# harukaki/brl

Measured on AMD Instinct MI355X. Metric: env-steps/sec at num_envs=8192, 32-step rollout, 1/2/4/8 MI355X, higher is better.
Workload: dtype u8

## Files before the change

brl_amd/_capi.py:

```python
from __future__ import annotations

import ctypes as C
import os

_PKG = os.path.dirname(os.path.abspath(__file__))
LIB_PATH = os.path.join(_PKG, "lib", "libbrl_hip.so")

STATE_WORDS = 16
OBS_SIZE = 480
NUM_ACTIONS = 38

_vp = C.c_void_p


class Fields(C.Structure):
    _names = ["current_player", "terminated", "rewards", "step_count", "turn", "dealer", "vul_ns", "vul_ew",
              "shuffled_players", "last_bid", "last_bidder", "call_x", "call_xx", "pass_num",
              "first_denomination_ns", "first_denomination_ew", "hand", "tricks", "lut_idx", "board_ctr", "illegal"]
    _fields_ = [(n, _vp) for n in _names]


class TransitionPtrs(C.Structure):
    _names = ["done", "action", "value", "reward", "log_prob", "obs", "legal_action_mask"]
    _fields_ = [(n, _vp) for n in _names]


class TableInfoPtrs(C.Structure):
    _names = ["terminated", "rewards", "last_bid", "last_bidder", "call_x", "call_xx"]
    _fields_ = [(n, _vp) for n in _names]


class MacroExt(C.Structure):
    _fields_ = [("first", C.c_int32), ("last", C.c_int32), ("value_in", _vp), ("value_stride", C.c_int64), ("value_out", _vp),
                ("done_out", _vp), ("reward_out", _vp), ("actor", _vp), ("reward_scale", C.c_float), ("obs_fmt", C.c_int32),
                ("terminated_count", _vp), ("obs_cast", _vp), ("in_fmt", C.c_int32), ("reserved", C.c_int32),
                ("head_h", _vp), ("head_ldh", C.c_int64), ("head_w", _vp), ("head_b", _vp), ("head_hidden", C.c_int32),
                ("head_fmt", C.c_int32), ("head_part", _vp), ("head_part_stride", C.c_int64), ("head_part_ld", C.c_int32),
                ("head_nparts", C.c_int32)]


class EvalStatsPtrs(C.Structure):
    _names = ["illegal_prob_sum", "step_count", "pass_count", "bid_count"]
    _fields_ = [(n, _vp) for n in _names]


class MlpRef(C.Structure):
    _fields_ = [("nlayers", C.c_int32), ("act", C.c_int32), ("in_features", C.c_int64), ("hidden", C.c_int64),
                ("w", _vp * 8), ("b", _vp * 8), ("actor_w", _vp), ("actor_b", _vp), ("critic_w", _vp), ("critic_b", _vp)]


class ShardGeom(C.Structure):
    _fields_ = [("nbuckets", C.c_int32), ("world", C.c_int32), ("nsub", C.c_int32), ("reserved", C.c_int32),
                ("off", C.c_int64 * 12), ("len", C.c_int64 * 12)]


class FairNet(C.Structure):
    _fields_ = [("w", _vp * 11), ("b", _vp * 11), ("head_w", _vp), ("head_b", _vp)]


class FairWork(C.Structure):
    _names = ("inp", "dzs", "gates", "cat6", "x4", "dz0", "dz6", "dheads", "tiles", "partials", "gram_partials")
    _fields_ = [(n, _vp) for n in _names]


EVAL_COUNTS = 231


class BrlError(RuntimeError):
    pass


_lib = None


def lib() -> C.CDLL:
    global _lib
    if _lib is not None:
        return _lib
    if not os.path.exists(LIB_PATH):
        raise BrlError(
            f"{LIB_PATH} is missing: the HIP extension has not been built. "
            "Run `python -m brl_amd.build` (needs hipcc, gfx950). brl_amd has no CPU fallback."
        )
    L = C.CDLL(LIB_PATH)
    i64, i32, u32, u64, f32 = C.c_int64, C.c_int, C.c_uint32, C.c_uint64, C.c_float
    L.brl_last_error.restype = C.c_char_p
    L.brl_version.restype = i32
    sigs = {
        "brl_create": [i32, _vp, _vp, i64, C.POINTER(_vp)],
        "brl_set_lut": [_vp, _vp, _vp, i64],
        "brl_destroy": [_vp],
        "brl_set_rng": [_vp, u64, u64],
        "brl_init_random": [_vp, _vp, i64, u32, _vp],
        "brl_init_from_deals": [_vp, _vp, i64, _vp, _vp, _vp, _vp, _vp, _vp, _vp],
        "brl_step": [_vp, _vp, _vp, i64, _vp, i32, _vp, _vp, _vp, _vp, _vp, _vp],
        "brl_observe": [_vp, _vp, i64, _vp, _vp, _vp, _vp],
        "brl_get_fields": [_vp, _vp, i64, C.POINTER(Fields), _vp],
        "brl_rollout_random": [_vp, _vp, i64, i32, i32, u32, f32, C.POINTER(TransitionPtrs), _vp, _vp, _vp, _vp],
        "brl_rollout_random_gae": [_vp, _vp, i64, i32, u32, f32, C.POINTER(TransitionPtrs), _vp, _vp, _vp, _vp, f32, f32, _vp, _vp,
                                   _vp],
        "brl_policy_step": [_vp, _vp, _vp, i64, _vp, i32, u32, i32, _vp, _vp, _vp, _vp, _vp, _vp, _vp, _vp],
        "brl_policy_step_at": [_vp, _vp, _vp, i64, _vp, i64, i32, _vp, u32, i32, _vp, _vp, _vp, _vp, _vp, _vp, _vp, _vp],
        "brl_policy_step_ex": [_vp, _vp, _vp, i64, _vp, i64, i32, _vp, u32, i32, _vp, _vp, _vp, _vp, _vp, _vp, _vp,
                               C.POINTER(MacroExt), _vp],
        "brl_obs_cast": [_vp, _vp, i64, _vp, i32, _vp],
        "brl_obs_cast_rows": [_vp, _vp, _vp, i64, _vp, i32, _vp],
        "brl_live_index": [_vp, _vp, i64, _vp, _vp, i64, _vp],
        "brl_linear_act_heads": [_vp, _vp, i64, _vp, i64, _vp, _vp, i64, i64, i32, i32, i32, i32, _vp, i64, i32, _vp, i64, i64, _vp],
        "brl_linear_act": [_vp, _vp, i64, _vp, i64, _vp, _vp, i64, i64, i32, i32, i32, i32, _vp],
        "brl_gae": [_vp, _vp, _vp, _vp, _vp, f32, f32, i32, i64, _vp, _vp, _vp],
        "brl_imp_reward": [_vp, _vp, _vp, _vp, i64, _vp],
        "brl_duplicate_step": [_vp, _vp, _vp, i64, _vp, C.POINTER(TableInfoPtrs), C.POINTER(TableInfoPtrs),
                               _vp, _vp, _vp, _vp, _vp, _vp],
        "brl_eval_step": [_vp, _vp, _vp, i64, _vp, i64, _vp, i64, C.POINTER(TableInfoPtrs), C.POINTER(TableInfoPtrs),
                          C.POINTER(EvalStatsPtrs), i32, _vp, _vp, _vp, _vp, _vp, _vp, _vp, _vp, _vp],
        "brl_eval_step_team": [_vp, _vp, _vp, i64, _vp, i64, i32, C.POINTER(TableInfoPtrs), C.POINTER(TableInfoPtrs),
                               C.POINTER(EvalStatsPtrs), i32, _vp, _vp, _vp, _vp, _vp, _vp, _vp, _vp, _vp, _vp],
        "brl_eval_reduce": [_vp, i64, C.POINTER(TableInfoPtrs), C.POINTER(TableInfoPtrs), _vp, _vp, _vp, _vp],
        "brl_ppo_loss": [i32, _vp, i64, _vp, _vp, _vp, _vp, _vp, _vp, _vp, i64, f32, f32, f32, i32, i32, _vp, _vp, _vp, _vp, _vp],
        "brl_ppo_stats": [i32, _vp, i64, _vp, f32, f32, _vp, _vp],
        "brl_ppo_heads_loss_split": [i32, _vp, i64, _vp, _vp, i64, _vp, _vp, _vp, _vp, _vp, _vp, i64, f32, f32, f32, i32, i32, i32, _vp, _vp, _vp, _vp, _vp, i32, _vp],
        "brl_ppo_heads_bwd": [i32, _vp, _vp, i64, _vp, i64, i64, i32, i32, _vp, _vp, _vp, _vp, _vp, _vp, i64, _vp, _vp, _vp, _vp],
        "brl_ppo_stats_rows": [i32, _vp, _vp, i64, i64, f32, f32, f32, _vp, _vp],
        "brl_mb_gather_bind": [i32, C.POINTER(TransitionPtrs), _vp, _vp, _vp, _vp, i64, _vp, _vp, _vp, _vp, _vp, _vp, _vp, i64, _vp, _vp],
        "brl_adam_clip_fin_gather": [i32, _vp, _vp, _vp, _vp, i64, _vp, f32, _vp, f32, f32, f32, f32, _vp, i64, _vp, _vp, _vp, i64,
                                     i32, _vp, _vp, _vp, _vp, _vp],
        "brl_mb_gather_dev": [i32, _vp, i64, _vp],
        "brl_ppo_stats_gram": [i32, _vp, i64, i64, _vp, i64, f32, f32, f32, _vp, _vp, _vp, _vp],
        "brl_ppo_illegal_grad": [i32, _vp, _vp, _vp, f32, i64, _vp, _vp],
        "brl_act_bwd_colsum": [i32, _vp, _vp, i64, i64, i64, i32, _vp, _vp],
        "brl_act_bwd_colsum_heads_dw": [i32, _vp, _vp, i64, i64, i64, i32, _vp, _vp, _vp, i64, i64, i64, i32, _vp, _vp, _vp, _vp, i64,
                                        _vp, _vp, _vp, _vp],
        "brl_bias_finalize_ex": [i32, i32, _vp, _vp, _vp, _vp, _vp],
        "brl_bias_finalize_rows": [i32, i32, _vp, _vp, _vp, _vp, i32, _vp, _vp],
        "brl_fair_forward": [i32, C.POINTER(FairNet), _vp, i64, i32, _vp, _vp, _vp],
        "brl_mlp_gemm_group": [i32, i32, i32, _vp, _vp, _vp, _vp, _vp, _vp, _vp, _vp, _vp, _vp],
        "brl_fair_chain": [i32, C.POINTER(FairNet), _vp, _vp, _vp, _vp, _vp, _vp, _vp, i64, f32, f32, f32, i32, i32, i32, i32,
                           C.POINTER(FairWork), _vp],
        "brl_mlp_gemm": [i32, i32, i32, _vp, i64, _vp, i64, _vp, i64, i64, i64, i64, i32, _vp, _vp, i64, _vp, _vp, _vp],
        "brl_mlp_gemm_x3_workspace": [i64, i64, i64, _vp],
        "brl_mlp_gemm_x3_group": [i32, i32, i32, _vp, _vp, _vp, _vp, _vp, _vp, _vp, _vp, _vp, _vp],
        "brl_split_planes": [i32, _vp, i64, _vp, i64, _vp],
        "brl_linear_x3p": [i32, _vp, i32, i64, i64, _vp, i64, i64, _vp, i32, _vp, i64, _vp, i64, i64, i64, i64, i64, _vp],
        "brl_mlp_gemm_x3": [i32, i32, i32, _vp, i64, _vp, i64, _vp, i64, i64, i64, i64, i32, _vp, _vp, i64, _vp, _vp, i64, _vp],
        "brl_mlp_forward_rows": [i32, C.POINTER(MlpRef), _vp, _vp, i64, _vp, i64, _vp, i64, _vp],
        "brl_adam_shard_norm": [i32, _vp, C.POINTER(ShardGeom), i32, i32, f32, _vp, _vp, _vp, _vp],
        "brl_adam_shard_apply": [i32, _vp, _vp, _vp, _vp, C.POINTER(ShardGeom), i32, i32, _vp, _vp, f32, _vp, f32, f32, f32, f32, f32, _vp,
                                 _vp, i64, _vp],
        "brl_mlp_gemm_dh_heads_dw": [i32, _vp, i64, _vp, i64, _vp, i64, i64, i64, i64, i32, _vp, i64, _vp, _vp, _vp, i64, i64, i64, i32,
                                     _vp, _vp, _vp, _vp, i64, _vp, _vp, _vp, _vp],
    }
    sigs.update(sl_signatures())
    for name, args in sigs.items():
        fn = getattr(L, name)
        fn.argtypes = args
        fn.restype = i32
    _lib = L
    return L


EXPORTS = ["brl_last_error", "brl_version", "brl_create", "brl_set_lut", "brl_destroy", "brl_set_rng",
           "brl_init_random", "brl_init_from_deals", "brl_step", "brl_observe", "brl_get_fields",
           "brl_rollout_random", "brl_policy_step", "brl_policy_step_at", "brl_obs_cast", "brl_obs_cast_rows", "brl_live_index", "brl_linear_act", "brl_linear_act_heads", "brl_gae", "brl_imp_reward", "brl_duplicate_step",
           "brl_eval_step", "brl_eval_reduce", "brl_ppo_loss", "brl_ppo_stats", "brl_policy_step_ex",
           "brl_eval_step_team", "brl_rollout_random_gae", "brl_ppo_heads_loss_split", "brl_adam_shard_norm", "brl_adam_shard_apply", "brl_ppo_heads_bwd", "brl_ppo_stats_gram",
           "brl_act_bwd_colsum", "brl_act_bwd_colsum_heads_dw", "brl_bias_finalize_ex", "brl_ppo_stats_rows", "brl_mb_gather_bind", "brl_mb_gather_dev", "brl_ppo_illegal_grad", "brl_adam_clip_fin_gather", "brl_mlp_gemm", "brl_mlp_gemm_dh_heads_dw", "brl_mlp_forward_rows",
           "brl_bias_finalize_rows", "brl_fair_chain", "brl_mlp_gemm_group", "brl_fair_forward", "brl_mlp_gemm_x3", "brl_mlp_gemm_x3_workspace", "brl_mlp_gemm_x3_group", "brl_split_planes", "brl_linear_x3p"]


def sl_signatures() -> dict:
    i64, i32, u64, f32 = C.c_int64, C.c_int, C.c_uint64, C.c_float
    return {
        "brl_sl_sample": [i32, _vp, _vp, i64, u64, i64, _vp, _vp, _vp],
        "brl_sl_replay": [i32, _vp, _vp, _vp, i64, _vp, _vp, i64, _vp, _vp, _vp, _vp],
        "brl_sl_loss": [i32, _vp, i64, _vp, _vp, i64, f32, _vp, _vp, _vp, i64, _vp],
    }


def check(rc: int) -> None:
    if rc != 0:
        raise BrlError(f"libbrl_hip error {rc}: {lib().brl_last_error().decode()}")


def ptr(t):
    if t is None:
        return None
    assert t.is_contiguous(), "brl_amd passes raw pointers: tensors must be contiguous"
    return t.data_ptr()
```

brl_amd/csrc/brl_mlp_gemm_x3.hip:

```cpp
#include <hip/hip_runtime.h>
#include <stdint.h>

#include "abi_common.hpp"
#include "mlp_gemm_x3.hpp"
#include "mlp_linear_x3p.hpp"

static int64_t x3_tiles(int64_t m, int64_t n) { return ((m + 127) / 128) * ((n + 127) / 128); }

static int64_t x3_workspace_bytes(int64_t m, int64_t n, int64_t k) {
  const int sk = mgs::pick_splitk(m, n, k);
  if (sk == 1) return 0;
  const int64_t tiles = x3_tiles(m, n);
  return ((tiles * 4 + 255) / 256) * 256 + tiles * sk * (int64_t)mgs::SLAB_FLOATS * 4;
}

extern "C" int brl_mlp_gemm_x3_workspace(int64_t m, int64_t n, int64_t k, int64_t *bytes) {
  NEED(bytes && m > 0 && n > 0 && k > 0, "bytes / m / n / k");
  *bytes = x3_workspace_bytes(m, n, k);
  return BRL_OK;
}

extern "C" int brl_mlp_gemm_x3(int device, int layout, int epilogue, const float *a, int64_t lda, const float *b, int64_t ldb, float *c,
                               int64_t ldc, int64_t m, int64_t n, int64_t k, int act, const float *bias, const float *gate, int64_t ldg,
                               float *colsum, void *workspace, int64_t workspace_bytes, void *stream) {
  NEED(a && b && c && m > 0 && n > 0 && k > 0, "a / b / c / m / n / k");
  NEED(layout >= BRL_GEMM_NT && layout <= BRL_GEMM_TN, "layout (BRL_GEMM_NT / _NN / _TN)");
  NEED(m < (1 << 24) && n < (1 << 24) && k < (1 << 24), "m / n / k below 2^24");
  NEED(n % 4 == 0 && ldc % 4 == 0 && lda % 4 == 0 && ldb % 4 == 0 && ldc >= n, "n and the leading dimensions multiples of 4 (16-byte pieces)");
  const bool akc = layout != BRL_GEMM_TN, bkc = layout == BRL_GEMM_NT;
  NEED(k % 32 == 0, "k a multiple of 32 (whole 32-deep chunks; other k: brl_mlp_gemm)");
  NEED(akc ? lda >= k : lda >= ((m + 3) & ~(int64_t)3), "lda (where m is contiguous in a: at least m rounded up to 4 — whole 16-byte pieces are read)");
  NEED(bkc ? ldb >= k : ldb >= n, "ldb");
  NEED((akc ? m * lda : k * lda) < (1ll << 29) && (bkc ? n * ldb : k * ldb) < (1ll << 29), "operands below 2 GB");
  NEED(act == 0 || act == 1, "act (0 ReLU, 1 tanh)");
  NEED((epilogue == BRL_GEMM_EPI_NONE) || (epilogue == BRL_GEMM_EPI_BIAS_ACT && layout == BRL_GEMM_NT && bias) ||
           (epilogue == BRL_GEMM_EPI_GATE_COLSUM && layout == BRL_GEMM_NN && gate && ldg >= n && ldg % 4 == 0),
       "epilogue (NONE; BIAS_ACT with NT + bias; GATE_COLSUM with NN + gate)");
  NEED((((uintptr_t)a | (uintptr_t)b | (uintptr_t)c | (uintptr_t)bias | (uintptr_t)gate | (uintptr_t)colsum) & 15) == 0, "16-byte alignment");
  HIP_TRY(hipSetDevice(device));
  mgs::Args X{};
  mg::Args &G = X.g;
  G.A = a; G.lda = lda; G.B = b; G.ldb = ldb; G.C = c; G.ldc = ldc;
  G.M = (int)m; G.N = (int)n; G.K = (int)k; G.act = act;
  G.bias = bias; G.gate = gate; G.ldg = ldg; G.colsum = colsum;
  const int64_t tiles = x3_tiles(m, n);
  int sk = mgs::pick_splitk(m, n, k);
  const int64_t tick = ((tiles * 4 + 255) / 256) * 256;
  if (sk > 1 && (workspace == nullptr || workspace_bytes < tick + tiles * sk * (int64_t)mgs::SLAB_FLOATS * 4)) sk = 1;
  NEED(sk == 1 || (((uintptr_t)workspace) & 255) == 0, "workspace: 256-byte alignment");
  NEED(sk == 1 || tiles * sk * (int64_t)mgs::SLAB_FLOATS * 4 < (1ll << 31), "partial tiles below 2 GB");
  X.splitk = sk;
  X.tickets = (unsigned *)workspace;
  X.slabs = sk > 1 ? (float *)((char *)workspace + tick) : nullptr;
  const unsigned blocks = (unsigned)(tiles * sk);
  hipStream_t s = (hipStream_t)stream;
#define X3_LAUNCH(AK, BK_, E) hipLaunchKernelGGL((mgs::k_gemm_x3s<AK, BK_, E>), dim3(blocks), dim3(mgs::THREADS), 0, s, X)
  if (layout == BRL_GEMM_NT) {
    if (epilogue == BRL_GEMM_EPI_BIAS_ACT) X3_LAUNCH(true, true, mg::EPI_BIAS_ACT);
    else X3_LAUNCH(true, true, mg::EPI_NONE);
  } else if (layout == BRL_GEMM_NN) {
    if (epilogue == BRL_GEMM_EPI_GATE_COLSUM) X3_LAUNCH(true, false, mg::EPI_GATE_COLSUM);
    else X3_LAUNCH(true, false, mg::EPI_NONE);
  } else {
    X3_LAUNCH(false, false, mg::EPI_NONE);
  }
#undef X3_LAUNCH
  HIP_TRY(hipGetLastError());
  return BRL_OK;
}

extern "C" int brl_mlp_gemm_x3_group(int device, int layout, int count, const float *const *a, const int64_t *lda, const float *const *b,
                                     const int64_t *ldb, float *const *c, const int64_t *ldc, const int64_t *m, const int64_t *n,
                                     const int64_t *k, void *stream) {
  NEED(count >= 1 && count <= mgs::GROUP_MAX && a && lda && b && ldb && c && ldc && m && n && k, "count (1..8) / NULL array");
  NEED(layout >= BRL_GEMM_NT && layout <= BRL_GEMM_TN, "layout (BRL_GEMM_NT / _NN / _TN)");
  const bool akc = layout != BRL_GEMM_TN, bkc = layout == BRL_GEMM_NT;
  mgs::GroupArgs GA{};
  GA.n = count;
  for (int i = 0; i < count; i++) {
    NEED(a[i] && b[i] && c[i] && m[i] > 0 && n[i] > 0 && k[i] > 0, "a / b / c / m / n / k");
    NEED(m[i] < (1 << 24) && n[i] < (1 << 24) && k[i] < (1 << 24), "m / n / k below 2^24");
    NEED(n[i] % 4 == 0 && ldc[i] % 4 == 0 && lda[i] % 4 == 0 && ldb[i] % 4 == 0 && ldc[i] >= n[i], "n and the leading dimensions multiples of 4");
    NEED(k[i] % 32 == 0, "k a multiple of 32 (whole 32-deep chunks; other k: brl_mlp_gemm_group)");
    NEED(akc ? lda[i] >= k[i] : lda[i] >= ((m[i] + 3) & ~(int64_t)3), "lda (where m is contiguous in a: at least m rounded up to 4)");
    NEED(bkc ? ldb[i] >= k[i] : ldb[i] >= n[i], "ldb");
    NEED((akc ? m[i] * lda[i] : k[i] * lda[i]) < (1ll << 29) && (bkc ? n[i] * ldb[i] : k[i] * ldb[i]) < (1ll << 29), "operands below 2 GB");
    NEED((((uintptr_t)a[i] | (uintptr_t)b[i] | (uintptr_t)c[i]) & 15) == 0, "16-byte alignment");
    mgs::Args &X = GA.x[i];
    mg::Args &G = X.g;
    G.A = a[i]; G.lda = lda[i]; G.B = b[i]; G.ldb = ldb[i]; G.C = c[i]; G.ldc = ldc[i];
    G.M = (int)m[i]; G.N = (int)n[i]; G.K = (int)k[i];
    X.splitk = 1;
    GA.first[i + 1] = GA.first[i] + (int)x3_tiles(m[i], n[i]);
  }
  HIP_TRY(hipSetDevice(device));
  hipStream_t s = (hipStream_t)stream;
  const unsigned blocks = (unsigned)GA.first[count];
  if (layout == BRL_GEMM_NT) hipLaunchKernelGGL((mgs::k_gemm_x3s_group<true, true>), dim3(blocks), dim3(mgs::THREADS), 0, s, GA);
  else if (layout == BRL_GEMM_NN) hipLaunchKernelGGL((mgs::k_gemm_x3s_group<true, false>), dim3(blocks), dim3(mgs::THREADS), 0, s, GA);
  else hipLaunchKernelGGL((mgs::k_gemm_x3s_group<false, false>), dim3(blocks), dim3(mgs::THREADS), 0, s, GA);
  HIP_TRY(hipGetLastError());
  return BRL_OK;
}

extern "C" int brl_split_planes(int device, const float *x, int64_t n, uint16_t *planes, int64_t plane_stride, void *stream) {
  NEED(x && planes && n > 0 && n % 4 == 0 && plane_stride >= n && plane_stride % 4 == 0, "x / planes / n (a multiple of 4) / plane_stride");
  NEED((((uintptr_t)x) & 15) == 0 && (((uintptr_t)planes) & 7) == 0, "alignment (x 16 bytes, planes 8)");
  HIP_TRY(hipSetDevice(device));
  hipLaunchKernelGGL(lx3::k_split_planes, dim3((unsigned)((n / 4 + 255) / 256)), dim3(256), 0, (hipStream_t)stream, x, planes, plane_stride, n / 4);
  HIP_TRY(hipGetLastError());
  return BRL_OK;
}

extern "C" int brl_linear_x3p(int device, const uint16_t *x_planes, int npx, int64_t ldx, int64_t sx, const uint16_t *w_planes, int64_t ldw,
                              int64_t sw, const float *bias, int relu, float *y, int64_t ldy, uint16_t *y_planes, int64_t ldyp, int64_t syp,
                              int64_t m, int64_t n, int64_t k, void *stream) {
  NEED(x_planes && w_planes && bias && (y || y_planes) && m > 0 && n > 0 && k > 0, "x_planes / w_planes / bias / an output / m / n / k");
  NEED(npx == 1 || npx == 3, "npx (3 planes, or 1: x exact in bf16)");
  NEED(n % 128 == 0 && k % 32 == 0, "n a multiple of 128, k a multiple of 32");
  NEED(m < (1 << 24) && n < (1 << 24) && k < (1 << 24), "m / n / k below 2^24");
  NEED(ldx >= k && ldx % 8 == 0 && ldw >= k && ldw % 8 == 0, "ldx / ldw (at least k, multiples of 8: 16-byte pieces)");
  NEED(m * ldx < (1ll << 31) && n * ldw < (1ll << 31), "planes below 4 GB each");
  NEED(!y || (ldy >= n && ldy % 4 == 0), "ldy");
  NEED(!y_planes || (ldyp >= n && ldyp % 8 == 0 && syp % 8 == 0), "ldyp / syp (multiples of 8)");
  NEED(sx % 8 == 0 && sw % 8 == 0, "plane strides multiples of 8");
  NEED((((uintptr_t)x_planes | (uintptr_t)w_planes | (uintptr_t)bias | (uintptr_t)y | (uintptr_t)y_planes) & 15) == 0, "16-byte alignment");
  HIP_TRY(hipSetDevice(device));
  lx3::Args G{};
  G.x = x_planes; G.ldx = ldx; G.sx = sx; G.w = w_planes; G.ldw = ldw; G.sw = sw; G.bias = bias;
  G.y = y; G.ldy = ldy; G.yp = y_planes; G.ldyp = ldyp; G.syp = syp;
  G.M = (int)m; G.N = (int)n; G.K = (int)k; G.relu = relu ? 1 : 0;
  hipStream_t s = (hipStream_t)stream;
  const unsigned blocks = (unsigned)(((m + 127) / 128) * (n / 128));
  if (npx == 3) hipLaunchKernelGGL(lx3::k_linear_x3p<3>, dim3(blocks), dim3(lx3::THREADS), 0, s, G);
  else hipLaunchKernelGGL(lx3::k_linear_x3p<1>, dim3(blocks), dim3(lx3::THREADS), 0, s, G);
  HIP_TRY(hipGetLastError());
  return BRL_OK;
}
```

brl_amd/csrc/brl_ppo.hip:

```cpp
#include <hip/hip_runtime.h>
#include <math.h>
#include <stdint.h>
#include <stdio.h>
#include <stdlib.h>
#include <string.h>

#include "abi_common.hpp"

static inline unsigned thread_grid(int64_t n, int bs) { return (unsigned)((n + bs - 1) / bs); }

struct PpoArgs {
  const float *logits;
  int64_t ls;
  const float *value;
  const uint8_t *mask;
  const int32_t *action;
  const float *old_value, *old_logp, *gae, *tgt;
  int64_t B;
  float clip_eps, vf_coef, ent_coef;
  int masked, value_clipping;
  float *dlogits, *dvalue, *partials, *illp;
  int64_t vs, dls, dvs;
};

template <int CTRL, int ROW_MASK = 0xF>
__device__ __forceinline__ float dpp_move_f(float old, float v) {
  return __uint_as_float((unsigned)__builtin_amdgcn_update_dpp((int)__float_as_uint(old), (int)__float_as_uint(v), CTRL, ROW_MASK, 0xF, false));
}
__device__ __forceinline__ float wave_sum_f(float v) {
  v += dpp_move_f<0xB1>(0.0f, v);
  v += dpp_move_f<0x4E>(0.0f, v);
  v += dpp_move_f<0x124>(0.0f, v);
  v += dpp_move_f<0x128>(0.0f, v);
  v += dpp_move_f<0x142, 0xA>(0.0f, v);
  v += dpp_move_f<0x143, 0xC>(0.0f, v);
  return __uint_as_float(__builtin_amdgcn_readlane(__float_as_uint(v), 63));
}
__device__ __forceinline__ float wave_max_f(float v) {
  const float ninf = -INFINITY;
  v = fmaxf(v, dpp_move_f<0xB1>(ninf, v));
  v = fmaxf(v, dpp_move_f<0x4E>(ninf, v));
  v = fmaxf(v, dpp_move_f<0x124>(ninf, v));
  v = fmaxf(v, dpp_move_f<0x128>(ninf, v));
  v = fmaxf(v, dpp_move_f<0x142, 0xA>(ninf, v));
  v = fmaxf(v, dpp_move_f<0x143, 0xC>(ninf, v));
  return __uint_as_float(__builtin_amdgcn_readlane(__float_as_uint(v), 63));
}

struct PpoSampleIn {
  bool legal;
  int act;
  float old_logp, old_value, tgt, gae;
};
__device__ __forceinline__ PpoSampleIn ppo_sample_load(const PpoArgs &A, int64_t b, bool valid, int lane) {
  const int64_t bb = valid ? b : 0;
  PpoSampleIn S;
  S.legal = (lane < BRL_NUM_ACTIONS) && A.mask[bb * BRL_NUM_ACTIONS + ((lane < BRL_NUM_ACTIONS) ? lane : 0)] != 0;
  S.act = A.action[bb];
  S.old_logp = A.old_logp[bb];
  S.old_value = A.old_value[bb];
  S.tgt = A.tgt[bb];
  S.gae = A.gae[bb];
  return S;
}
__device__ __forceinline__ void ppo_loss_sample(const PpoArgs &A, const PpoSampleIn &S, int64_t b, bool valid, int lane, float lg, float v,
                                                float g, float (&st)[5], float &illp_lane) {
  const bool in = lane < BRL_NUM_ACTIONS;
  const bool legal = S.legal;
  const float invB = 1.0f / (float)A.B;
  const float mx = wave_max_f(legal ? lg : -INFINITY);
  const float lse = logf(wave_sum_f(legal ? expf(lg - mx) : 0.0f));
  const float lsm = legal ? (lg - mx) - lse : 0.0f;
  const float p = legal ? expf(lsm) : 0.0f;
  const float mx2 = wave_max_f(in ? lg : -INFINITY);
  const float lse2 = logf(wave_sum_f(in ? expf(lg - mx2) : 0.0f));
  const float lsm2 = in ? (lg - mx2) - lse2 : 0.0f;
  const float p2 = in ? expf(lsm2) : 0.0f;
  const int act = S.act;
  const float lsel = A.masked ? lsm : lsm2, psel = A.masked ? p : p2;
  const float lp = __shfl(lsel, act & 63, 64);
  const float logratio = lp - S.old_logp;
  const float ratio = expf(logratio);
  const float eps = A.clip_eps;
  const float a1 = ratio * g, a2 = fminf(fmaxf(ratio, 1.0f - eps), 1.0f + eps) * g;
  const float la = -fminf(a1, a2);
  const bool inside = (ratio >= 1.0f - eps) && (ratio <= 1.0f + eps);
  const float dratio = ((a1 < a2) || inside) ? -g : 0.0f;
  const float dlp = dratio * ratio * invB;
  const float ov = S.old_value, t = S.tgt;
  float vl, dv;
  if (A.value_clipping) {
    const float dcl = fminf(fmaxf(v - ov, -eps), eps);
    const float vc = ov + dcl;
    const float l1 = (v - t) * (v - t), l2 = (vc - t) * (vc - t);
    vl = 0.5f * fmaxf(l1, l2);
    const bool unclipped = (v - ov >= -eps) && (v - ov <= eps);
    dv = (l1 >= l2) ? (v - t) : (unclipped ? (vc - t) : 0.0f);
  } else {
    vl = 0.5f * (v - t) * (v - t);
    dv = v - t;
  }
  const float H = -wave_sum_f((legal && p > 0.0f) ? p * lsm : 0.0f);
  const float dH = legal ? -p * (lsm + H) : 0.0f;
  const float onehot = (lane == act) ? 1.0f : 0.0f;
  const bool live = A.masked ? legal : in;
  const float dz = (live ? dlp * (onehot - psel) : 0.0f) - A.ent_coef * invB * dH;
  illp_lane = legal ? 0.0f : p2;
  if (valid && in) {
    A.dlogits[b * A.dls + lane] = dz;
    if (A.illp) A.illp[b * BRL_NUM_ACTIONS + lane] = illp_lane;
  }
  if (lane == 0 && valid) A.dvalue[b * A.dvs] = A.vf_coef * dv * invB;
  st[0] = valid ? vl : 0.0f;
  st[1] = valid ? la : 0.0f;
  st[2] = valid ? H : 0.0f;
  st[3] = valid ? (ratio - 1.0f) - logratio : 0.0f;
  st[4] = (valid && fabsf(ratio - 1.0f) > eps) ? 1.0f : 0.0f;
}

__global__ __launch_bounds__(256) void k_ppo_loss(PpoArgs A) {
  __shared__ float part[4][8];
  const int lane = (int)(threadIdx.x & 63u), wave = (int)(threadIdx.x >> 6);
  const int64_t b = (int64_t)blockIdx.x * 4 + wave;
  const bool valid = b < A.B;
  const int64_t bb = valid ? b : 0;
  const float lg = (lane < BRL_NUM_ACTIONS) ? A.logits[bb * A.ls + lane] : 0.0f;
  const PpoSampleIn S = ppo_sample_load(A, b, valid, lane);
  float st[5], ill;
  ppo_loss_sample(A, S, b, valid, lane, lg, A.value[bb * A.vs], S.gae, st, ill);
  if (lane == 0) {
#pragma unroll
    for (int k = 0; k < 5; k++) part[wave][k] = st[k];
  }
  __syncthreads();
  if (threadIdx.x < 8) {
    const int k = (int)threadIdx.x;
    A.partials[(int64_t)blockIdx.x * 8 + k] = (k < 5) ? ((part[0][k] + part[1][k]) + (part[2][k] + part[3][k])) : 0.0f;
  }
}

__global__ __launch_bounds__(512) void k_ppo_stats(const float *partials, int64_t nblk, int64_t batch, const float *G,
                                                   float vf_coef, float ent_coef, float *out, const int32_t *row_index) {
  if (row_index != nullptr) out += 8 * (int64_t)(*row_index);
  constexpr int D = BRL_NUM_ACTIONS, DD = D * D;
  __shared__ float g[DD], m[DD], t[DD], vec[D], red[2], st[8];
  const int tid = (int)threadIdx.x, lane = tid & 63, wv = tid >> 6;
  if (wv >= 3) {
    const int k = wv - 3;
    float s = 0.0f;
    for (int64_t i = lane; i < nblk; i += 64) s += partials[i * 8 + k];
    s = wave_sum_f(s);
    if (lane == 0) st[k] = s / (float)batch;
  }
  for (int e = tid; e < DD; e += 512) g[e] = G ? G[e] : 0.0f;
  __syncthreads();
  auto trace_of = [&](const float *x) {
    if (wv == 0) {
      const float s = wave_sum_f((lane < D) ? x[lane * D + lane] : 0.0f);
      if (lane == 0) red[0] = fmaxf(s, 1.17549435e-38f);
    }
    __syncthreads();
    return red[0];
  };
  float tr = trace_of(g);
  for (int e = tid; e < DD; e += 512) m[e] = g[e] / tr;
  __syncthreads();
  for (int it = 0; it < 8; it++) {
    for (int e = tid; e < DD; e += 512) {
      const int i = e / D, j = e - i * D;
      float s = 0.0f;
#pragma unroll 2
      for (int k = 0; k < D; k++) s += m[i * D + k] * m[k * D + j];
      t[e] = s;
    }
    __syncthreads();
    tr = trace_of(t);
    for (int e = tid; e < DD; e += 512) m[e] = t[e] / tr;
    __syncthreads();
  }
  if (tid < D) {
    float s = 0.0f;
    for (int k = 0; k < D; k++) s += m[tid * D + k];
    vec[tid] = s;
  }
  __syncthreads();
  if (wv == 0) {
    float gv = 0.0f;
    if (lane < D)
      for (int k = 0; k < D; k++) gv += g[lane * D + k] * vec[k];
    const float vi = (lane < D) ? vec[lane] : 0.0f;
    const float num = wave_sum_f(vi * gv), den = wave_sum_f(vi * vi);
    if (lane == 0) {
      out[6] = 0.5f * sqrtf(fmaxf(num / fmaxf(den, 1.17549435e-38f), 0.0f));
      out[0] = st[1] + vf_coef * st[0] - ent_coef * st[2];
      out[1] = st[0]; out[2] = st[1]; out[3] = st[2]; out[4] = st[3]; out[5] = st[4];
      out[7] = 0.0f;
    }
  }
}

#include "ppo_update.hpp"
#include "ppo_heads.hpp"
#include "fair_chain.hpp"

extern "C" int brl_ppo_loss(int device, const float *logits, int64_t logits_stride, const float *value, const uint8_t *mask,
                            const int32_t *action, const float *old_value, const float *old_log_prob, const float *gae,
                            const float *targets, int64_t batch, float clip_eps, float vf_coef, float ent_coef, int masked,
                            int value_clipping, float *dlogits, float *dvalue, float *partials, float *illegal_probs,
                            void *stream) {
  NEED(batch > 0, "batch");
  NEED(logits && value && mask && action && old_value && old_log_prob && gae && targets, "NULL input array");
  NEED(dlogits && dvalue && partials, "NULL output array");
  NEED(logits_stride >= BRL_NUM_ACTIONS, "logits_stride");
  HIP_TRY(hipSetDevice(device));
  PpoArgs A{logits, logits_stride, value, mask, action, old_value, old_log_prob, gae, targets, batch, clip_eps, vf_coef,
            ent_coef, masked, value_clipping, dlogits, dvalue, partials, illegal_probs, 1, BRL_NUM_ACTIONS, 1};
  hipLaunchKernelGGL(k_ppo_loss, dim3(thread_grid(batch, 4)), dim3(256), 0, (hipStream_t)stream, A);
  HIP_TRY(hipGetLastError());
  return BRL_OK;
}

extern "C" int brl_mb_gather_bind(int device, const brl_transition *flat, const float *adv, const float *targets, const int64_t *perm,
                                  const int32_t *mb_index, int64_t mbs, float *x0, uint8_t *mask, int32_t *action, float *old_value,
                                  float *old_log_prob, float *gae_out, float *targets_out, int64_t nsteps, void *args_dev,
                                  void *stream) {
  NEED(flat && flat->obs && flat->legal_action_mask && flat->action && flat->value && flat->log_prob, "trajectory");
  NEED(adv && targets && perm && mb_index && mbs > 0, "adv / targets / perm / mb_index / mbs");
  NEED(x0 && mask && action && old_value && old_log_prob && gae_out && targets_out && args_dev, "NULL output array / args_dev");
  HIP_TRY(hipSetDevice(device));
  static_assert(sizeof(GatherArgs) <= 256, "args_dev is 256 bytes");
  NEED(nsteps > 0, "nsteps (minibatches in perm)");
  GatherArgs A{flat->obs, flat->legal_action_mask, flat->action, flat->value, flat->log_prob, adv, targets, perm, mb_index, mbs,
               x0, mask, action, old_value, old_log_prob, gae_out, targets_out, nsteps};
  hipLaunchKernelGGL(k_mb_gather_bind, dim3(1), dim3(64), 0, (hipStream_t)stream, A, (GatherArgs *)args_dev);
  HIP_TRY(hipGetLastError());
  return BRL_OK;
}

extern "C" int brl_mb_gather_dev(int device, const void *args_dev, int64_t mbs, void *stream) {
  NEED(args_dev && mbs > 0, "args_dev / mbs");
  HIP_TRY(hipSetDevice(device));
  hipLaunchKernelGGL(k_mb_gather_dev, dim3((unsigned)mbs), dim3(128), 0, (hipStream_t)stream, (const GatherArgs *)args_dev);
  HIP_TRY(hipGetLastError());
  return BRL_OK;
}

extern "C" int brl_act_bwd_colsum(int device, float *dh, const float *h, int64_t rows, int64_t cols, int64_t ld, int act,
                                  float *scratch, void *stream) {
  NEED(dh && h && scratch && rows > 0 && cols > 0 && ld >= cols, "dh / h / scratch / rows / cols / ld");
  NEED(cols % 4 == 0 && ld % 4 == 0, "cols and ld multiples of 4");
  NEED(act == 0 || act == 1, "act (0 ReLU, 1 tanh)");
  HIP_TRY(hipSetDevice(device));
  const int64_t tiles = (rows + 15) / 16;
  hipLaunchKernelGGL(k_relu_bwd_tiles4, dim3((unsigned)((cols + 255) / 256), (unsigned)tiles), dim3(256), 0, (hipStream_t)stream,
                     dh, h, rows, cols, ld, scratch, act);
  HIP_TRY(hipGetLastError());
  return BRL_OK;
}

extern "C" int brl_act_bwd_colsum_heads_dw(int device, float *dz, const float *hh, int64_t rows, int64_t cols, int64_t ld, int act,
                                           float *scratch, const float *dheads, const float *h, int64_t ldh, int64_t batch,
                                           int64_t hidden, int nsplit, float *dw_partials, float *db_partials,
                                           const float *loss_partials, const float *gram_partials, int64_t ngroups,
                                           const int32_t *row_index, float *stat_sums, float *gram_sums, void *stream) {
  NEED(dz && hh && scratch && rows > 0 && cols > 0 && ld >= cols, "dz / h / scratch / rows / cols / ld");
  NEED(cols % 4 == 0 && ld % 4 == 0, "cols and ld multiples of 4");
  NEED(act == 0 || act == 1, "act (0 ReLU, 1 tanh)");
  NEED(batch > 0 && hidden > 0 && hidden % 256 == 0 && ldh >= hidden && ldh % 4 == 0, "batch / hidden (a multiple of 256) / ldh");
  NEED(dheads && h && dw_partials && db_partials, "NULL array");
  NEED(nsplit >= 1 && (batch + nsplit - 1) / nsplit <= 64, "nsplit: at most 64 rows per split");
  HIP_TRY(hipSetDevice(device));
  HeadsBwdArgs A{};
  A.dheads = dheads; A.h = h; A.ldh = ldh; A.B = batch; A.H = (int)hidden; A.act = act; A.nsplit = nsplit;
  A.rows_per_split = (int)((batch + nsplit - 1) / nsplit);
  A.dWh_partials = dw_partials; A.dbh_partials = db_partials;
  A.blocks_a = (int)(hidden / HB_JT) * nsplit;
  const bool sums = gram_sums != nullptr;
  NEED(!sums || (loss_partials && gram_partials && ngroups > 0 && row_index && stat_sums), "statistics sums: partials / ngroups / row_index / stat_sums");
  A.loss_partials = loss_partials; A.gram_partials = gram_partials; A.ngroups = (int)ngroups; A.row_index = row_index;
  A.stat_sums = stat_sums; A.gram_sums = gram_sums;
  const int gx = (int)((cols + 255) / 256), gy = (int)((rows + 15) / 16);
  const unsigned blocks = (unsigned)(gx * gy + A.blocks_a + (sums ? HB_GRAM_BLOCKS : 0));
  hipLaunchKernelGGL(k_relu_bwd_tiles4_heads_dw, dim3(blocks), dim3(256), 0, (hipStream_t)stream, dz, hh, rows, cols, ld, scratch, act, gx, gy, A);
  HIP_TRY(hipGetLastError());
  return BRL_OK;
}

extern "C" int brl_bias_finalize_ex(int device, int nseg, const float *const *partials, const int64_t *cols, const int64_t *tiles,
                                    float *const *out, void *stream) {
  NEED(nseg >= 1 && nseg <= BIAS_MAX_SEGS && partials && cols && tiles && out, "nseg / partials / cols / tiles / out");
  HIP_TRY(hipSetDevice(device));
  BiasSegs S{};
  S.n = nseg;
  int64_t maxc = 0;
  for (int i = 0; i < nseg; i++) {
    NEED(partials[i] && out[i] && cols[i] > 0 && tiles[i] > 0, "segment");
    S.tiles[i] = tiles[i]; S.partials[i] = partials[i]; S.cols[i] = cols[i]; S.db[i] = out[i];
    maxc = cols[i] > maxc ? cols[i] : maxc;
  }
  hipLaunchKernelGGL(k_bias_finalize, dim3((unsigned)((maxc + 63) / 64), (unsigned)nseg), dim3(256), 0, (hipStream_t)stream, S);
  HIP_TRY(hipGetLastError());
  return BRL_OK;
}

extern "C" int brl_bias_finalize_rows(int device, int nseg, const float *const *partials, const int64_t *cols, const int64_t *tiles,
                                      float *const *out, int first_row_seg, const int32_t *row_index, void *stream) {
  NEED(nseg >= 1 && nseg <= BIAS_MAX_SEGS && partials && cols && tiles && out, "nseg / partials / cols / tiles / out");
  NEED(first_row_seg >= 0 && first_row_seg <= nseg && (row_index || first_row_seg == nseg), "first_row_seg / row_index");
  HIP_TRY(hipSetDevice(device));
  BiasSegs S{};
  S.n = nseg;
  int64_t maxc = 0;
  for (int i = 0; i < nseg; i++) {
    NEED(partials[i] && out[i] && cols[i] > 0 && tiles[i] > 0, "segment");
    S.tiles[i] = tiles[i]; S.partials[i] = partials[i]; S.cols[i] = cols[i]; S.db[i] = out[i];
    maxc = cols[i] > maxc ? cols[i] : maxc;
  }
  S.row_index = (first_row_seg < nseg) ? row_index : nullptr;
  S.first_row_seg = first_row_seg;
  hipLaunchKernelGGL(k_bias_finalize, dim3((unsigned)((maxc + 63) / 64), (unsigned)nseg), dim3(256), 0, (hipStream_t)stream, S);
  HIP_TRY(hipGetLastError());
  return BRL_OK;
}

#ifdef FAIR_TIMING
extern "C" int brl_fair_set_dbg(void *p) {
  HIP_TRY(hipMemcpyToSymbol(HIP_SYMBOL(g_fair_dbg), &p, sizeof(p)));
  return BRL_OK;
}
#endif

extern "C" int brl_fair_chain(int device, const brl_fair_net *net, const float *x0, const uint8_t *mask, const int32_t *action,
                              const float *old_value, const float *old_log_prob, const float *gae, const float *targets,
                              int64_t batch, float clip_eps, float vf_coef, float ent_coef, int masked, int value_clipping,
                              int reward_scaling, int act, const brl_fair_work *work, void *stream) {
  NEED(net && work && x0 && mask && action && old_value && old_log_prob && gae && targets, "NULL input");
  NEED(batch > 0 && batch % fair::R == 0, "batch (a multiple of 16)");
  NEED(act == 0 || act == 1, "act");
  fair::Args A{};
  for (int l = 0; l < 11; l++) {
    NEED(net->w[l] && net->b[l], "net: NULL layer");
    NEED((((uintptr_t)net->w[l]) & 15) == 0 && (((uintptr_t)net->b[l]) & 15) == 0, "net: 16-byte alignment");
    A.net.w[l] = net->w[l]; A.net.b[l] = net->b[l];
  }
  NEED(net->head_w && net->head_b && (((uintptr_t)net->head_w) & 15) == 0, "net: heads");
  A.net.wh = net->head_w; A.net.bh = net->head_b;
  NEED(work->inp && work->dzs && work->gates && work->cat6 && work->x4 && work->dz0 && work->dz6 && work->dheads && work->tiles &&
       work->partials, "work: NULL array");
  const void *al[] = {x0, work->inp, work->dzs, work->gates, work->cat6, work->x4, work->dz0, work->dz6, work->tiles};
  for (const void *q : al) NEED((((uintptr_t)q) & 15) == 0, "16-byte alignment");
  A.o = fair::Bufs{work->inp, work->dzs, work->gates, work->cat6, work->x4, work->dz0, work->dz6, work->dheads, work->tiles,
                   work->partials, work->gram_partials};
  A.x0 = x0;
  A.P = PpoArgs{nullptr, 0, nullptr, mask, action, old_value, old_log_prob, gae, targets, batch, clip_eps, vf_coef,
                ent_coef, masked, value_clipping, nullptr, nullptr, nullptr, nullptr, 1, BRL_NUM_ACTIONS, 1};
  A.act = act;
  A.reward_scaling = reward_scaling;
  HIP_TRY(hipSetDevice(device));
  A.nrows = batch;
  hipLaunchKernelGGL(fair::k_fair_chain<true>, dim3((unsigned)(batch / fair::R)), dim3(fair::NW * 64), 0, (hipStream_t)stream, A);
  HIP_TRY(hipGetLastError());
  return BRL_OK;
}

extern "C" int brl_fair_forward(int device, const brl_fair_net *net, const float *x, int64_t rows, int act, float *logits, float *value,
                                void *stream) {
  NEED(net && x && logits && value, "NULL array");
  NEED(rows >= 0 && rows < (1ll << 31), "rows");
  NEED(act == 0 || act == 1, "act");
  if (rows == 0) return BRL_OK;
  fair::Args A{};
  for (int l = 0; l < 11; l++) {
    NEED(net->w[l] && net->b[l], "net: NULL layer");
    NEED((((uintptr_t)net->w[l]) & 15) == 0 && (((uintptr_t)net->b[l]) & 15) == 0, "net: 16-byte alignment");
    A.net.w[l] = net->w[l]; A.net.b[l] = net->b[l];
  }
  NEED(net->head_w && net->head_b && (((uintptr_t)net->head_w) & 15) == 0 && (((uintptr_t)x) & 15) == 0, "net: heads / x: 16-byte alignment");
  A.net.wh = net->head_w; A.net.bh = net->head_b;
  A.x0 = x;
  A.act = act;
  A.nrows = rows;
  A.logits_out = logits;
  A.value_out = value;
  HIP_TRY(hipSetDevice(device));
  hipLaunchKernelGGL(fair::k_fair_chain<false>, dim3((unsigned)((rows + fair::R - 1) / fair::R)), dim3(fair::NW * 64), 0,
                     (hipStream_t)stream, A);
  HIP_TRY(hipGetLastError());
  return BRL_OK;
}

extern "C" int brl_ppo_heads_loss_split(int device, const float *h, int64_t ldh, const float *head_w, const float *head_b,
                                        int64_t hidden, const uint8_t *mask, const int32_t *action, const float *old_value,
                                        const float *old_log_prob, const float *gae, const float *targets, int64_t batch,
                                        float clip_eps, float vf_coef, float ent_coef, int masked, int value_clipping,
                                        int reward_scaling, float *heads_out, float *dheads, float *partials, float *gram_partials,
                                        float *head_parts, int ksplit, void *stream) {
  NEED(batch > 0 && hidden > 0 && hidden % 16 == 0 && ldh >= hidden && ldh % 4 == 0, "batch / hidden (a multiple of 16) / ldh");
  NEED(h && head_w && head_b && mask && action && old_value && old_log_prob && gae && targets, "NULL input array");
  NEED(dheads && partials && head_parts, "NULL output array");
  NEED(ksplit >= 1 && ksplit <= 8, "ksplit (1..8)");
  HIP_TRY(hipSetDevice(device));
  constexpr int64_t HS = BRL_NUM_ACTIONS + 1;
  HeadsProductArgs G{};
  G.h = h; G.ldh = ldh; G.Wh = head_w; G.H = (int)hidden; G.B = batch; G.ksplit = ksplit; G.parts = head_parts; G.part_stride = batch * HS;
  hipLaunchKernelGGL(k_heads_product, dim3((unsigned)((batch + 15) / 16), (unsigned)ksplit), dim3(HD_WAVES * 64), 0, (hipStream_t)stream, G);
  HeadsLossArgs A{};
  A.h = h; A.ldh = ldh; A.Wh = head_w; A.bh = head_b; A.H = (int)hidden;
  A.P = PpoArgs{nullptr, HS, nullptr, mask, action, old_value, old_log_prob, gae, targets, batch, clip_eps, vf_coef,
                ent_coef, masked, value_clipping, dheads, dheads + BRL_NUM_ACTIONS, partials, nullptr, HS, HS, HS};
  A.heads_out = heads_out; A.gram_partials = gram_partials; A.reward_scaling = reward_scaling;
  A.parts = head_parts; A.nparts = ksplit; A.part_stride = batch * HS;
  hipLaunchKernelGGL(k_heads_loss, dim3((unsigned)((batch + HD_ROWS - 1) / HD_ROWS)), dim3(HD_WAVES * 64), 0, (hipStream_t)stream, A);
  HIP_TRY(hipGetLastError());
  return BRL_OK;
}

extern "C" int brl_ppo_heads_bwd(int device, const float *dheads, const float *h, int64_t ldh, const float *head_w, int64_t batch,
                                 int64_t hidden, int act, int nsplit, float *dw_partials, float *db_partials, float *dh,
                                 float *tile_sums, const float *loss_partials, const float *gram_partials, int64_t ngroups,
                                 const int32_t *row_index, float *stat_sums, float *gram_sums, void *stream) {
  NEED(batch > 0 && hidden > 0 && hidden % 256 == 0 && ldh >= hidden && ldh % 4 == 0, "batch / hidden (a multiple of 256) / ldh");
  NEED(dheads && h && head_w && dh && tile_sums && (!dw_partials == !db_partials), "NULL array");
  const bool with_dw = dw_partials != nullptr;
  NEED(act == 0 || act == 1, "act (0 ReLU, 1 tanh)");
  NEED(nsplit >= 1 && (batch + nsplit - 1) / nsplit <= 64, "nsplit: at most 64 rows per split");
  HIP_TRY(hipSetDevice(device));
  HeadsBwdArgs A{};
  A.dheads = dheads; A.h = h; A.ldh = ldh; A.Wh = head_w; A.B = batch; A.H = (int)hidden; A.act = act; A.nsplit = nsplit;
  A.rows_per_split = (int)((batch + nsplit - 1) / nsplit);
  A.dWh_partials = dw_partials; A.dbh_partials = db_partials; A.dh = dh; A.tile_sums = tile_sums;
  A.blocks_a = (int)(hidden / HB_JT) * nsplit;
  const bool sums = with_dw && gram_sums != nullptr;
  NEED(!sums || (loss_partials && gram_partials && ngroups > 0 && row_index && stat_sums), "statistics sums: partials / ngroups / row_index / stat_sums");
  A.loss_partials = loss_partials; A.gram_partials = gram_partials; A.ngroups = (int)ngroups; A.row_index = row_index;
  A.stat_sums = stat_sums; A.gram_sums = gram_sums;
  const int64_t blocks_b = (hidden / 256) * ((batch + HB_ROWS - 1) / HB_ROWS);
  hipLaunchKernelGGL(k_heads_bwd_dh, dim3((unsigned)blocks_b), dim3(256), 0, (hipStream_t)stream, A);
  if (with_dw)
    hipLaunchKernelGGL(k_heads_bwd_dw, dim3((unsigned)(A.blocks_a + (sums ? HB_GRAM_BLOCKS : 0))), dim3(256), 0, (hipStream_t)stream, A);
  HIP_TRY(hipGetLastError());
  return BRL_OK;
}

extern "C" int brl_ppo_stats_gram(int device, const float *partials, int64_t npartials, int64_t batch, const float *gram_partials,
                                  int64_t ngram, float vf_coef, float ent_coef, float illegal_coef, float *out_rows,
                                  const int32_t *row_index, float *vec_out, void *stream) {
  NEED(partials && out_rows && npartials > 0 && batch > 0, "partials / out_rows / npartials / batch");
  NEED(gram_partials && ngram > 0, "gram_partials / ngram");
  HIP_TRY(hipSetDevice(device));
  hipLaunchKernelGGL(k_ppo_stats2, dim3(1), dim3(1024), 0, (hipStream_t)stream, partials, npartials, batch, gram_partials, ngram,
                     vf_coef, ent_coef, illegal_coef, out_rows, row_index, vec_out);
  HIP_TRY(hipGetLastError());
  return BRL_OK;
}

extern "C" int brl_ppo_illegal_grad(int device, const float *heads, const uint8_t *mask, const float *vec, float illegal_coef,
                                    int64_t batch, float *dheads, void *stream) {
  NEED(heads && mask && vec && dheads && batch > 0, "heads / mask / vec / dheads / batch");
  HIP_TRY(hipSetDevice(device));
  hipLaunchKernelGGL(k_illegal_grad, dim3(thread_grid(batch, 4)), dim3(256), 0, (hipStream_t)stream, heads, mask, vec, illegal_coef,
                     batch, dheads);
  HIP_TRY(hipGetLastError());
  return BRL_OK;
}

extern "C" int brl_ppo_stats_rows(int device, const float *stat_sums, const float *gram_sums, int64_t rows, int64_t batch, float vf_coef,
                                  float ent_coef, float illegal_coef, float *out_rows, void *stream) {
  NEED(stat_sums && gram_sums && out_rows && rows > 0 && batch > 0, "stat_sums / gram_sums / out_rows / rows / batch");
  HIP_TRY(hipSetDevice(device));
  hipLaunchKernelGGL(k_ppo_stats2, dim3((unsigned)rows), dim3(256), 0, (hipStream_t)stream, stat_sums, (int64_t)1, batch, gram_sums,
                     (int64_t)1, vf_coef, ent_coef, illegal_coef, out_rows, (const int32_t *)nullptr, (float *)nullptr);
  HIP_TRY(hipGetLastError());
  return BRL_OK;
}

extern "C" int brl_adam_clip_fin_gather(int device, float *p, float *g, float *m, float *v, int64_t n, float *step, float lr,
                                        const float *lr_dev, float beta1, float beta2, float eps, float max_norm, float *scratch,
                                        int64_t scratch_len, int32_t *mb_index, float *norm_out, const void *gather_args, int64_t mbs,
                                        int nseg, const float *const *partials, const int64_t *cols, const int64_t *tiles,
                                        float *const *out, void *stream) {
  NEED(nseg >= 1 && nseg <= BIAS_MAX_SEGS && partials && cols && tiles && out, "nseg / partials / cols / tiles / out");
  NEED(p && g && m && v && step && scratch && n > 0 && n % 4 == 0, "p / g / m / v / step / scratch / n (a multiple of 4)");
  NEED(!gather_args || (mb_index && mbs > 0), "gather_args needs mb_index and the minibatch size");
  BiasSegs S{};
  S.n = nseg;
  int64_t covered = 0;
  const float *lo = g + n;
  for (int i = 0; i < nseg; i++) {
    NEED(partials[i] && out[i] && cols[i] > 0 && tiles[i] > 0, "segment");
    NEED(out[i] >= g && out[i] + cols[i] <= g + n, "segment outputs must lie inside the gradient buffer");
    S.tiles[i] = tiles[i]; S.partials[i] = partials[i]; S.cols[i] = cols[i]; S.db[i] = out[i];
    covered += cols[i];
    lo = (out[i] < lo) ? out[i] : lo;
  }
  const int64_t tail_lo = lo - g;
  NEED(tail_lo % 4 == 0 && covered <= n - tail_lo && n - tail_lo - covered < 4, "the finalised segments must tile the end of the gradient buffer");
  FinBlocks FB{};
  for (int i = 0; i < nseg; i++) FB.off[i + 1] = FB.off[i] + (int)((cols[i] + 63) / 64);
  NEED(scratch_len >= ADAM_BLOCKS + (int64_t)FB.off[nseg], "scratch too small for the finalize blocks' partials");
  HIP_TRY(hipSetDevice(device));
  const int npartials = ADAM_BLOCKS + FB.off[nseg];
  hipLaunchKernelGGL(k_adam_norm_fin, dim3((unsigned)npartials), dim3(ADAM_THREADS), 0, (hipStream_t)stream, g, n, 1.0f, scratch, step,
                     mb_index, S, tail_lo, FB);
  const unsigned extra = gather_args ? (unsigned)((mbs + 1) / 2) : 0u;
  AdamRange R{};
  R.p = p; R.g = g; R.m = m; R.v = v; R.lo4 = 0; R.hi4 = n >> 2; R.partials = scratch; R.npartials = npartials; R.step = step;
  R.lr_dev = lr_dev; R.lr = lr; R.b1 = beta1; R.b2 = beta2; R.eps = eps; R.max_norm = max_norm; R.gscale = 1.0f; R.norm_out = norm_out;
  hipLaunchKernelGGL(k_adam_apply, dim3((unsigned)ADAM_BLOCKS + extra), dim3(ADAM_THREADS), 0, (hipStream_t)stream, R, ADAM_BLOCKS,
                     (const GatherArgs *)gather_args);
  HIP_TRY(hipGetLastError());
  return BRL_OK;
}

static int shard_geom(const brl_shard_geom *geom, int rank_lo, int rank_hi, ShardGeom *out) {
  NEED(geom && geom->nbuckets >= 1 && geom->nbuckets <= SHARD_MAX_BUCKETS && geom->world >= 1 && geom->nsub >= 1, "geometry");
  NEED(rank_lo >= 0 && rank_lo < rank_hi && rank_hi <= geom->world, "rank range");
  ShardGeom G{};
  G.nb = geom->nbuckets; G.world = geom->world; G.J = geom->nsub;
  for (int b = 0; b < G.nb; b++) {
    NEED(geom->off[b] >= 0 && geom->off[b] % 4 == 0 && geom->len[b] > 0 && geom->len[b] % 4 == 0, "bucket offsets / slice lengths multiples of 4 floats");
    G.off4[b] = geom->off[b] >> 2; G.len4[b] = geom->len[b] >> 2;
    G.blk[b + 1] = G.blk[b] + (int)((G.len4[b] + SHARD_PER4 - 1) / SHARD_PER4);
  }
  *out = G;
  return BRL_OK;
}

extern "C" int brl_adam_shard_norm(int device, const float *g, const brl_shard_geom *geom, int rank_lo, int rank_hi, float grad_scale,
                                   float *partials, float *step, int32_t *mb_index, void *stream) {
  NEED(g && partials && step, "g / partials / step");
  ShardGeom G;
  if (int rc = shard_geom(geom, rank_lo, rank_hi, &G)) return rc;
  HIP_TRY(hipSetDevice(device));
  hipLaunchKernelGGL(k_shard_norm, dim3((unsigned)((rank_hi - rank_lo) * G.nb * G.J)), dim3(ADAM_THREADS), 0, (hipStream_t)stream, g, G,
                     rank_lo, grad_scale, partials, step, mb_index);
  HIP_TRY(hipGetLastError());
  return BRL_OK;
}

extern "C" int brl_adam_shard_apply(int device, float *p, const float *g, float *m, float *v, const brl_shard_geom *geom, int rank_lo,
                                    int rank_hi, const float *partials, const float *step, float lr, const float *lr_dev, float beta1,
                                    float beta2, float eps, float max_norm, float grad_scale, float *norm_out, const void *gather_args,
                                    int64_t mbs, void *stream) {
  NEED(p && g && m && v && partials && step, "p / g / m / v / partials / step");
  NEED(!gather_args || mbs > 0, "gather_args needs the minibatch size");
  ShardGeom G;
  if (int rc = shard_geom(geom, rank_lo, rank_hi, &G)) return rc;
  HIP_TRY(hipSetDevice(device));
  AdamRange R{};
  R.p = p; R.g = g; R.m = m; R.v = v; R.partials = partials; R.npartials = G.world * G.nb * G.J; R.step = step;
  R.lr_dev = lr_dev; R.lr = lr; R.b1 = beta1; R.b2 = beta2; R.eps = eps; R.max_norm = max_norm; R.gscale = grad_scale; R.norm_out = norm_out;
  const int sweep = (rank_hi - rank_lo) * G.blk[G.nb];
  const unsigned extra = gather_args ? (unsigned)((mbs + 1) / 2) : 0u;
  hipLaunchKernelGGL(k_shard_apply, dim3((unsigned)sweep + extra), dim3(ADAM_THREADS), 0, (hipStream_t)stream, R, G, rank_lo, sweep,
                     (const GatherArgs *)gather_args);
  HIP_TRY(hipGetLastError());
  return BRL_OK;
}

extern "C" int brl_ppo_stats(int device, const float *partials, int64_t batch, const float *gram, float vf_coef,
                             float ent_coef, float *out, void *stream) {
  NEED(partials && out && batch > 0, "partials / out / batch");
  HIP_TRY(hipSetDevice(device));
  hipLaunchKernelGGL(k_ppo_stats, dim3(1), dim3(512), 0, (hipStream_t)stream, partials, (int64_t)thread_grid(batch, 4), batch,
                     gram, vf_coef, ent_coef, out, (const int32_t *)nullptr);
  HIP_TRY(hipGetLastError());
  return BRL_OK;
}
```

brl_amd/csrc/mlp_gemm_x3.hpp:

```cpp
#pragma once

#include "mlp_gemm.hpp"

namespace mgs {

using mg::BoolTag;
using mg::f32x4;
using mg::IntTag;
using mg::row16_sum;
typedef __bf16 bf16x8 __attribute__((ext_vector_type(8)));
typedef float f32x16 __attribute__((ext_vector_type(16)));
typedef unsigned u32x4 __attribute__((ext_vector_type(4)));
typedef unsigned u32x2 __attribute__((ext_vector_type(2)));
typedef short s16x4 __attribute__((ext_vector_type(4)));

constexpr int BK = 32, THREADS = 512;
constexpr int PLANE = 128 * BK * 2;
constexpr int OFF_B = 3 * PLANE, STAGE = 6 * PLANE;
constexpr int LDS_BYTES = 2 * STAGE;
constexpr int SLAB_FLOATS = 128 * 128;

#ifndef MGS_R1
#define MGS_R1 6
#endif
#ifndef MGS_BAR
#define MGS_BAR 20
#endif
#ifndef MGS_EXP
#define MGS_EXP 0
#endif

struct Args {
  mg::Args g;
  float *slabs;
  unsigned *tickets;
  int splitk;
};

template <bool A_KC, bool B_KC, int EPI>
__device__ __forceinline__ void gemm_tile(const Args &X, unsigned char *lds, int bid, int nblk) {
  const mg::Args &G = X.g;
  constexpr int NP = 4;
  const int tid = (int)threadIdx.x, lane = tid & 63, w = __builtin_amdgcn_readfirstlane(tid >> 6);
  const int tiles_m = (G.M + 127) / 128, tiles_n = (G.N + 127) / 128, SK = X.splitk;
  if (bid >= tiles_m * tiles_n * SK) return;
  const int L = (nblk % 8 == 0) ? (bid % 8) * (nblk / 8) + bid / 8 : bid;
  const int tile = L / SK, ks = L - tile * SK;
  int tm, tn;
  if (tiles_m % 2 == 0 && tiles_n % 4 == 0) {
    const int blk = tile >> 3, i = tile & 7;
    tm = 2 * (blk / (tiles_n / 4)) + (i >> 2);
    tn = 4 * (blk % (tiles_n / 4)) + (i & 3);
  } else {
    tm = tile / tiles_n;
    tn = tile - tm * tiles_n;
  }
  const int m0 = tm * 128, n0 = tn * 128;
  const int nchunks = G.K / BK;
  const int cps = (nchunks + SK - 1) / SK;
  const int c0 = ks * cps, c1 = (c0 + cps < nchunks) ? c0 + cps : nchunks;
  const int ni = c1 > c0 ? c1 - c0 : 0;

  uint32_t go[NP];
  int lw[NP];
#pragma unroll
  for (int j = 0; j < NP; j++) {
    const bool isB = j >= 2;
    const int q = tid + 512 * (j & 1);
    const int x0 = isB ? n0 : m0, Xn = isB ? G.N : G.M;
    const int64_t ld = isB ? G.ldb : G.lda;
    const int base = isB ? OFF_B : 0;
    if (isB ? B_KC : A_KC) {
      const int row = q >> 3, P = (q >> 1) & 3, half = q & 1;
      const int x = (x0 + row < Xn) ? x0 + row : Xn - 1;
      go[j] = (uint32_t)(((int64_t)x * ld + 16 * half + 4 * P) * 4);
      lw[j] = base + row * 64 + ((P ^ ((row >> 2) & 3)) << 4) + 8 * half;
    } else {
      const int kr = q >> 5, p = q & 31;
      const int col = (x0 + 4 * p < Xn) ? x0 + 4 * p : 0;
      go[j] = (uint32_t)(((int64_t)kr * ld + col) * 4);
      lw[j] = base + kr * 256 + ((p ^ ((kr & 3) << 3)) << 3);
    }
  }
  const uint32_t stepa = (uint32_t)((A_KC ? (int64_t)BK : (int64_t)BK * G.lda) * 4), stepb = (uint32_t)((B_KC ? (int64_t)BK : (int64_t)BK * G.ldb) * 4);
  const __amdgpu_buffer_rsrc_t srda = __builtin_amdgcn_make_buffer_rsrc(const_cast<float *>(G.A), (short)0, 0x7FFFFFFF, 0x00020000);
  const __amdgpu_buffer_rsrc_t srdb = __builtin_amdgcn_make_buffer_rsrc(const_cast<float *>(G.B), (short)0, 0x7FFFFFFF, 0x00020000);
  uint32_t soa = (uint32_t)c0 * stepa, sob = (uint32_t)c0 * stepb;
  unsigned msk;
  asm volatile("s_mov_b32 %0, 0xffff0000" : "=s"(msk));
#ifndef MGS_SETS
#define MGS_SETS 1
#endif
  f32x4 rg[MGS_SETS][NP];
  int nreq = 0;
  auto gload = [&](auto set_tag, int j) __attribute__((always_inline)) {
    constexpr int S = decltype(set_tag)::value;
    const bool isB = j >= 2;
    rg[S][j] = __builtin_bit_cast(f32x4, __builtin_amdgcn_raw_buffer_load_b128(isB ? srdb : srda, (int)go[j], (int)(isB ? sob : soa), 0));
  };
  auto gadvance = [&]() __attribute__((always_inline)) {
    nreq++;
    if (nreq < ni) { soa += stepa; sob += stepb; }
  };
  unsigned sh[3][2];
  float sr0, sr1;
  auto stage_part = [&](auto set_tag, int j, int half, int part, unsigned char *st) __attribute__((always_inline)) {
    constexpr int S = decltype(set_tag)::value;
    if (part == 0) {
      const f32x4 v = rg[S][j];
      const float x0 = half ? v.z : v.x, x1 = half ? v.w : v.y;
      const unsigned u0 = __float_as_uint(x0), u1 = __float_as_uint(x1);
      sh[0][half] = __builtin_amdgcn_perm(u1, u0, 0x07060302u);
      if (MGS_EXP & 1) { sr0 = x0; sr1 = x1; }
      else { sr0 = x0 - __uint_as_float(u0 & msk); sr1 = x1 - __uint_as_float(u1 & msk); }
    } else if (part == 1) {
      const unsigned v0 = __float_as_uint(sr0), v1 = __float_as_uint(sr1);
      sh[1][half] = __builtin_amdgcn_perm(v1, v0, 0x07060302u);
      if (!(MGS_EXP & 1)) { sr0 = sr0 - __uint_as_float(v0 & msk); sr1 = sr1 - __uint_as_float(v1 & msk); }
    } else {
      sh[2][half] = __builtin_amdgcn_perm(__float_as_uint(sr1), __float_as_uint(sr0), 0x07060302u);
      if (half) {
        unsigned char *p = st + lw[j];
        *reinterpret_cast<u32x2 *>(p) = u32x2{sh[0][0], sh[0][1]};
        *reinterpret_cast<u32x2 *>(p + PLANE) = u32x2{sh[1][0], sh[1][1]};
        *reinterpret_cast<u32x2 *>(p + 2 * PLANE) = u32x2{sh[2][0], sh[2][1]};
      }
    }
  };

  const int wm = w >> 2, wn = w & 3, r32 = lane & 31, hh = lane >> 5;
  int fa[2], fb;
  {
    const int qq = (lane >> 2) & 3, xg = 16 * ((lane >> 4) & 1) + 4 * (lane & 3);
#pragma unroll
    for (int b = 0; b < 2; b++) {
      const int ra = wm * 64 + 32 * b + r32;
      fa[b] = A_KC ? ra * 64 + ((hh ^ ((ra >> 2) & 3)) << 4) : (4 * hh + qq) * 256 + ((((wm * 64 + 32 * b + xg) >> 2) ^ (qq << 3)) << 3);
    }
    const int rb = wn * 32 + r32;
    fb = OFF_B + (B_KC ? rb * 64 + ((hh ^ ((rb >> 2) & 3)) << 4) : (4 * hh + qq) * 256 + ((((wn * 32 + xg) >> 2) ^ (qq << 3)) << 3));
  }
  auto read_frag = [&](const unsigned char *st, int s, int u) __attribute__((always_inline)) -> bf16x8 {
    const bool isB = u >= 6;
    const bool kc = isB ? B_KC : A_KC;
    const int base = isB ? fb : fa[u / 3], plane = (u % 3) * PLANE;
    if (kc) return __builtin_bit_cast(bf16x8, *reinterpret_cast<const u32x4 *>(st + (base ^ (s << 5)) + plane));
    const unsigned char *p = st + base + plane + 2048 * s;
    const s16x4 lo4 = __builtin_amdgcn_ds_read_tr16_b64_v4i16((__attribute__((address_space(3))) s16x4 *)(p));
    const s16x4 hi4 = __builtin_amdgcn_ds_read_tr16_b64_v4i16((__attribute__((address_space(3))) s16x4 *)(p + 4096));
    typedef short s16x8 __attribute__((ext_vector_type(8)));
    return __builtin_bit_cast(bf16x8, s16x8{lo4[0], lo4[1], lo4[2], lo4[3], hi4[0], hi4[1], hi4[2], hi4[3]});
  };

  f32x16 acc[2][2];
#pragma unroll
  for (int b = 0; b < 2; b++)
#pragma unroll
    for (int c = 0; c < 2; c++)
#pragma unroll
      for (int e = 0; e < 16; e++) acc[b][c][e] = 0.0f;
  auto mf = [&](const bf16x8 (&f)[9], int t) __attribute__((always_inline)) {
    const int b = t / 6, p = t % 6;
    const int pa = (p == 0 || p == 3 || p == 5) ? 0 : (p == 2 || p == 4) ? 1 : 2;
    const int pb = (p == 1 || p == 4 || p == 5) ? 0 : (p == 2 || p == 3) ? 1 : 2;
    const int cls = p < 5 ? 1 : 0;
    if (!(MGS_EXP & 2)) acc[b][cls] = __builtin_amdgcn_mfma_f32_32x32x16_bf16(f[6 + pb], f[3 * b + pa], acc[b][cls], 0, 0, 0);
  };

  MG_STAMP(0);
  if (ni > 0) {
#pragma unroll
    for (int j = 0; j < NP; j++) gload(IntTag<0>{}, j);
    gadvance();
#pragma unroll
    for (int j = 0; j < NP; j++)
#pragma unroll
      for (int h = 0; h < 2; h++)
#pragma unroll
        for (int part = 0; part < 3; part++) stage_part(IntTag<0>{}, j, h, part, lds);
#pragma unroll
    for (int j = 0; j < NP; j++) gload(IntTag<(MGS_SETS == 2 ? 1 : 0)>{}, j);
    gadvance();
    if (MGS_SETS == 2) {
#pragma unroll
      for (int j = 0; j < NP; j++) gload(IntTag<0>{}, j);
      gadvance();
    }
  }
  __syncthreads();
  bf16x8 f0[9], f1[9];
  if (ni > 0) {
#pragma unroll
    for (int u = 0; u < 9; u++) f0[u] = read_frag(lds, 0, u);
  }
  MG_STAMP(1);
  auto phase = [&](auto par_tag) __attribute__((always_inline)) {
    constexpr int PAR = decltype(par_tag)::value, NS = PAR ^ 1;
    unsigned char *st = lds + PAR * STAGE, *sn = lds + NS * STAGE;
    constexpr bool real = true, nxt = true, nxt2 = true;
    constexpr int BAR = MGS_BAR;
    auto slot = [&](int s) __attribute__((always_inline)) {
      if (s >= MGS_R1 && s < MGS_R1 + 3 && real) f1[6 + (s - MGS_R1)] = read_frag(st, 1, 6 + (s - MGS_R1));
      if (s >= MGS_R1 + 3 && s < MGS_R1 + 6 && real) f1[s - MGS_R1 - 3] = read_frag(st, 1, s - MGS_R1 - 3);
      if (s >= 12 && s < 15 && real) f1[3 + (s - 12)] = read_frag(st, 1, 3 + (s - 12));
      if (s < BAR && nxt) {
#pragma unroll
        for (int h = 0; h < 8; h++) {
          const int b = (h * (BAR - 2)) / 8;
#pragma unroll
          for (int part = 0; part < 3; part++)
            if (s == b + part) stage_part(IntTag<(MGS_SETS == 2 ? NS : 0)>{}, h >> 1, h & 1, part, sn);
        }
      }
#pragma unroll
      for (int j = 0; j < NP; j++) {
        if (s == ((2 * j + 1) * (BAR - 2)) / 8 + 2 && nxt2) {
          gload(IntTag<(MGS_SETS == 2 ? NS : 0)>{}, j);
          if (j == NP - 1) gadvance();
        }
      }
      if (s == BAR) {
        asm volatile("s_waitcnt lgkmcnt(0)" ::: "memory");
        __builtin_amdgcn_s_barrier();
        asm volatile("" ::: "memory");
      }
      if (s > BAR && nxt) {
        constexpr int order[9] = {6, 7, 8, 0, 1, 2, 3, 4, 5};
        const int n = 23 - BAR, k = s - BAR - 1;
#pragma unroll
        for (int q = (9 * k) / n; q < (9 * (k + 1)) / n; q++) f0[order[q]] = read_frag(sn, 0, order[q]);
      }
    };
#define MGS_STEP(s)                                                                 \
    {                                                                               \
      __builtin_amdgcn_sched_barrier(0);                                            \
      if (real) { if ((s) < 12) mf(f0, (s)); else mf(f1, (s) - 12); }                \
      __builtin_amdgcn_sched_barrier(0);                                            \
      slot(s);                                                                      \
    }
    MGS_STEP(0) MGS_STEP(1) MGS_STEP(2) MGS_STEP(3) MGS_STEP(4) MGS_STEP(5) MGS_STEP(6) MGS_STEP(7)
    MGS_STEP(8) MGS_STEP(9) MGS_STEP(10) MGS_STEP(11) MGS_STEP(12) MGS_STEP(13) MGS_STEP(14) MGS_STEP(15)
    MGS_STEP(16) MGS_STEP(17) MGS_STEP(18) MGS_STEP(19) MGS_STEP(20) MGS_STEP(21) MGS_STEP(22) MGS_STEP(23)
    __builtin_amdgcn_sched_barrier(0);
#undef MGS_STEP
  };
  {
    int i = 0;
    for (; i + 1 < ni; i += 2) {
      phase(IntTag<0>{});
      phase(IntTag<1>{});
    }
    if (i < ni) phase(IntTag<0>{});
  }
  MG_STAMP(2);

  f32x16 v[2];
#pragma unroll
  for (int b = 0; b < 2; b++)
#pragma unroll
    for (int e = 0; e < 16; e++) v[b][e] = acc[b][1][e] + acc[b][0][e];
  if (SK > 1) {
    const __amdgpu_buffer_rsrc_t srs = __builtin_amdgcn_make_buffer_rsrc(X.slabs, (short)0, 0x7FFFFFFF, 0x00020000);
    const uint32_t sbase = (uint32_t)(((int64_t)tile * SK + ks) * SLAB_FLOATS * 4);
#pragma unroll
    for (int b = 0; b < 2; b++)
#pragma unroll
      for (int g = 0; g < 4; g++)
        __builtin_amdgcn_raw_buffer_store_b128(__builtin_bit_cast(u32x4, f32x4{v[b][4 * g], v[b][4 * g + 1], v[b][4 * g + 2], v[b][4 * g + 3]}), srs,
                                               (int)(sbase + (uint32_t)((((w * 2 + b) * 4 + g) * 64 + lane) * 16)), 0, 16);
    asm volatile("s_waitcnt vmcnt(0)" ::: "memory");
    __syncthreads();
    unsigned *flag = reinterpret_cast<unsigned *>(lds);
    if (tid == 0) {
      const unsigned old = __hip_atomic_fetch_add(&X.tickets[tile], 1u, __ATOMIC_RELAXED, __HIP_MEMORY_SCOPE_AGENT);
      *flag = (old == (unsigned)(SK - 1)) ? 1u : 0u;
      if (old == (unsigned)(SK - 1)) __hip_atomic_store(&X.tickets[tile], 0u, __ATOMIC_RELAXED, __HIP_MEMORY_SCOPE_AGENT);
    }
    __syncthreads();
    if (*flag == 0u) return;
    const uint32_t tbase = (uint32_t)((int64_t)tile * SK * SLAB_FLOATS * 4);
#pragma unroll
    for (int b = 0; b < 2; b++)
#pragma unroll
      for (int g = 0; g < 4; g++) {
        const uint32_t idx = (uint32_t)((((w * 2 + b) * 4 + g) * 64 + lane) * 16);
        f32x4 o = __builtin_bit_cast(f32x4, __builtin_amdgcn_raw_buffer_load_b128(srs, (int)(tbase + idx), 0, 16));
        for (int q = 1; q < SK; q++) {
          const f32x4 p = __builtin_bit_cast(f32x4, __builtin_amdgcn_raw_buffer_load_b128(srs, (int)(tbase + idx), q * SLAB_FLOATS * 4, 16));
          o.x += p.x; o.y += p.y; o.z += p.z; o.w += p.w;
        }
        v[b][4 * g] = o.x; v[b][4 * g + 1] = o.y; v[b][4 * g + 2] = o.z; v[b][4 * g + 3] = o.w;
      }
  }
  const bool relu = G.act == 0;
#pragma unroll
  for (int g = 0; g < 4; g++) {
    const int n = n0 + 32 * wn + 8 * g + 4 * hh, nc = n < G.N ? n : 0;
    f32x4 bias4 = f32x4{0.f, 0.f, 0.f, 0.f};
    if (EPI == mg::EPI_BIAS_ACT) bias4 = *reinterpret_cast<const f32x4 *>(G.bias + nc);
    f32x4 cs = f32x4{0.f, 0.f, 0.f, 0.f};
#pragma unroll
    for (int b = 0; b < 2; b++) {
      const int em = m0 + 64 * wm + 32 * b + r32;
      const bool ok = em < G.M && n < G.N;
      f32x4 o = f32x4{v[b][4 * g], v[b][4 * g + 1], v[b][4 * g + 2], v[b][4 * g + 3]};
      if (EPI == mg::EPI_BIAS_ACT) {
        if (relu) {
#pragma unroll
          for (int i = 0; i < 4; i++) o[i] = fmaxf(o[i] + bias4[i], 0.0f);
        } else {
#pragma unroll
          for (int i = 0; i < 4; i++) o[i] = tanhf(o[i] + bias4[i]);
        }
      }
      if (EPI == mg::EPI_GATE_COLSUM) {
        const f32x4 gt = *reinterpret_cast<const f32x4 *>(G.gate + (int64_t)(em < G.M ? em : G.M - 1) * G.ldg + nc);
        if (relu) {
#pragma unroll
          for (int i = 0; i < 4; i++) o[i] = gt[i] > 0.0f ? o[i] : 0.0f;
        } else {
#pragma unroll
          for (int i = 0; i < 4; i++) o[i] = o[i] * (1.0f - gt[i] * gt[i]);
        }
#pragma unroll
        for (int i = 0; i < 4; i++) cs[i] += ok ? o[i] : 0.0f;
      }
      if (ok) *reinterpret_cast<f32x4 *>(G.C + (int64_t)em * G.ldc + n) = o;
    }
    if (EPI == mg::EPI_GATE_COLSUM && G.colsum != nullptr) {
#pragma unroll
      for (int i = 0; i < 4; i++) {
        float c = row16_sum(cs[i]);
        c += __shfl_xor(c, 16, 64);
        cs[i] = c;
      }
      if (r32 == 0 && n < G.N && 2 * tm + wm < (G.M + 63) / 64) *reinterpret_cast<f32x4 *>(G.colsum + (int64_t)(2 * tm + wm) * G.N + n) = cs;
    }
  }
  MG_STAMP(3);
}

template <bool A_KC, bool B_KC, int EPI>
__global__ __launch_bounds__(THREADS) void k_gemm_x3s(Args X) {
  __shared__ __attribute__((aligned(16))) unsigned char lds[LDS_BYTES];
  gemm_tile<A_KC, B_KC, EPI>(X, lds, (int)blockIdx.x, (int)gridDim.x);
}

constexpr int GROUP_MAX = 8;
struct GroupArgs {
  int n;
  int first[GROUP_MAX + 1];
  Args x[GROUP_MAX];
};
template <bool A_KC, bool B_KC>
__global__ __launch_bounds__(THREADS) void k_gemm_x3s_group(GroupArgs GA) {
  __shared__ __attribute__((aligned(16))) unsigned char lds[LDS_BYTES];
  const int b = (int)blockIdx.x;
  int p = 0;
  while (p + 1 < GA.n && b >= GA.first[p + 1]) p++;
  gemm_tile<A_KC, B_KC, mg::EPI_NONE>(GA.x[p], lds, b - GA.first[p], GA.first[p + 1] - GA.first[p]);
}

static inline int pick_splitk(int64_t m, int64_t n, int64_t k) {
  const int64_t tiles = ((m + 127) / 128) * ((n + 127) / 128);
  int sk = 1;
  while (sk < 8 && tiles * sk < 256 && k / 32 / (2 * sk) >= 2) sk *= 2;
  return sk;
}

}
```

brl_amd/csrc/ppo_heads.hpp:

```cpp
#pragma once

constexpr int HD_ROWS = 4;
constexpr int HD_WAVES = 8;
constexpr int HD_MAX_PARTS = 8;
#include "heads_dw_role.hpp"


struct HeadsLossArgs {
  const float *h;
  int64_t ldh;
  const float *Wh;
  const float *bh;
  int H;
  PpoArgs P;
  float *heads_out;
  float *gram_partials;
  int reward_scaling;
  const float *parts;
  int nparts;
  int64_t part_stride;
};

__global__ __launch_bounds__(HD_WAVES * 64) void k_heads_loss(HeadsLossArgs A) {
  __shared__ float illp_s[HD_ROWS][BRL_NUM_ACTIONS + 2];
  __shared__ float part_s[HD_ROWS][8];
  __shared__ float rs_red[HD_WAVES], rs_stat[2];
  const int tid = (int)threadIdx.x, lane = tid & 63, w = tid >> 6;
  const int64_t B = A.P.B, row0 = (int64_t)blockIdx.x * HD_ROWS;

  float adv_mean = 0.0f, adv_inv = 1.0f;
  if (A.reward_scaling) {
    float s = 0.0f;
    for (int64_t i = tid; i < B; i += HD_WAVES * 64) s += A.P.gae[i];
    s = wave_sum_f(s);
    if (lane == 0) rs_red[w] = s;
    __syncthreads();
    if (tid == 0) {
      float t = 0.0f;
      for (int k = 0; k < HD_WAVES; k++) t += rs_red[k];
      rs_stat[0] = t / (float)B;
    }
    __syncthreads();
    adv_mean = rs_stat[0];
    float q = 0.0f;
    for (int64_t i = tid; i < B; i += HD_WAVES * 64) {
      const float d = A.P.gae[i] - adv_mean;
      q += d * d;
    }
    q = wave_sum_f(q);
    __syncthreads();
    if (lane == 0) rs_red[w] = q;
    __syncthreads();
    if (tid == 0) {
      float t = 0.0f;
      for (int k = 0; k < HD_WAVES; k++) t += rs_red[k];
      rs_stat[1] = 1.0f / (sqrtf(t / (float)B) + 1e-8f);
    }
    __syncthreads();
    adv_inv = rs_stat[1];
  }

  const int64_t my_b = row0 + ((w < HD_ROWS) ? w : 0);
  const bool my_valid = w < HD_ROWS && my_b < B;
  const PpoSampleIn my_in = ppo_sample_load(A.P, my_b, my_valid, lane);
  const float my_bias = (lane < HD_NOUT) ? A.bh[lane] : 0.0f;
  float my_part[HD_MAX_PARTS];
#pragma unroll
  for (int p = 0; p < HD_MAX_PARTS; p++)
    my_part[p] = (my_valid && lane < HD_NOUT && p < A.nparts) ? A.parts[(int64_t)p * A.part_stride + my_b * HD_NOUT + lane] : 0.0f;

  if (w < HD_ROWS) {
    const int sl = w;
    const int64_t b = my_b;
    const bool valid = my_valid;
    float hv = 0.0f;
    if (lane < HD_NOUT) {
      hv = my_bias;
#pragma unroll
      for (int p = 0; p < HD_MAX_PARTS; p++) hv += my_part[p];
      if (valid && A.heads_out) A.heads_out[b * HD_NOUT + lane] = hv;
    }
    const float v = __shfl(hv, BRL_NUM_ACTIONS, 64);
    const float g = A.reward_scaling ? (my_in.gae - adv_mean) * adv_inv : my_in.gae;
    float st[5], ill;
    ppo_loss_sample(A.P, my_in, b, valid, lane, hv, v, g, st, ill);
    if (lane < BRL_NUM_ACTIONS) illp_s[sl][lane] = valid ? ill : 0.0f;
    if (lane == 0) {
#pragma unroll
      for (int k = 0; k < 8; k++) part_s[sl][k] = (k < 5) ? st[k] : 0.0f;
    }
  }
  __syncthreads();
  if (tid < 8) {
    float s = 0.0f;
    for (int k = 0; k < HD_ROWS; k++) s += part_s[k][tid];
    A.P.partials[(int64_t)blockIdx.x * 8 + tid] = s;
  }
  if (A.gram_partials != nullptr) {
    for (int e = tid; e < HD_GRAM; e += HD_WAVES * 64) {
      const int i = e / BRL_NUM_ACTIONS, j = e - i * BRL_NUM_ACTIONS;
      float s = 0.0f;
#pragma unroll
      for (int k = 0; k < HD_ROWS; k++) s += illp_s[k][i] * illp_s[k][j];
      A.gram_partials[(int64_t)blockIdx.x * HD_GRAM + e] = s;
    }
  }
}

constexpr int HB_NG = 10;
constexpr int HB_ROWS = 16;

struct HeadsProductArgs {
  const float *h;
  int64_t ldh;
  const float *Wh;
  int H;
  int64_t B;
  int ksplit;
  float *parts;
  int64_t part_stride;
};

__global__ __launch_bounds__(HD_WAVES * 64) void k_heads_product(HeadsProductArgs A) {
  __shared__ float red[HD_WAVES][3][4][64];
  const int tid = (int)threadIdx.x, lane = tid & 63, w = tid >> 6;
  const int64_t row0 = (int64_t)blockIdx.x * 16;
  const int ks = (int)blockIdx.y;
  const int ngroups = A.H / 16, gps = (ngroups + A.ksplit - 1) / A.ksplit;
  const int g_lo = ks * gps, g_hi = (g_lo + gps < ngroups) ? g_lo + gps : ngroups;
  const int r = lane & 15, kq = lane >> 4;
  const int64_t arow = (row0 + r < A.B) ? row0 + r : A.B - 1;
  const float *ap = A.h + arow * A.ldh + 4 * kq;
  const float *bp[3];
  bool bok[3];
#pragma unroll
  for (int nb = 0; nb < 3; nb++) {
    const int n = 16 * nb + r;
    bok[nb] = n < HD_NOUT;
    bp[nb] = A.Wh + (int64_t)(bok[nb] ? n : 0) * A.H + 4 * kq;
  }
  hd_f32x4 acc[3];
#pragma unroll
  for (int nb = 0; nb < 3; nb++) acc[nb] = hd_f32x4{0.f, 0.f, 0.f, 0.f};
  constexpr int GP = 4;
  for (int g0 = g_lo + w; g0 < g_hi; g0 += GP * HD_WAVES) {
    hd_f32x4 av[GP], bv[GP][3];
#pragma unroll
    for (int u = 0; u < GP; u++) {
      const int g = g0 + u * HD_WAVES;
      const int gc = (g < g_hi) ? g : g0;
      av[u] = *reinterpret_cast<const hd_f32x4 *>(ap + 16 * gc);
#pragma unroll
      for (int nb = 0; nb < 3; nb++) bv[u][nb] = *reinterpret_cast<const hd_f32x4 *>(bp[nb] + 16 * gc);
    }
#pragma unroll
    for (int u = 0; u < GP; u++) {
      if (g0 + u * HD_WAVES >= g_hi) break;
#pragma unroll
      for (int nb = 0; nb < 3; nb++) {
#pragma unroll
        for (int s_ = 0; s_ < 4; s_++)
          acc[nb] = __builtin_amdgcn_mfma_f32_16x16x4f32(av[u][s_], bok[nb] ? bv[u][nb][s_] : 0.0f, acc[nb], 0, 0, 0);
      }
    }
  }
#pragma unroll
  for (int nb = 0; nb < 3; nb++)
#pragma unroll
    for (int q = 0; q < 4; q++) red[w][nb][q][lane] = acc[nb][q];
  __syncthreads();
  float *out = A.parts + (int64_t)ks * A.part_stride;
  for (int e = tid; e < 16 * HD_NOUT; e += HD_WAVES * 64) {
    const int row = e / HD_NOUT, col = e - row * HD_NOUT;
    const int nb = col >> 4, c = col & 15, q = row & 3, rq = row >> 2;
    float v = 0.0f;
#pragma unroll
    for (int k = 0; k < HD_WAVES; k++) v += red[k][nb][q][16 * rq + c];
    if (row0 + row < A.B) out[(row0 + row) * HD_NOUT + col] = v;
  }
}


__global__ __launch_bounds__(256) void k_heads_bwd_dw(HeadsBwdArgs A) { heads_bwd_dw_block(A, (int)blockIdx.x); }

__global__ __launch_bounds__(256) void k_relu_bwd_tiles4_heads_dw(float *dh, const float *h, int64_t rows, int64_t cols, int64_t ld,
                                                                   float *partials, int act, int gx, int gy, HeadsBwdArgs A) {
  const int b = (int)blockIdx.x;
  if (b < gx * gy) relu_bwd_tiles4_block(dh, h, rows, cols, ld, partials, act, b % gx, b / gx);
  else heads_bwd_dw_block(A, b - gx * gy);
}

__global__ __launch_bounds__(256) void k_heads_bwd_dh(HeadsBwdArgs A) {
  __shared__ __attribute__((aligned(16))) float dh_s[HB_ROWS][HD_NOUT + 1];
  __shared__ float4 cs_s[4][64];
  const int tid = (int)threadIdx.x;
  const int bb = (int)blockIdx.x;
  const int ct = bb % (A.H / 256), rt = bb / (A.H / 256);
  const int64_t r0 = (int64_t)rt * HB_ROWS;
  for (int e = tid; e < HB_ROWS * HD_NOUT; e += 256) {
    const int rr = e / HD_NOUT, c = e - rr * HD_NOUT;
    dh_s[rr][c] = (r0 + rr < A.B) ? A.dheads[(r0 + rr) * HD_NOUT + c] : 0.0f;
  }
  __syncthreads();
  const int c4 = tid & 63, rg = tid >> 6;
  const int col = ct * 256 + 4 * c4;
  float4 acc[4];
#pragma unroll
  for (int u = 0; u < 4; u++) acc[u] = make_float4(0.f, 0.f, 0.f, 0.f);
  float4 hv[4];
#pragma unroll
  for (int u = 0; u < 4; u++) {
    const int64_t rw = r0 + rg + 4 * u;
    hv[u] = *reinterpret_cast<const float4 *>(A.h + ((rw < A.B) ? rw : A.B - 1) * A.ldh + col);
  }
  const float *wp = A.Wh + col;
  static_assert(HD_NOUT == 39, "three batches of 13 head rows");
#pragma unroll 1
  for (int n0 = 0; n0 < HD_NOUT; n0 += 13) {
    float4 wv[13];
#pragma unroll
    for (int k = 0; k < 13; k++) wv[k] = *reinterpret_cast<const float4 *>(wp + (int64_t)(n0 + k) * A.H);
#pragma unroll
    for (int k = 0; k < 13; k++) {
#pragma unroll
      for (int u = 0; u < 4; u++) {
        const float d = dh_s[rg + 4 * u][n0 + k];
        acc[u].x += d * wv[k].x; acc[u].y += d * wv[k].y; acc[u].z += d * wv[k].z; acc[u].w += d * wv[k].w;
      }
    }
  }
  float4 cs = make_float4(0.f, 0.f, 0.f, 0.f);
#pragma unroll
  for (int u = 0; u < 4; u++) {
    const int64_t rw = r0 + rg + 4 * u;
    float4 z;
    if (A.act == 0) {
      z = make_float4(hv[u].x > 0.f ? acc[u].x : 0.f, hv[u].y > 0.f ? acc[u].y : 0.f, hv[u].z > 0.f ? acc[u].z : 0.f,
                      hv[u].w > 0.f ? acc[u].w : 0.f);
    } else {
      z = make_float4(acc[u].x * (1.0f - hv[u].x * hv[u].x), acc[u].y * (1.0f - hv[u].y * hv[u].y),
                      acc[u].z * (1.0f - hv[u].z * hv[u].z), acc[u].w * (1.0f - hv[u].w * hv[u].w));
    }
    if (rw < A.B) {
      *reinterpret_cast<float4 *>(A.dh + rw * (int64_t)A.H + col) = z;
      cs.x += z.x; cs.y += z.y; cs.z += z.z; cs.w += z.w;
    }
  }
  cs_s[rg][c4] = cs;
  __syncthreads();
  if (rg == 0) {
    const float4 a = cs_s[0][c4], b = cs_s[1][c4], c = cs_s[2][c4], e = cs_s[3][c4];
    *reinterpret_cast<float4 *>(A.tile_sums + (int64_t)rt * A.H + col) =
        make_float4((a.x + b.x) + (c.x + e.x), (a.y + b.y) + (c.y + e.y), (a.z + b.z) + (c.z + e.z), (a.w + b.w) + (c.w + e.w));
  }
}

__global__ __launch_bounds__(1024) void k_ppo_stats2(const float *partials, int64_t nblk, int64_t batch, const float *gram_partials,
                                                    int64_t ngram, float vf_coef, float ent_coef, float ill_coef, float *out,
                                                    const int32_t *row_index, float *vec_out) {
  if (row_index != nullptr) out += 8 * (int64_t)(*row_index);
  out += 8 * (int64_t)blockIdx.x;
  partials += (int64_t)blockIdx.x * nblk * 8;
  gram_partials += (int64_t)blockIdx.x * ngram * (BRL_NUM_ACTIONS * BRL_NUM_ACTIONS);
  constexpr int D = BRL_NUM_ACTIONS, DD = D * D;
  __shared__ float g[DD], m[DD], t[DD], vec[64], st[8], tr_s;
  const int tid = (int)threadIdx.x, lane = tid & 63, wv = tid >> 6;
  const int NT = (int)blockDim.x;
  const int w0 = (NT >= 1024) ? 8 : 3;
  for (int k = (wv >= w0) ? wv - w0 : 5; k < 5; k += (NT >= 1024) ? 5 : 1) {
    float s = 0.0f;
    for (int64_t i = lane; i < nblk; i += 64) s += partials[i * 8 + k];
    s = wave_sum_f(s);
    if (lane == 0) st[k] = s / (float)batch;
  }
  for (int e = tid; e < DD; e += NT) {
    float s = 0.0f;
    for (int64_t i = 0; i < ngram; i += 32) {
      float v[32];
#pragma unroll
      for (int u = 0; u < 32; u++) v[u] = gram_partials[((i + u < ngram) ? i + u : i) * DD + e];
#pragma unroll
      for (int u = 0; u < 32; u++) s += (i + u < ngram) ? v[u] : 0.0f;
    }
    g[e] = s;
  }
  __syncthreads();
  auto trace_of = [&](const float *x) {
    if (wv == 0) {
      const float s = wave_sum_f((lane < D) ? x[lane * D + lane] : 0.0f);
      if (lane == 0) tr_s = 1.0f / fmaxf(s, 1.17549435e-38f);
    }
    __syncthreads();
    return tr_s;
  };
  float inv = trace_of(g);
  for (int e = tid; e < DD; e += NT) m[e] = g[e] * inv;
  __syncthreads();
  for (int it = 0; it < 4; it++) {
    for (int e = tid; e < DD; e += NT) {
      const int i = e / D, j = e - i * D;
      float s = 0.0f;
#pragma unroll 2
      for (int k = 0; k < D; k++) s += m[k * D + i] * m[k * D + j];
      t[e] = s;
    }
    __syncthreads();
    inv = trace_of(t);
    for (int e = tid; e < DD; e += NT) m[e] = t[e] * inv;
    __syncthreads();
  }
  if (wv == 0) {
    float mc[D];
#pragma unroll
    for (int k = 0; k < D; k++) mc[k] = (lane < D) ? m[k * D + lane] : 0.0f;
    float v = (lane < D) ? 1.0f : 0.0f;
    for (int it = 0; it < 16; it++) {
      float s = 0.0f;
#pragma unroll
      for (int k = 0; k < D; k++)
        s += mc[k] * __uint_as_float(__builtin_amdgcn_readlane(__float_as_uint(v), k));
      const float nrm = wave_sum_f(s * s);
      v = (nrm > 0.0f) ? s * (1.0f / sqrtf(nrm)) : v;
    }
    float gv = 0.0f;
#pragma unroll
    for (int k = 0; k < D; k++)
      gv += ((lane < D) ? g[k * D + lane] : 0.0f) * __uint_as_float(__builtin_amdgcn_readlane(__float_as_uint(v), k));
    const float num = wave_sum_f(v * gv), den = wave_sum_f(v * v);
    const float sigma = sqrtf(fmaxf(num / fmaxf(den, 1.17549435e-38f), 0.0f));
    if (vec_out != nullptr && lane < D + 2) vec_out[lane] = (lane < D) ? v * (1.0f / sqrtf(fmaxf(den, 1.17549435e-38f))) : ((lane == D) ? sigma : 0.0f);
    if (lane == 0) {
      out[6] = 0.5f * sigma;
      out[0] = st[1] + vf_coef * st[0] - ent_coef * st[2] + ill_coef * (0.5f * sigma);
      out[1] = st[0]; out[2] = st[1]; out[3] = st[2]; out[4] = st[3]; out[5] = st[4];
      out[7] = 0.0f;
    }
  }
}

__global__ __launch_bounds__(256) void k_illegal_grad(const float *heads, const uint8_t *mask, const float *vec, float coef, int64_t B,
                                                      float *dheads) {
  const int lane = (int)(threadIdx.x & 63u), wave = (int)(threadIdx.x >> 6);
  const int64_t b = (int64_t)blockIdx.x * 4 + wave;
  if (b >= B) return;
  const bool in = lane < BRL_NUM_ACTIONS;
  const float lg = in ? heads[b * HD_NOUT + lane] : 0.0f;
  const bool illegal = in && mask[b * BRL_NUM_ACTIONS + lane] == 0;
  const float v1 = in ? vec[lane] : 0.0f, sigma = vec[BRL_NUM_ACTIONS];
  const float mx = wave_max_f(in ? lg : -INFINITY);
  const float ex = in ? expf(lg - mx) : 0.0f;
  const float p = ex / wave_sum_f(ex);
  const float q = wave_sum_f(illegal ? p * v1 : 0.0f);
  if (in && sigma > 0.0f) dheads[b * HD_NOUT + lane] += (0.5f * coef) * (q / sigma) * p * ((illegal ? v1 : 0.0f) - q);
}
```

brl_amd/csrc/ppo_update.hpp:

```cpp
#pragma once

struct GatherArgs {
  const uint8_t *obs, *mask;
  const int32_t *action;
  const float *value, *log_prob, *adv, *tgt;
  const int64_t *perm;
  const int32_t *mb_index;
  int64_t B;
  float *x0;
  uint8_t *o_mask;
  int32_t *o_action;
  float *o_value, *o_log_prob, *o_adv, *o_tgt;
  int64_t nsteps;
};

__device__ __forceinline__ void mb_gather_row(const GatherArgs &A, int64_t b, int t);

__global__ __launch_bounds__(128) void k_mb_gather_dev(const GatherArgs *Ad) {
  const GatherArgs A = *Ad;
  mb_gather_row(A, blockIdx.x, (int)threadIdx.x);
}
__global__ void k_mb_gather_bind(GatherArgs A, GatherArgs *dst) {
  if (threadIdx.x == 0 && blockIdx.x == 0) *dst = A;
}

__device__ __forceinline__ void mb_gather_row(const GatherArgs &A, int64_t b, int t) {
  const int64_t row = A.perm[(int64_t)(*A.mb_index) * A.B + b];
  if (t < 120) {
    const uint32_t w = reinterpret_cast<const uint32_t *>(A.obs + row * BRL_OBS_SIZE)[t];
    reinterpret_cast<float4 *>(A.x0 + b * BRL_OBS_SIZE)[t] =
        make_float4((float)(w & 0xFFu), (float)((w >> 8) & 0xFFu), (float)((w >> 16) & 0xFFu), (float)(w >> 24));
  }
  if (t < BRL_NUM_ACTIONS) A.o_mask[b * BRL_NUM_ACTIONS + t] = A.mask[row * BRL_NUM_ACTIONS + t];
  if (t >= 64 && t < 69) {
    const int k = t - 64;
    const uint32_t *src = (k == 0) ? reinterpret_cast<const uint32_t *>(A.action)
                        : (k == 1) ? reinterpret_cast<const uint32_t *>(A.value)
                        : (k == 2) ? reinterpret_cast<const uint32_t *>(A.log_prob)
                        : (k == 3) ? reinterpret_cast<const uint32_t *>(A.adv) : reinterpret_cast<const uint32_t *>(A.tgt);
    uint32_t *dst = (k == 0) ? reinterpret_cast<uint32_t *>(A.o_action)
                  : (k == 1) ? reinterpret_cast<uint32_t *>(A.o_value)
                  : (k == 2) ? reinterpret_cast<uint32_t *>(A.o_log_prob)
                  : (k == 3) ? reinterpret_cast<uint32_t *>(A.o_adv) : reinterpret_cast<uint32_t *>(A.o_tgt);
    dst[b] = src[row];
  }
}

__device__ __forceinline__ void relu_bwd_tiles4_block(float *dh, const float *h, int64_t rows, int64_t cols, int64_t ld,
                                                      float *partials, int act, const int bx, const int by) {
  __shared__ float4 part[4][64];
  const int cg = (int)(threadIdx.x & 63u), rg = (int)(threadIdx.x >> 6);
  const int64_t col = ((int64_t)bx * 64 + cg) * 4, r0 = (int64_t)by * 16 + rg;
  const bool cv = col < cols;
  float4 d[4], hv[4];
  const int64_t cc = cv ? col : cols - 4;
#pragma unroll
  for (int k = 0; k < 4; k++) {
    const int64_t r = r0 + 4 * k, rc = (r < rows) ? r : rows - 1;
    d[k] = *reinterpret_cast<const float4 *>(dh + rc * ld + cc);
  }
  if (h != nullptr) {
#pragma unroll
    for (int k = 0; k < 4; k++) {
      const int64_t r = r0 + 4 * k, rc = (r < rows) ? r : rows - 1;
      hv[k] = *reinterpret_cast<const float4 *>(h + rc * ld + cc);
    }
  } else {
#pragma unroll
    for (int k = 0; k < 4; k++) hv[k] = make_float4(1.f, 1.f, 1.f, 1.f);
  }
  float4 s = make_float4(0.f, 0.f, 0.f, 0.f);
#pragma unroll
  for (int k = 0; k < 4; k++) {
    const int64_t r = r0 + 4 * k;
    const bool v = cv && r < rows;
    const float4 z = (act == 0 || h == nullptr)
        ? make_float4((v && hv[k].x > 0.f) ? d[k].x : 0.f, (v && hv[k].y > 0.f) ? d[k].y : 0.f,
                      (v && hv[k].z > 0.f) ? d[k].z : 0.f, (v && hv[k].w > 0.f) ? d[k].w : 0.f)
        : make_float4(v ? d[k].x * (1.f - hv[k].x * hv[k].x) : 0.f, v ? d[k].y * (1.f - hv[k].y * hv[k].y) : 0.f,
                      v ? d[k].z * (1.f - hv[k].z * hv[k].z) : 0.f, v ? d[k].w * (1.f - hv[k].w * hv[k].w) : 0.f);
    if (h != nullptr && cv && r < rows) *reinterpret_cast<float4 *>(dh + r * ld + col) = z;
    s.x += z.x; s.y += z.y; s.z += z.z; s.w += z.w;
  }
  part[rg][cg] = s;
  __syncthreads();
  if (rg == 0 && cv) {
    const float4 a = part[0][cg], b = part[1][cg], c = part[2][cg], e = part[3][cg];
    *reinterpret_cast<float4 *>(partials + (int64_t)by * cols + col) =
        make_float4((a.x + b.x) + (c.x + e.x), (a.y + b.y) + (c.y + e.y), (a.z + b.z) + (c.z + e.z), (a.w + b.w) + (c.w + e.w));
  }
}

__global__ __launch_bounds__(256) void k_relu_bwd_tiles4(float *dh, const float *h, int64_t rows, int64_t cols, int64_t ld,
                                                          float *partials, int act = 0) {
  relu_bwd_tiles4_block(dh, h, rows, cols, ld, partials, act, (int)blockIdx.x, (int)blockIdx.y);
}

constexpr int BIAS_MAX_SEGS = 16;
struct BiasSegs {
  int n;
  int64_t tiles[BIAS_MAX_SEGS];
  const float *partials[BIAS_MAX_SEGS];
  int64_t cols[BIAS_MAX_SEGS];
  float *db[BIAS_MAX_SEGS];
  const int32_t *row_index;
  int first_row_seg;
};

__device__ __forceinline__ float bias_finalize_block(const BiasSegs &S, const int seg, const int bx, float (*part)[64]) {
  const int c = (int)(threadIdx.x & 63u), g = (int)(threadIdx.x >> 6);
  const int64_t col = (int64_t)bx * 64 + c, cols = S.cols[seg];
  const float *p = S.partials[seg];
  float s = 0.0f;
  if (col < cols) {
    const int64_t nt = S.tiles[seg];
    for (int64_t t0 = g; t0 < nt; t0 += 64) {
      float v[16];
#pragma unroll
      for (int u = 0; u < 16; u++) v[u] = p[((t0 + 4 * u < nt) ? t0 + 4 * u : t0) * cols + col];
#pragma unroll
      for (int u = 0; u < 16; u++) s += (t0 + 4 * u < nt) ? v[u] : 0.0f;
    }
  }
  part[g][c] = s;
  __syncthreads();
  float v = 0.0f;
  if (g == 0 && col < cols) {
    v = (part[0][c] + part[1][c]) + (part[2][c] + part[3][c]);
    float *db = S.db[seg];
    if (S.row_index != nullptr && seg >= S.first_row_seg) db += (int64_t)(*S.row_index) * cols;
    db[col] = v;
  }
  return v;
}

__global__ __launch_bounds__(256) void k_bias_finalize(BiasSegs S) {
  __shared__ float part[4][64];
  (void)bias_finalize_block(S, (int)blockIdx.y, (int)blockIdx.x, part);
}

constexpr int ADAM_BLOCKS = 1024, ADAM_THREADS = 256;

struct FinBlocks { int off[BIAS_MAX_SEGS + 1]; };

__global__ __launch_bounds__(ADAM_THREADS) void k_adam_norm_fin(const float *g, int64_t n, float gscale, float *partials, float *step,
                                                                int32_t *mb_index, BiasSegs S, int64_t tail_lo, FinBlocks FB) {
  static_assert(ADAM_THREADS == 256, "the finalize blocks are 4 x 64 threads");
  __shared__ float red[ADAM_THREADS / 64];
  __shared__ float part[4][64];
  if ((int)blockIdx.x >= ADAM_BLOCKS) {
    const int e = (int)blockIdx.x - ADAM_BLOCKS;
    int seg = 0;
    while (seg + 1 < S.n && e >= FB.off[seg + 1]) seg++;
    const int bx = e - FB.off[seg];
    float v = bias_finalize_block(S, seg, bx, part) * gscale;
    v = wave_sum_f(v * v);
    if (threadIdx.x == 0) partials[blockIdx.x] = v;
    return;
  }
  const int64_t n4 = n >> 2, t4 = tail_lo >> 2;
  const int64_t chunk = (n4 + ADAM_BLOCKS - 1) / ADAM_BLOCKS;
  int64_t lo = (int64_t)blockIdx.x * chunk, hi = (lo + chunk < n4) ? lo + chunk : n4;
  hi = (hi < t4) ? hi : t4;
  float s = 0.0f;
  for (int64_t i = lo + threadIdx.x; i < hi; i += ADAM_THREADS) {
    float4 x = reinterpret_cast<const float4 *>(g)[i];
    x.x *= gscale; x.y *= gscale; x.z *= gscale; x.w *= gscale;
    s += (x.x * x.x + x.y * x.y) + (x.z * x.z + x.w * x.w);
  }
  s = wave_sum_f(s);
  if ((threadIdx.x & 63u) == 0) red[threadIdx.x >> 6] = s;
  __syncthreads();
  if (threadIdx.x == 0) {
    partials[blockIdx.x] = (red[0] + red[1]) + (red[2] + red[3]);
    if (blockIdx.x == 0) {
      *step += 1.0f;
      if (mb_index) *mb_index += 1;
    }
  }
}

#include "adam_role.hpp"

__global__ __launch_bounds__(ADAM_THREADS) void k_adam_apply(AdamRange R, int nb, const GatherArgs *gather) {
  __shared__ float red[8];
  const int b = (int)blockIdx.x;
  if (b >= nb) {
    const GatherArgs A = *gather;
    if ((int64_t)(*A.mb_index) >= A.nsteps) return;
    const int64_t row = ((int64_t)b - nb) * 2 + (threadIdx.x >> 7);
    if (row < A.B) mb_gather_row(A, row, (int)(threadIdx.x & 127u));
    return;
  }
  adam_range_block(R, b, nb, red);
}

constexpr int SHARD_MAX_BUCKETS = 12;
constexpr int64_t SHARD_PER4 = 1024;
struct ShardGeom {
  int nb, world, J;
  int64_t off4[SHARD_MAX_BUCKETS], len4[SHARD_MAX_BUCKETS];
  int blk[SHARD_MAX_BUCKETS + 1];
};

__global__ __launch_bounds__(ADAM_THREADS) void k_shard_norm(const float *g, ShardGeom G, int rank_lo, float gscale, float *partials,
                                                             float *step, int32_t *mb_index) {
  __shared__ float red[ADAM_THREADS / 64];
  const int e = (int)blockIdx.x, j = e % G.J, rb = e / G.J, b = rb % G.nb, r = rank_lo + rb / G.nb;
  const int64_t len = G.len4[b], chunk = (len + G.J - 1) / G.J;
  const int64_t base = G.off4[b] + (int64_t)r * len;
  const int64_t lo = base + (int64_t)j * chunk, hi = (lo + chunk < base + len) ? lo + chunk : base + len;
  float s = 0.0f;
  for (int64_t i = lo + threadIdx.x; i < hi; i += ADAM_THREADS) {
    float4 x = reinterpret_cast<const float4 *>(g)[i];
    x.x *= gscale; x.y *= gscale; x.z *= gscale; x.w *= gscale;
    s += (x.x * x.x + x.y * x.y) + (x.z * x.z + x.w * x.w);
  }
  s = wave_sum_f(s);
  if ((threadIdx.x & 63u) == 0) red[threadIdx.x >> 6] = s;
  __syncthreads();
  if (threadIdx.x == 0) {
    partials[((int64_t)r * G.nb + b) * G.J + j] = (red[0] + red[1]) + (red[2] + red[3]);
    if (e == 0) {
      *step += 1.0f;
      if (mb_index) *mb_index += 1;
    }
  }
}

__global__ __launch_bounds__(ADAM_THREADS) void k_shard_apply(AdamRange R, ShardGeom G, int rank_lo, int sweep, const GatherArgs *gather) {
  __shared__ float red[8];
  const int e = (int)blockIdx.x;
  if (e >= sweep) {
    const GatherArgs A = *gather;
    if ((int64_t)(*A.mb_index) >= A.nsteps) return;
    const int64_t row = ((int64_t)e - sweep) * 2 + (threadIdx.x >> 7);
    if (row < A.B) mb_gather_row(A, row, (int)(threadIdx.x & 127u));
    return;
  }
  const int per_rank = G.blk[G.nb], r = rank_lo + e / per_rank, q = e % per_rank;
  int b = 0;
  while (b + 1 < G.nb && q >= G.blk[b + 1]) b++;
  R.lo4 = G.off4[b] + (int64_t)r * G.len4[b];
  R.hi4 = R.lo4 + G.len4[b];
  if (e != 0) R.norm_out = nullptr;
  adam_range_block(R, q - G.blk[b], G.blk[b + 1] - G.blk[b], red);
}
```

brl_amd/fused_update.py:

```python
from __future__ import annotations

import torch
import torch.distributed as dist

from ._capture import quiet_gc
from .roll_out import Transition


_CAPTURE_GROUP = {}


def _capture_group():
    key = dist.get_world_size(), dist.get_rank()
    if key not in _CAPTURE_GROUP:
        g = dist.new_group(backend="nccl")
        try:
            dev = torch.device("cuda", torch.cuda.current_device())
            g._get_backend(dev).eager_connect_single_device(dev)
        except Exception:
            pass
        _CAPTURE_GROUP[key] = g
    return _CAPTURE_GROUP[key]


class _DistCollectives:

    def __init__(self):
        self.rank, self.world = dist.get_rank(), dist.get_world_size()
        self.capturable = dist.get_backend() == "nccl"
        self.capture_group = _capture_group() if self.capturable else None

    def _group(self):
        return self.capture_group if (self.capturable and torch.cuda.is_current_stream_capturing()) else None

    def all_reduce(self, t, async_op):
        return dist.all_reduce(t, op=dist.ReduceOp.SUM, group=self._group(), async_op=async_op)

    def reduce_scatter(self, out, inp, async_op):
        return dist.reduce_scatter_tensor(out, inp, op=dist.ReduceOp.SUM, group=self._group(), async_op=async_op)

    def all_gather(self, out, inp, async_op):
        return dist.all_gather_into_tensor(out, inp, group=self._group(), async_op=async_op)

    def agree(self, ok: bool, device) -> bool:
        t = torch.tensor([1 if ok else 0], dtype=torch.int32, device=device if self.capturable else "cpu")
        dist.all_reduce(t, op=dist.ReduceOp.MIN)
        return bool(int(t.item()))


class FusedStep:

    def __init__(self, config, params, opt, mbs: int, device, world: int = 1, log_capacity: int = 0, collective=None):
        from . import _capi
        self.cfg, self.params, self.opt, self.mbs, self.dev = config, params, opt, int(mbs), device
        self.lib, self.capi = _capi.lib(), _capi
        self.world = int(world)
        from .dist import distributed
        multi = self.world > 1 or bool(config.get("force_collectives", False)) or (collective is None and distributed())
        self.multi = multi
        self.allreduce_mode = str(config.get("grad_allreduce", "flat")) if multi else "none"
        if self.allreduce_mode not in ("none", "flat", "sharded"):
            raise ValueError("config['grad_allreduce'] must be 'sharded' or 'flat'")
        self.coll = collective if collective is not None else (_DistCollectives() if multi else None)
        self.rank = int(getattr(self.coll, "rank", 0)) if multi else 0
        err = None
        self._saved = None
        try:
            self._setup(log_capacity)
        except Exception as e:
            err = e
            self._restore()
        self._agree(err, "allocation / first launches")
        self._capture_all()

    def _restore(self):
        if self._saved is not None:
            with torch.no_grad():
                for t, q in zip((self.P, self.M, self.V, self.step, self.mb_index), self._saved):
                    t.copy_(q)
            self._saved = None

    def _setup(self, log_capacity):
        config, params, opt, device, multi = self.cfg, self.params, self.opt, self.dev, self.multi
        _capi = self.capi
        if config.get("tuned_gemm", True):
            from . import tuned
            tuned.enable()
        f = self._f = lambda *shape: torch.zeros(shape, dtype=torch.float32, device=device)
        B = self.mbs
        self.act = 0 if params.act is torch.relu else 1
        self.ill_coef = float(config.get("illegal_action_l2norm_coef", 0.0) or 0.0)
        plist, sizes, offs, lens, n = self._layout()
        assert len(plist) == len(list(params.parameters()))
        self.n = n
        if multi:
            g = _capi.ShardGeom()
            g.nbuckets, g.world = len(offs), self.world
            g.nsub = max(1, 1024 // (self.world * len(offs)))
            for b, (o, ln) in enumerate(zip(offs, lens)):
                g.off[b], g.len[b] = o, ln
            self.geom, self.bucket_off, self.bucket_len = g, offs, lens
            self.norm_partials = f(self.world * g.nbuckets * g.nsub)
        self.P, self.G, self.M, self.V = f(n), f(n), f(n), f(n)
        self.step = torch.zeros((), dtype=torch.float32, device=device)
        self.plist = plist
        off = 0
        views = {}
        with torch.no_grad():
            for q, k in zip(plist, sizes):
                sl = slice(off, off + k)
                self.P[sl].copy_(q.detach().reshape(-1))
                st = opt.state.get(q, {})
                if "exp_avg" in st:
                    self.M[sl].copy_(st["exp_avg"].reshape(-1))
                    self.V[sl].copy_(st["exp_avg_sq"].reshape(-1))
                q.data = self.P[sl].view(q.shape)
                q.grad = self.G[sl].view(q.shape)
                st_step = st.get("step")
                opt.state[q] = {"step": st_step.to(device=device, dtype=torch.float32).reshape(()) if torch.is_tensor(st_step)
                                else torch.zeros((), dtype=torch.float32, device=device),
                                "exp_avg": self.M[sl].view(q.shape), "exp_avg_sq": self.V[sl].view(q.shape)}
                views[q] = sl
                off += k
        self.views = views
        self.x0 = f(B, 480)
        self.mask = torch.zeros((B, 38), dtype=torch.uint8, device=device)
        self.mask[:, 0] = 1
        self.action = torch.zeros(B, dtype=torch.int32, device=device)
        self.old_v, self.old_lp, self.adv, self.tgt = f(B), f(B), f(B), f(B)
        self.lgroups = (B + 3) // 4
        self.partials = f(self.lgroups, 8)
        self.out = f(8)
        self._log_cap = max(int(config.get("update_log_capacity", 4096)), int(log_capacity))
        self.log = f(self._log_cap, 8)
        self.stat_sums = f(self._log_cap, 8)
        self.gram_sums = f(self._log_cap, 38 * 38)
        self.norm = f(1)
        self.mb_index = torch.zeros(1, dtype=torch.int32, device=device)
        self._alloc()
        self.perm = None
        self.gargs = torch.zeros(256, dtype=torch.uint8, device=device)
        z = lambda shape, dt: torch.zeros(shape, dtype=dt, device=device)
        dmask = z((B, 38), torch.bool)
        dmask[:, 0] = True
        self._dummy = (Transition(z((B,), torch.bool), z((B,), torch.int32), f(B), f(B), f(B), z((B, 480), torch.bool), dmask),
                       f(B), f(B), (torch.arange(8 * B, device=device) % B).to(torch.int64))
        self._bind_gather(*self._dummy)
        d0 = opt.defaults
        self.lr, (self.b1, self.b2), self.eps = float(d0["lr"]), d0["betas"], float(d0["eps"])
        self.lr_dev = torch.full((1,), float(opt.param_groups[0]["lr"]), dtype=torch.float32, device=device)
        self.max_norm = float(config["max_grad_norm"]) if config.get("global_gradient_clipping", True) else 0.0
        self.program = self._build_program()
        want = config.get("collective_in_graph")
        self.in_graph = (not multi) or (bool(getattr(self.coll, "capturable", False)) if want is None else bool(want))
        self._works = {}
        self.moments_partial = False
        self.graph = self.graph_multi = self.segs = None
        self._saved = [t.clone() for t in (self.P, self.M, self.V, self.step, self.mb_index)]
        self._side = torch.cuda.Stream()
        self._side.wait_stream(torch.cuda.current_stream())
        with torch.cuda.stream(self._side), torch.no_grad():
            for _ in range(2):
                for item in self.program:
                    if item[0] == "k":
                        item[1]()
        torch.cuda.current_stream().wait_stream(self._side)
        torch.cuda.synchronize()

    def _capture_all(self):
        from ._capture import graph_kwargs
        config, multi, side = self.cfg, self.multi, self._side
        gkw = graph_kwargs()
        try:
            err = None
            scratch = None
            try:
                if multi and self.in_graph:
                    with quiet_gc():
                        scratch = self._capture_steps(1, gkw)
                else:
                    with torch.cuda.stream(side), torch.no_grad():
                        self._run_program(True)
                        self._drain()
                    torch.cuda.current_stream().wait_stream(side)
            except Exception as e:
                err = e
            self._agree(err, "first pass of the program's collectives")
            if scratch is not None:
                scratch.replay()
                torch.cuda.synchronize()
                del scratch
            try:
                with quiet_gc():
                    if self.in_graph:
                        self.graph = self._capture_steps(1, gkw)
                        self.graph_steps = int(config.get("update_graph_steps", 8))
                        if self.graph_steps > 1:
                            self.graph_multi = self._capture_steps(self.graph_steps, gkw)
                    else:
                        pool = torch.cuda.graph_pool_handle()
                        self.segs = []
                        run = []

                        def close():
                            if run:
                                fns = list(run)
                                g = torch.cuda.CUDAGraph()
                                with torch.cuda.graph(g, pool=pool, **gkw), torch.no_grad():
                                    for fn in fns:
                                        fn()
                                self.segs.append(("g", g))
                                run.clear()
                        for item in self.program:
                            if item[0] == "k":
                                run.append(item[1])
                            elif item[0] == "c":
                                close()
                                self.segs.append(item)
                        close()
            except Exception as e:
                err = e
            self._agree(err, "capture of the step")
        finally:
            self._restore()

    def _agree(self, err, what):
        agree = getattr(self.coll, "agree", None) if self.multi else None
        ok = err is None
        if agree is not None:
            ok = agree(ok, self.dev)
        if err is not None:
            raise err
        if not ok:
            raise RuntimeError(f"FusedStep: {what} failed on another rank: no rank builds the fused step")

    def _capture_steps(self, k, gkw):
        g = torch.cuda.CUDAGraph()
        with torch.cuda.graph(g, **gkw), torch.no_grad():
            for _ in range(k):
                self._run_program(True)
            self._drain()
        return g

    def _run_program(self, async_op):
        for item in self.program:
            if item[0] == "k":
                item[1]()
            elif item[0] == "c":
                w = item[2](async_op)
                if w is not None:
                    self._works[item[1]] = w
            else:
                w = self._works.pop(item[1], None)
                if w is not None:
                    w.wait()

    def _drain(self):
        for key in list(self._works):
            self._works.pop(key).wait()

    def _bind_gather(self, fl: Transition, adv, tgt, perm, first=True):
        import ctypes as C
        tp = self.capi.TransitionPtrs()
        for name in self.capi.TransitionPtrs._names:
            t = getattr(fl, name)
            setattr(tp, name, (t.view(torch.uint8) if t.dtype == torch.bool else t).data_ptr())
        self.capi.check(self.lib.brl_mb_gather_bind(self._di(), C.byref(tp), adv.data_ptr(), tgt.data_ptr(), perm.data_ptr(),
                                                    self.mb_index.data_ptr(), self.mbs, self.x0.data_ptr(), self.mask.data_ptr(),
                                                    self.action.data_ptr(), self.old_v.data_ptr(), self.old_lp.data_ptr(),
                                                    self.adv.data_ptr(), self.tgt.data_ptr(), perm.numel() // self.mbs,
                                                    self.gargs.data_ptr(), torch.cuda.current_stream().cuda_stream))
        if first:
            self.capi.check(self.lib.brl_mb_gather_dev(self._di(), self.gargs.data_ptr(), self.mbs, torch.cuda.current_stream().cuda_stream))

    def _di(self):
        return self.dev.index if self.dev.index is not None else torch.cuda.current_device()

    def _shard_norm(self, lo, hi):
        import ctypes as C
        self.capi.check(self.lib.brl_adam_shard_norm(self._di(), self.G.data_ptr(), C.byref(self.geom), lo, hi, 1.0 / self.world,
                                                     self.norm_partials.data_ptr(), self.step.data_ptr(), self.mb_index.data_ptr(),
                                                     torch.cuda.current_stream().cuda_stream))

    def _shard_apply(self, lo, hi):
        import ctypes as C
        self.capi.check(self.lib.brl_adam_shard_apply(
            self._di(), self.P.data_ptr(), self.G.data_ptr(), self.M.data_ptr(), self.V.data_ptr(), C.byref(self.geom), lo, hi,
            self.norm_partials.data_ptr(), self.step.data_ptr(), self.lr, self.lr_dev.data_ptr(), float(self.b1), float(self.b2),
            self.eps, self.max_norm, 1.0 / self.world, self.norm.data_ptr(), self.gargs.data_ptr(), self.mbs,
            torch.cuda.current_stream().cuda_stream))

    def begin_update(self, flat: Transition, adv_f, tgt_f, perms):
        steps = sum(p.numel() for p in perms) // self.mbs
        if steps > self._log_cap:
            raise RuntimeError("FusedStep: more minibatch steps per update than its log holds (log_capacity)")
        self._keep = (Transition(*[x.contiguous() for x in flat]), adv_f.contiguous(), tgt_f.contiguous())
        fl, adv_c, tgt_c = self._keep
        self._steps = steps
        with torch.no_grad():
            self._readopt()
            allp = torch.cat(perms)
            if self.perm is None or self.perm.numel() != allp.numel():
                self.perm = torch.empty_like(allp)
            self.perm.copy_(allp)
            self.mb_index.zero_()
            self.step.copy_(self.opt.state[self.plist[0]]["step"])
            self.lr_dev.fill_(float(self.opt.param_groups[0]["lr"]))
            self._bind_gather(fl, adv_c, tgt_c, self.perm)

    def _readopt(self):
        for q in self.plist:
            sl = self.views[q]
            if q.data.data_ptr() != self.P[sl].data_ptr():
                self.P[sl].copy_(q.data.reshape(-1))
                q.data = self.P[sl].view(q.shape)
            st = self.opt.state.get(q)
            if st is None or "exp_avg" not in st:
                self.M[sl].zero_(); self.V[sl].zero_()
                self.opt.state[q] = {"step": torch.zeros((), dtype=torch.float32, device=self.dev),
                                     "exp_avg": self.M[sl].view(q.shape), "exp_avg_sq": self.V[sl].view(q.shape)}
                continue
            if st["exp_avg"].data_ptr() != self.M[sl].data_ptr():
                self.M[sl].copy_(st["exp_avg"].reshape(-1))
                self.V[sl].copy_(st["exp_avg_sq"].reshape(-1))
                st["exp_avg"], st["exp_avg_sq"] = self.M[sl].view(q.shape), self.V[sl].view(q.shape)
            if not torch.is_tensor(st["step"]) or st["step"].device != self.P.device:
                st["step"] = torch.as_tensor(float(st["step"]), dtype=torch.float32, device=self.dev).reshape(())

    def run_steps(self, n: int):
        if self.allreduce_mode == "sharded" and n > 0:
            self.moments_partial = True
        if self.in_graph:
            k = self.graph_steps if self.graph_multi is not None else 0
            while k and n >= k:
                self.graph_multi.replay()
                n -= k
            for _ in range(n):
                self.graph.replay()
            return
        for _ in range(n):
            for item in self.segs:
                if item[0] == "g":
                    item[1].replay()
                else:
                    w = item[2](False)
                    if w is not None:
                        w.wait()

    def gather_optimizer_state(self):
        if self.allreduce_mode != "sharded":
            return
        self.moments_partial = False
        r = self.rank
        for t in (self.M, self.V):
            for o, ln in zip(self.bucket_off, self.bucket_len):
                w = self.coll.all_gather(t[o:o + self.world * ln], t[o + r * ln:o + (r + 1) * ln], False)
                if w is not None:
                    w.wait()

    def end_update(self):
        with torch.no_grad():
            for q in self.plist:
                self.opt.state[q]["step"].copy_(self.step)
            self.capi.check(self.lib.brl_ppo_stats_rows(self._di(), self.stat_sums.data_ptr(), self.gram_sums.data_ptr(), self._steps,
                                                        self.mbs, float(self.cfg["vf_coef"]), float(self.cfg["ent_coef"]),
                                                        self.ill_coef, self.log.data_ptr(),
                                                        torch.cuda.current_stream().cuda_stream))
            self._bind_gather(*self._dummy, first=False)
        self._keep = None
        return self.log[:self._steps]


class FusedMinibatch(FusedStep):

    @staticmethod
    def supports(config, params) -> bool:
        return (bool(config.get("fused_update", True)) and str(getattr(params, "model", "")).startswith("DeepMind")
                and getattr(params, "act", None) in (torch.relu, torch.tanh)
                and params.body[0].weight.shape[0] % 256 == 0
                and next(params.parameters()).is_cuda and next(params.parameters()).dtype == torch.float32)

    def _layout(self):
        params, multi = self.params, self.multi
        body = list(params.body)
        nl = len(body)
        H = body[0].weight.shape[0]
        K = params.actor.weight.shape[0] + 1
        self.H, self.K, self.nl = H, K, nl
        plist = [lin.weight for lin in body[1:]] + [body[0].weight, params.actor.weight, params.critic.weight] \
            + [lin.bias for lin in body] + [params.actor.bias, params.critic.bias]
        sizes = [q.numel() for q in plist]
        hid = (nl - 1) * H * H
        tail = sum(sizes) - hid
        self.sharded_geom = multi and (H * H) % (4 * self.world) == 0
        if self.allreduce_mode == "sharded" and not self.sharded_geom:
            raise ValueError(f"grad_allreduce='sharded' needs hidden^2 divisible by 4 * world (hidden {H}, world {self.world}): use 'flat'")
        quantum = 4 * self.world if multi else 4
        tail_pad = (tail + quantum - 1) // quantum * quantum
        n = hid + tail_pad
        offs = lens = None
        if multi:
            if self.sharded_geom:
                offs = [l * H * H for l in range(nl - 1)] + [hid]
                lens = [H * H // self.world] * (nl - 1) + [tail_pad // self.world]
            else:
                n = (sum(sizes) + quantum - 1) // quantum * quantum
                offs, lens = [0], [n // self.world]
        self._hid = hid
        return plist, sizes, offs, lens, n

    def _alloc(self):
        import ctypes as C
        params, views, f, B, config = self.params, self.views, self._f, self.mbs, self.cfg
        body = list(params.body)
        nl, H, K, hid = self.nl, self.H, self.K, self._hid
        self.W = [lin.weight for lin in body]
        self.b = [lin.bias for lin in body]
        self.GW = [self.G[views[lin.weight]].view(lin.weight.shape) for lin in body]
        self.Gb = [self.G[views[lin.bias]] for lin in body]
        wa = views[params.actor.weight]
        self.Wh = self.P[wa.start:wa.start + K * H].view(K, H)
        self.GWh = self.G[wa.start:wa.start + K * H].view(K, H)
        ba = views[params.actor.bias]
        self.bh = self.P[ba.start:ba.start + K]
        self.Gbh = self.G[ba.start:ba.start + K]
        self.hs = f(nl, B, H)
        self.dzs = f(nl, B, H)
        self.h = [self.hs[l] for l in range(nl)]
        self.GW_hidden = self.G[:hid].view(nl - 1, H, H) if nl > 1 else None
        self.dheads = f(B, K)
        self.heads = f(B, K) if self.ill_coef else None
        self.head_ksplit = max(1, min(4, H // 256))
        self.head_parts = f(self.head_ksplit, B, K)
        self.vec = f(40) if self.ill_coef else None
        groups = (B + 15) // 16
        self.gram_partials = f(self.lgroups, 38 * 38)
        self.scratch = f(8192)
        self.nsplit = (B + 63) // 64
        self.dwh_partials = f(self.nsplit, K * H)
        self.dbh_partials = f(self.nsplit, K)
        self.own_gemm = bool(config.get("own_gemm", True)) and B % 4 == 0 and H % 4 == 0 and nl > 1
        self.own_fwd = self.own_gemm and bool(config.get("own_gemm_fwd", False))
        self.dw_x3 = (config.get("dw_gemm") or "bf16x3") == "bf16x3" and B % 32 == 0 and H % 4 == 0 and self.x0.shape[1] % 4 == 0 and nl <= 8
        if self.dw_x3:
            a_ = [self.dzs[l] for l in range(nl)]
            b_ = [self.x0] + [self.hs[l] for l in range(nl - 1)]
            c_ = [self.GW[l] for l in range(nl)]
            i64, vp = C.c_int64 * nl, C.c_void_p * nl
            self._gdw = (vp(*[t_.data_ptr() for t_ in a_]), i64(*[t_.stride(0) for t_ in a_]), vp(*[t_.data_ptr() for t_ in b_]),
                         i64(*[t_.stride(0) for t_ in b_]), vp(*[t_.data_ptr() for t_ in c_]), i64(*[t_.stride(0) for t_ in c_]),
                         i64(*[t_.shape[0] for t_ in c_]), i64(*[t_.shape[1] for t_ in c_]), i64(*([B] * nl)))
        self.dw_deferred = nl > 1
        groups64 = (B + 63) // 64
        self.tile_rows = [64 if (self.own_gemm and l < nl - 1) else 16 for l in range(nl)]
        self.tile_sums = [f(groups * H) for _ in body]
        nseg = nl + 2
        self._seg_scratch = (C.c_void_p * nseg)(*([self.dwh_partials.data_ptr()] + [t.data_ptr() for t in self.tile_sums]
                                                  + [self.dbh_partials.data_ptr()]))
        self._seg_cols = (C.c_int64 * nseg)(*([K * H] + [H] * nl + [K]))
        self._seg_tiles = (C.c_int64 * nseg)(*([self.nsplit] + [groups64 if r == 64 else groups for r in self.tile_rows] + [self.nsplit]))
        self._seg_db = (C.c_void_p * nseg)(*([self.GWh.data_ptr()] + [g.data_ptr() for g in self.Gb] + [self.Gbh.data_ptr()]))
        self._nseg = nseg

    def _build_program(self):
        nl = self.nl
        if self.allreduce_mode == "none":
            return [("k", self._step_single)]
        co, G, P = self.coll, self.G, self.P
        if self.allreduce_mode == "flat":
            return [("k", self._grads_chain),
                    ("c", "ar", lambda a: co.all_reduce(G, a)), ("w", "ar"),
                    ("k", lambda: (self._shard_norm(0, self.world), self._shard_apply(0, self.world)))]
        r = self.rank
        bucket = lambda t, b: t[self.bucket_off[b]:self.bucket_off[b] + self.world * self.bucket_len[b]]
        mine = lambda t, b: t[self.bucket_off[b] + r * self.bucket_len[b]:self.bucket_off[b] + (r + 1) * self.bucket_len[b]]
        tail = nl - 1
        np_ = self.norm_partials
        per = np_.numel() // self.world
        prog = [("w", "ag%d" % tail), ("k", lambda: self._forward(0))]
        for l in range(1, nl):
            prog += [("w", "ag%d" % (l - 1)), ("k", lambda l=l: self._forward(l))]
        prog += [("k", self._heads)]
        for l in range(nl - 1, 0, -1):
            prog += [("k", lambda l=l: self._dw(l)),
                     ("c", "rs%d" % (l - 1), lambda a, l=l: co.reduce_scatter(mine(G, l - 1), bucket(G, l - 1), a)),
                     ("k", lambda l=l: self._dz(l))]
        prog += [("k", lambda: (self._dw(0), self._seg_fin())),
                 ("c", "rs%d" % tail, lambda a: co.reduce_scatter(mine(G, tail), bucket(G, tail), a))]
        prog += [("w", "rs%d" % b) for b in range(nl)]
        prog += [("k", lambda: self._shard_norm(r, r + 1)),
                 ("c", "agn", lambda a: co.all_gather(np_, np_[r * per:(r + 1) * per], a)), ("w", "agn"),
                 ("k", lambda: self._shard_apply(r, r + 1))]
        for b in [tail] + list(range(nl - 1)):
            prog += [("c", "ag%d" % b, lambda a, b=b: co.all_gather(bucket(P, b), mine(P, b), a))]
        return prog

    def _step_single(self):
        for l in range(self.nl):
            self._forward(l)
        self._heads()
        self._backward_chain()
        self._fin_opt()

    def _grads_chain(self):
        for l in range(self.nl):
            self._forward(l)
        self._heads()
        if self.cfg.get("per_layer_dw", False):
            for l in range(self.nl - 1, 0, -1):
                self._dw(l)
                self._dz(l)
            self._dw(0)
        else:
            self._backward_chain()
        self._seg_fin()

    def _forward(self, l):
        x = self.x0 if l == 0 else self.h[l - 1]
        W, b = self.W[l], self.b[l]
        if self.own_fwd and l > 0:
            self.capi.check(self.lib.brl_mlp_gemm(self._di(), 0, 1, x.data_ptr(), x.stride(0), W.data_ptr(), W.stride(0),
                                                  self.h[l].data_ptr(), self.h[l].stride(0), self.mbs, W.shape[0], W.shape[1], self.act,
                                                  b.data_ptr(), None, 0, None, None, torch.cuda.current_stream().cuda_stream))
        elif self.act == 0:
            torch._addmm_activation(b, x, W.t(), use_gelu=False, out=self.h[l])
        else:
            torch.addmm(b, x, W.t(), out=self.h[l]).tanh_()

    def _heads(self):
        L, chk, B = self.lib, self.capi.check, self.mbs
        s = torch.cuda.current_stream().cuda_stream
        di, cfg = self._di(), self.cfg
        x = self.h[self.nl - 1]
        chk(L.brl_ppo_heads_loss_split(di, x.data_ptr(), x.stride(0), self.Wh.data_ptr(), self.bh.data_ptr(), self.H,
                                       self.mask.data_ptr(), self.action.data_ptr(), self.old_v.data_ptr(), self.old_lp.data_ptr(),
                                       self.adv.data_ptr(), self.tgt.data_ptr(), B, float(cfg["clip_eps"]), float(cfg["vf_coef"]),
                                       float(cfg["ent_coef"]), int(bool(cfg.get("actor_illegal_action_mask", True))),
                                       int(bool(cfg.get("value_clipping", True))), int(bool(cfg.get("reward_scaling", False))),
                                       self.heads.data_ptr() if self.ill_coef else None,
                                       self.dheads.data_ptr(), self.partials.data_ptr(), self.gram_partials.data_ptr(),
                                       self.head_parts.data_ptr(), self.head_ksplit, s))
        if self.ill_coef:
            chk(L.brl_ppo_stats_gram(di, self.partials.data_ptr(), self.lgroups, B, self.gram_partials.data_ptr(), self.lgroups,
                                     float(cfg["vf_coef"]), float(cfg["ent_coef"]), self.ill_coef, self.out.data_ptr(), None,
                                     self.vec.data_ptr(), s))
            chk(L.brl_ppo_illegal_grad(di, self.heads.data_ptr(), self.mask.data_ptr(), self.vec.data_ptr(), self.ill_coef, B,
                                       self.dheads.data_ptr(), s))
        top = self.nl - 1
        chk(L.brl_ppo_heads_bwd(di, self.dheads.data_ptr(), x.data_ptr(), x.stride(0), self.Wh.data_ptr(), B, self.H, self.act,
                                self.nsplit, None if self.dw_deferred else self.dwh_partials.data_ptr(),
                                None if self.dw_deferred else self.dbh_partials.data_ptr(),
                                self.dzs[top].data_ptr(), self.tile_sums[top].data_ptr(), self.partials.data_ptr(),
                                self.gram_partials.data_ptr(), self.lgroups, self.mb_index.data_ptr(), self.stat_sums.data_ptr(),
                                self.gram_sums.data_ptr(), s))

    def _dz(self, l):
        L, chk, B, H = self.lib, self.capi.check, self.mbs, self.H
        s = torch.cuda.current_stream().cuda_stream
        di = self._di()
        first = l == self.nl - 1 and self.dw_deferred
        top = self.h[self.nl - 1]
        dz, out, W, gate, ts = self.dzs[l], self.dzs[l - 1], self.W[l], self.h[l - 1], self.tile_sums[l - 1]
        heads_dw = (self.dheads.data_ptr(), top.data_ptr(), top.stride(0), B, H, self.nsplit, self.dwh_partials.data_ptr(),
                    self.dbh_partials.data_ptr(), self.partials.data_ptr(), self.gram_partials.data_ptr(), self.lgroups,
                    self.mb_index.data_ptr(), self.stat_sums.data_ptr(), self.gram_sums.data_ptr(), s)
        if self.own_gemm:
            if first:
                chk(L.brl_mlp_gemm_dh_heads_dw(di, dz.data_ptr(), H, W.data_ptr(), W.stride(0), out.data_ptr(), H, B, W.shape[1], W.shape[0],
                                               self.act, gate.data_ptr(), H, ts.data_ptr(), *heads_dw))
            else:
                chk(L.brl_mlp_gemm(di, 1, 2, dz.data_ptr(), H, W.data_ptr(), W.stride(0), out.data_ptr(), H, B, W.shape[1], W.shape[0],
                                   self.act, None, gate.data_ptr(), H, ts.data_ptr(), None, s))
            return
        torch.mm(dz, W, out=out)
        if first:
            chk(L.brl_act_bwd_colsum_heads_dw(di, out.data_ptr(), gate.data_ptr(), B, H, H, self.act, ts.data_ptr(), *heads_dw))
        else:
            chk(L.brl_act_bwd_colsum(di, out.data_ptr(), gate.data_ptr(), B, H, H, self.act, ts.data_ptr(), s))

    def _dw(self, l):
        src = self.x0 if l == 0 else self.h[l - 1]
        if self.own_gemm and l > 0:
            dz, GW = self.dzs[l], self.GW[l]
            self.capi.check(self.lib.brl_mlp_gemm(self._di(), 2, 0, dz.data_ptr(), dz.stride(0), src.data_ptr(), src.stride(0),
                                                  GW.data_ptr(), GW.stride(0), GW.shape[0], GW.shape[1], self.mbs, self.act, None, None, 0,
                                                  None, None, torch.cuda.current_stream().cuda_stream))
        else:
            torch.mm(self.dzs[l].t(), src, out=self.GW[l])

    def _backward_chain(self):
        nl = self.nl
        for l in range(nl - 1, 0, -1):
            self._dz(l)
        if self.dw_x3:
            self.capi.check(self.lib.brl_mlp_gemm_x3_group(self._di(), 2, nl, *self._gdw, torch.cuda.current_stream().cuda_stream))
            return
        if nl > 1:
            torch.bmm(self.dzs[1:].transpose(1, 2), self.hs[:nl - 1], out=self.GW_hidden)
        torch.mm(self.dzs[0].t(), self.x0, out=self.GW[0])

    def _seg_fin(self):
        self.capi.check(self.lib.brl_bias_finalize_ex(self._di(), self._nseg, self._seg_scratch, self._seg_cols, self._seg_tiles,
                                                      self._seg_db, torch.cuda.current_stream().cuda_stream))

    def _fin_opt(self):
        self.capi.check(self.lib.brl_adam_clip_fin_gather(
            self._di(), self.P.data_ptr(), self.G.data_ptr(), self.M.data_ptr(), self.V.data_ptr(), self.n, self.step.data_ptr(), self.lr,
            self.lr_dev.data_ptr(), float(self.b1), float(self.b2), self.eps, self.max_norm, self.scratch.data_ptr(),
            self.scratch.numel(), self.mb_index.data_ptr(), self.norm.data_ptr(), self.gargs.data_ptr(), self.mbs, self._nseg,
            self._seg_scratch, self._seg_cols, self._seg_tiles, self._seg_db, torch.cuda.current_stream().cuda_stream))



class FusedFair(FusedStep):

    SQUARE = (1, 2, 3, 4, 5, 7, 8, 9, 10)
    INPUT = {1: "h0", 2: "h1", 3: "g1", 4: "h3", 5: "x2", 7: "h6", 8: "h7", 9: "g3", 10: "h9"}

    @staticmethod
    def supports(config, params) -> bool:
        return (bool(config.get("fused_update", True)) and getattr(params, "model", "") == "FAIR"
                and getattr(params, "act", None) in (torch.relu, torch.tanh)
                and next(params.parameters()).is_cuda and next(params.parameters()).dtype == torch.float32)

    def _layout(self):
        p = self.params
        L = list(p.l)
        plist = [L[l].weight for l in self.SQUARE] + [L[0].weight, L[6].weight, p.actor.weight, p.critic.weight] \
            + [lin.bias for lin in L] + [p.actor.bias, p.critic.bias]
        sizes = [q.numel() for q in plist]
        quantum = 4 * self.world if self.multi else 4
        n = (sum(sizes) + quantum - 1) // quantum * quantum
        return plist, sizes, ([0] if self.multi else None), ([n // self.world] if self.multi else None), n

    def _alloc(self):
        import ctypes as C
        p, f, B, views = self.params, self._f, self.mbs, self.views
        L = list(p.l)
        H = self.H = L[0].weight.shape[0]
        nsq = len(self.SQUARE)
        self.W, self.b = [lin.weight for lin in L], [lin.bias for lin in L]
        self.GW = [self.G[views[lin.weight]].view(lin.weight.shape) for lin in L]
        self.Gb = [self.G[views[lin.bias]] for lin in L]
        gv = lambda q: self.G[views[q]].view(q.shape)
        self.Wa, self.wc, self.ba, self.bc = p.actor.weight, p.critic.weight, p.actor.bias, p.critic.bias
        self.GWa, self.Gwc, self.Gba, self.Gbc = gv(p.actor.weight), gv(p.critic.weight), gv(p.actor.bias), gv(p.critic.bias)
        self.GW_square = self.G[:nsq * H * H].view(nsq, H, H)
        self.W6a, self.W6b = L[6].weight[:, :H], L[6].weight[:, H:]
        self.GW6 = self.GW[6]
        self.cat6 = f(B, H + 480)
        self.inp = f(nsq, B, H)
        self.dzs = f(nsq, B, H)
        self.t = {name: self.inp[i] for i, name in enumerate(self.INPUT[l] for l in self.SQUARE)}
        for name in "z0 h2 x1 h4 z6 h8 x3 h10 x4 dc dx dz0 dz6".split():
            self.t[name] = f(B, H)
        self.t["z5"] = self.cat6[:, :H]
        self.dz = {l: self.dzs[i] for i, l in enumerate(self.SQUARE)}
        self.dz[0], self.dz[6] = self.t["dz0"], self.t["dz6"]
        self.logits, self.value = f(B, 38), f(B)
        self.dlogits, self.dvalue, self.illp, self.gram = f(B, 38), f(B), f(B, 38), f(1, 38 * 38)
        self.ones_row = torch.ones((1, B), dtype=torch.float32, device=self.dev)
        self.unit_gate = torch.ones((B, H), dtype=torch.float32, device=self.dev) if self.act == 0 else f(B, H)
        self.own_gemm = bool(self.cfg.get("own_gemm", True)) and B % 4 == 0 and H % 4 == 0
        self.from_gemm = (1, 3, 7, 9) if self.own_gemm else ()
        t16, t64 = (B + 15) // 16, (B + 63) // 64
        self.tiles = [f((t64 if l in self.from_gemm else t16), H) for l in range(11)]
        self._seg_scratch = (C.c_void_p * 11)(*[t.data_ptr() for t in self.tiles])
        self._seg_cols = (C.c_int64 * 11)(*([H] * 11))
        self._seg_tiles = (C.c_int64 * 11)(*[t.shape[0] for t in self.tiles])
        self._seg_db = (C.c_void_p * 11)(*[g.data_ptr() for g in self.Gb])
        if not self.multi:
            g = self.capi.ShardGeom()
            g.nbuckets, g.world, g.nsub = 1, 1, 1024
            g.off[0], g.len[0] = 0, self.n
            self.geom, self.norm_partials = g, f(1024)
        self.chain = bool(self.cfg.get("fair_chain", True)) and B % 16 == 0 and H == 200 and self.x0.shape[1] == 480 and not self.ill_coef
        if self.ill_coef:
            self.heads39, self.dheads39, self.vec = f(B, 39), f(B, 39), f(40)
        if self.chain:
            nwg = B // 16
            assert p.critic.weight.data_ptr() == p.actor.weight.data_ptr() + 38 * H * 4 \
                and p.critic.bias.data_ptr() == p.actor.bias.data_ptr() + 38 * 4
            sw, sb = views[p.actor.weight], views[p.critic.bias]
            self.GWh = self.G[sw.start:sw.start + 39 * H].view(39, H)
            self.gates, self.dheads = f(4, B, H), f(B, 40)
            self.ctiles = f(11 * nwg * H + nwg * 39)
            self.cpartials, self.cgram = f(nwg, 8), f(nwg, 38 * 38)
            net, wk = self.capi.FairNet(), self.capi.FairWork()
            for l, lin in enumerate(L):
                net.w[l], net.b[l] = lin.weight.data_ptr(), lin.bias.data_ptr()
            net.head_w, net.head_b = p.actor.weight.data_ptr(), p.actor.bias.data_ptr()
            for name, t_ in (("inp", self.inp), ("dzs", self.dzs), ("gates", self.gates), ("cat6", self.cat6), ("x4", self.t["x4"]),
                             ("dz0", self.dz[0]), ("dz6", self.dz[6]), ("dheads", self.dheads), ("tiles", self.ctiles),
                             ("partials", self.cpartials), ("gram_partials", self.cgram)):
                setattr(wk, name, t_.data_ptr())
            self._net, self._work = net, wk
            parts = [self.ctiles.data_ptr() + 4 * l * nwg * H for l in range(12)] + [self.cpartials.data_ptr(), self.cgram.data_ptr()]
            outs = [g_.data_ptr() for g_ in self.Gb] + [self.G[views[p.actor.bias].start:].data_ptr(), self.stat_sums.data_ptr(),
                                                         self.gram_sums.data_ptr()]
            cols = [H] * 11 + [39, 8, 38 * 38]
            self._cseg = ((C.c_void_p * 14)(*parts), (C.c_int64 * 14)(*cols), (C.c_int64 * 14)(*([nwg] * 14)), (C.c_void_p * 14)(*outs))
            self.group_dw = self.own_gemm and bool(self.cfg.get("fair_group_dw", True))
            a_ = [self.dzs[i] for i in range(nsq)] + [self.dz[6], self.dz[0], self.dheads]
            b_ = [self.inp[i] for i in range(nsq)] + [self.cat6, self.x0, self.t["x4"]]
            c_ = [self.GW_square[i] for i in range(nsq)] + [self.GW6, self.GW[0], self.GWh]
            i64, vp = C.c_int64 * 12, C.c_void_p * 12
            self._gdw = (vp(*[t_.data_ptr() for t_ in a_]), i64(*[t_.stride(0) for t_ in a_]), vp(*[t_.data_ptr() for t_ in b_]),
                         i64(*[t_.stride(0) for t_ in b_]), vp(*[t_.data_ptr() for t_ in c_]), i64(*[t_.stride(0) for t_ in c_]),
                         i64(*[t_.shape[0] for t_ in c_]), i64(*[t_.shape[1] for t_ in c_]), i64(*([B] * 12)))

    def _build_program(self):
        if self.allreduce_mode == "none":
            return [("k", lambda: (self._grads(), self._shard_norm(0, 1), self._shard_apply(0, 1)))]
        co, G, P, r, W = self.coll, self.G, self.P, self.rank, self.world
        if self.allreduce_mode == "flat":
            return [("k", self._grads), ("c", "ar", lambda a: co.all_reduce(G, a)), ("w", "ar"),
                    ("k", lambda: (self._shard_norm(0, W), self._shard_apply(0, W)))]
        ln = self.bucket_len[0]
        np_ = self.norm_partials
        per = np_.numel() // W
        return [("w", "ag"), ("k", self._grads),
                ("c", "rs", lambda a: co.reduce_scatter(G[r * ln:(r + 1) * ln], G, a)), ("w", "rs"),
                ("k", lambda: self._shard_norm(r, r + 1)),
                ("c", "agn", lambda a: co.all_gather(np_, np_[r * per:(r + 1) * per], a)), ("w", "agn"),
                ("k", lambda: self._shard_apply(r, r + 1)),
                ("c", "ag", lambda a: co.all_gather(P, P[r * ln:(r + 1) * ln], a))]

    def _a(self, x, out):
        return torch.clamp_min(x, 0.0, out=out) if self.act == 0 else torch.tanh(x, out=out)

    def _lin(self, x, l, out, act):
        if act and self.act == 0:
            return torch._addmm_activation(self.b[l], x, self.W[l].t(), use_gelu=False, out=out)
        torch.addmm(self.b[l], x, self.W[l].t(), out=out)
        return out.tanh_() if act else out

    def _colsum(self, l, gate):
        dz = self.dz[l]
        self.capi.check(self.lib.brl_act_bwd_colsum(self._di(), dz.data_ptr(), gate.data_ptr(), self.mbs, self.H, dz.stride(0), self.act,
                                                    self.tiles[l].data_ptr(), torch.cuda.current_stream().cuda_stream))

    def _dx(self, l, gate, out, bias_of=None):
        dz, W = self.dz[l], self.W[l]
        if self.own_gemm:
            cs = self.tiles[bias_of] if bias_of is not None else None
            self.capi.check(self.lib.brl_mlp_gemm(self._di(), 1, 2, dz.data_ptr(), dz.stride(0), W.data_ptr(), W.stride(0), out.data_ptr(),
                                                  out.stride(0), self.mbs, W.shape[1], W.shape[0], self.act, None, gate.data_ptr(),
                                                  gate.stride(0), cs.data_ptr() if cs is not None else None, None,
                                                  torch.cuda.current_stream().cuda_stream))
            return
        torch.mm(dz, W, out=out)
        if bias_of is not None:
            self._colsum(bias_of, gate)
        elif self.act == 0:
            torch.mul(out, (gate > 0), out=out)
        else:
            torch.addcmul(out, out * gate, gate, value=-1.0, out=out)

    def _grads_chain(self):
        cfg, B = self.cfg, self.mbs
        s = torch.cuda.current_stream().cuda_stream
        chk, L, di = self.capi.check, self.lib, self._di()
        chk(L.brl_fair_chain(di, self._net, self.x0.data_ptr(), self.mask.data_ptr(), self.action.data_ptr(), self.old_v.data_ptr(),
                             self.old_lp.data_ptr(), self.adv.data_ptr(), self.tgt.data_ptr(), B, float(cfg["clip_eps"]),
                             float(cfg["vf_coef"]), float(cfg["ent_coef"]), int(bool(cfg.get("actor_illegal_action_mask", True))),
                             int(bool(cfg.get("value_clipping", True))), int(bool(cfg.get("reward_scaling", False))), self.act,
                             self._work, s))
        if self.group_dw:
            chk(L.brl_mlp_gemm_group(di, 2, 12, *self._gdw, s))
        else:
            torch.bmm(self.dzs.transpose(1, 2), self.inp, out=self.GW_square)
            torch.mm(self.dz[6].t(), self.cat6, out=self.GW6)
            torch.mm(self.dz[0].t(), self.x0, out=self.GW[0])
            torch.mm(self.dheads[:, :39].t(), self.t["x4"], out=self.GWh)
        chk(L.brl_bias_finalize_rows(di, 14, *self._cseg, 12, self.mb_index.data_ptr(), s))

    def _grads(self):
        if self.chain:
            return self._grads_chain()
        t, cfg, B, dz = self.t, self.cfg, self.mbs, self.dz
        a = self._a
        x0 = self.x0
        self._lin(x0, 0, t["z0"], False)
        a(t["z0"], t["h0"])
        self._lin(t["h0"], 1, t["h1"], True)
        self._lin(t["h1"], 2, t["h2"], True)
        torch.add(t["h2"], t["z0"], out=t["x1"])
        a(t["x1"], t["g1"])
        self._lin(t["g1"], 3, t["h3"], True)
        self._lin(t["h3"], 4, t["h4"], True)
        torch.add(t["h4"], t["x1"], out=t["x2"])
        self._lin(t["x2"], 5, t["z5"], False)
        self.cat6[:, self.H:].copy_(x0)
        self._lin(self.cat6, 6, t["z6"], False)
        a(t["z6"], t["h6"])
        self._lin(t["h6"], 7, t["h7"], True)
        self._lin(t["h7"], 8, t["h8"], True)
        torch.add(t["h8"], t["z6"], out=t["x3"])
        a(t["x3"], t["g3"])
        self._lin(t["g3"], 9, t["h9"], True)
        self._lin(t["h9"], 10, t["h10"], True)
        torch.add(t["h10"], t["x3"], out=t["x4"])
        torch.addmm(self.ba, t["x4"], self.Wa.t(), out=self.logits)
        torch.addmv(self.bc, t["x4"], self.wc[0], out=self.value)
        adv = self.adv
        if cfg.get("reward_scaling", False):
            adv = (adv - adv.mean()) / (adv.std(unbiased=False) + 1e-8)
        s = torch.cuda.current_stream().cuda_stream
        chk, L, di = self.capi.check, self.lib, self._di()
        chk(L.brl_ppo_loss(di, self.logits.data_ptr(), 38, self.value.data_ptr(), self.mask.data_ptr(), self.action.data_ptr(),
                           self.old_v.data_ptr(), self.old_lp.data_ptr(), adv.data_ptr(), self.tgt.data_ptr(), B, float(cfg["clip_eps"]),
                           float(cfg["vf_coef"]), float(cfg["ent_coef"]), int(bool(cfg.get("actor_illegal_action_mask", True))),
                           int(bool(cfg.get("value_clipping", True))), self.dlogits.data_ptr(), self.dvalue.data_ptr(),
                           self.partials.data_ptr(), self.illp.data_ptr(), s))
        row = self.mb_index.to(torch.int64)
        self.stat_sums.index_copy_(0, row, torch.mm(self.ones_row[:, :self.lgroups], self.partials))
        gram = torch.mm(self.illp.t(), self.illp)
        self.gram_sums.index_copy_(0, row, gram.view(1, -1))
        if self.ill_coef:
            chk(L.brl_ppo_stats_gram(di, self.partials.data_ptr(), self.lgroups, B, gram.data_ptr(), 1, float(cfg["vf_coef"]),
                                     float(cfg["ent_coef"]), self.ill_coef, self.out.data_ptr(), None, self.vec.data_ptr(), s))
            self.heads39[:, :38].copy_(self.logits)
            self.heads39[:, 38].copy_(self.value)
            self.dheads39[:, :38].copy_(self.dlogits)
            chk(L.brl_ppo_illegal_grad(di, self.heads39.data_ptr(), self.mask.data_ptr(), self.vec.data_ptr(), self.ill_coef, B,
                                       self.dheads39.data_ptr(), s))
            self.dlogits.copy_(self.dheads39[:, :38])
        dx = t["dx"]
        torch.mm(self.dlogits, self.Wa, out=dx)
        dx.addr_(self.dvalue, self.wc[0])
        torch.mm(self.dlogits.t(), t["x4"], out=self.GWa)
        torch.mm(self.dvalue[None, :], t["x4"], out=self.Gwc)
        torch.mm(self.ones_row, self.dlogits, out=self.Gba.view(1, -1))
        torch.sum(self.dvalue, 0, keepdim=True, out=self.Gbc)

        def block(lb, la, hb, ha, g):
            dz[lb].copy_(dx)
            self._colsum(lb, hb)
            self._dx(lb, ha, dz[la], bias_of=la)
            self._dx(la, g, t["dc"])
            dx.add_(t["dc"])

        block(10, 9, t["h10"], t["h9"], t["g3"])
        block(8, 7, t["h8"], t["h7"], t["h6"])
        dz[6].copy_(dx)
        self._colsum(6, self.unit_gate)
        torch.mm(dz[6], self.W6a, out=dz[5])
        self._colsum(5, self.unit_gate)
        torch.mm(dz[5], self.W[5], out=dx)
        block(4, 3, t["h4"], t["h3"], t["g1"])
        block(2, 1, t["h2"], t["h1"], t["h0"])
        dz[0].copy_(dx)
        self._colsum(0, self.unit_gate)
        torch.bmm(self.dzs.transpose(1, 2), self.inp, out=self.GW_square)
        torch.mm(dz[6].t(), self.cat6, out=self.GW6)
        torch.mm(dz[0].t(), x0, out=self.GW[0])
        chk(L.brl_bias_finalize_ex(di, 11, self._seg_scratch, self._seg_cols, self._seg_tiles, self._seg_db, s))
```

Baseline: 10.65 billion.

## Fold gradient-norm partials and bias finalize into grouped dW GEMM; fuse heads loss+bwd

The grouped x3 weight-gradient GEMM now accumulates per-wave squared-norm partials in its epilogue. Extra workgroups in the same launch finalize the bias-gradient segments and their norm contributions, so the separate norm/finalize pass over the gradient vector is dropped and Adam consumes the precomputed partials. A new opt-in kernel path fuses the PPO heads loss with the heads backward. Costs are a larger launch grid, tighter layout preconditions on gradient buffers, and a default-on path that only applies when allreduce is disabled.

```diff
diff --git a/brl_amd/_capi.py b/brl_amd/_capi.py
--- a/brl_amd/_capi.py
+++ b/brl_amd/_capi.py
@@ -151,6 +151,7 @@
                                      _vp, _vp, _vp, _vp, i64, _vp, _vp, _vp, _vp],
     }
     sigs.update(sl_signatures())
+    sigs.update(step_fused_signatures())
     for name, args in sigs.items():
         fn = getattr(L, name)
         fn.argtypes = args
@@ -177,6 +178,17 @@
     }
 
 
+def step_fused_signatures() -> dict:
+    i64, i32, f32 = C.c_int64, C.c_int, C.c_float
+    return {
+        "brl_ppo_heads_loss_bwd": [i32, _vp, i64, _vp, _vp, i64, _vp, _vp, _vp, _vp, _vp, _vp, i64, f32, f32, f32, i32, i32, i32, _vp,
+                                   _vp, _vp, _vp, _vp, i32, i32, _vp, _vp, _vp],
+        "brl_mlp_gemm_x3_group_fin": [i32, i32, i32, _vp, _vp, _vp, _vp, _vp, _vp, _vp, _vp, _vp, _vp, i64, i64, i32, _vp, _vp, _vp,
+                                      _vp, f32, _vp, i64, _vp, _vp, _vp, _vp],
+        "brl_adam_apply_gather": [i32, _vp, _vp, _vp, _vp, i64, _vp, f32, _vp, f32, f32, f32, f32, _vp, i64, _vp, _vp, i64, _vp],
+    }
+
+
 def check(rc: int) -> None:
     if rc != 0:
         raise BrlError(f"libbrl_hip error {rc}: {lib().brl_last_error().decode()}")
diff --git a/brl_amd/csrc/brl_mlp_gemm_x3.hip b/brl_amd/csrc/brl_mlp_gemm_x3.hip
--- a/brl_amd/csrc/brl_mlp_gemm_x3.hip
+++ b/brl_amd/csrc/brl_mlp_gemm_x3.hip
@@ -2,6 +2,7 @@
 #include <stdint.h>
 
 #include "abi_common.hpp"
+#include "../../include/brl_step_fused.h"
 #include "mlp_gemm_x3.hpp"
 #include "mlp_linear_x3p.hpp"
 
@@ -69,13 +70,11 @@
   return BRL_OK;
 }
 
-extern "C" int brl_mlp_gemm_x3_group(int device, int layout, int count, const float *const *a, const int64_t *lda, const float *const *b,
-                                     const int64_t *ldb, float *const *c, const int64_t *ldc, const int64_t *m, const int64_t *n,
-                                     const int64_t *k, void *stream) {
+static int x3_group_args(int layout, int count, const float *const *a, const int64_t *lda, const float *const *b, const int64_t *ldb,
+                         float *const *c, const int64_t *ldc, const int64_t *m, const int64_t *n, const int64_t *k, mgs::GroupArgs &GA) {
   NEED(count >= 1 && count <= mgs::GROUP_MAX && a && lda && b && ldb && c && ldc && m && n && k, "count (1..8) / NULL array");
   NEED(layout >= BRL_GEMM_NT && layout <= BRL_GEMM_TN, "layout (BRL_GEMM_NT / _NN / _TN)");
   const bool akc = layout != BRL_GEMM_TN, bkc = layout == BRL_GEMM_NT;
-  mgs::GroupArgs GA{};
   GA.n = count;
   for (int i = 0; i < count; i++) {
     NEED(a[i] && b[i] && c[i] && m[i] > 0 && n[i] > 0 && k[i] > 0, "a / b / c / m / n / k");
@@ -93,12 +92,71 @@
     X.splitk = 1;
     GA.first[i + 1] = GA.first[i] + (int)x3_tiles(m[i], n[i]);
   }
+  return BRL_OK;
+}
+
+extern "C" int brl_mlp_gemm_x3_group(int device, int layout, int count, const float *const *a, const int64_t *lda, const float *const *b,
+                                     const int64_t *ldb, float *const *c, const int64_t *ldc, const int64_t *m, const int64_t *n,
+                                     const int64_t *k, void *stream) {
+  mgs::GroupArgs GA{};
+  const int rc = x3_group_args(layout, count, a, lda, b, ldb, c, ldc, m, n, k, GA);
+  if (rc != BRL_OK) return rc;
   HIP_TRY(hipSetDevice(device));
   hipStream_t s = (hipStream_t)stream;
   const unsigned blocks = (unsigned)GA.first[count];
   if (layout == BRL_GEMM_NT) hipLaunchKernelGGL((mgs::k_gemm_x3s_group<true, true>), dim3(blocks), dim3(mgs::THREADS), 0, s, GA);
   else if (layout == BRL_GEMM_NN) hipLaunchKernelGGL((mgs::k_gemm_x3s_group<true, false>), dim3(blocks), dim3(mgs::THREADS), 0, s, GA);
   else hipLaunchKernelGGL((mgs::k_gemm_x3s_group<false, false>), dim3(blocks), dim3(mgs::THREADS), 0, s, GA);
+  HIP_TRY(hipGetLastError());
+  return BRL_OK;
+}
+
+extern "C" int brl_mlp_gemm_x3_group_fin(int device, int layout, int count, const float *const *a, const int64_t *lda, const float *const *b,
+                                         const int64_t *ldb, float *const *c, const int64_t *ldc, const int64_t *m, const int64_t *n,
+                                         const int64_t *k, const float *g, int64_t n_g, int64_t tail_lo, int nseg, const float *const *partials,
+                                         const int64_t *cols, const int64_t *tiles, float *const *out, float gscale, float *sq,
+                                         int64_t sq_len, float *step, int32_t *mb_index, int64_t *nsq, void *stream) {
+  mgs::GroupArgs GA{};
+  const int rc = x3_group_args(layout, count, a, lda, b, ldb, c, ldc, m, n, k, GA);
+  if (rc != BRL_OK) return rc;
+  NEED(g && sq && step && nsq && tail_lo > 0 && tail_lo % 4 == 0, "g / sq / step / nsq / tail_lo (a positive multiple of 4)");
+  const float *ends[mgs::GROUP_MAX];
+  int64_t total = 0;
+  for (int i = 0; i < count; i++) {
+    NEED(ldc[i] == n[i] && c[i] >= g && c[i] + m[i] * n[i] <= g + tail_lo, "the products' outputs must be dense and lie in g[0, tail_lo)");
+    total += m[i] * n[i];
+    ends[i] = c[i] + m[i] * n[i];
+  }
+  NEED(total == tail_lo, "the products' outputs must cover g[0, tail_lo)");
+  for (int i = 0; i < count; i++)
+    for (int j = 0; j < count; j++) NEED(i == j || ends[i] <= c[j] || ends[j] <= c[i], "the products' outputs overlap");
+  NEED(nseg >= 1 && nseg <= BIAS_MAX_SEGS && partials && cols && tiles && out, "nseg / partials / cols / tiles / out");
+  mgs::NormFin &F = GA.nf;
+  int64_t covered = 0;
+  for (int i = 0; i < nseg; i++) {
+    NEED(partials[i] && out[i] && cols[i] > 0 && tiles[i] > 0, "segment");
+    NEED(out[i] >= g + tail_lo && out[i] + cols[i] <= g + n_g, "the finalised segments lie in g[tail_lo, n)");
+    covered += cols[i];
+    F.S.tiles[i] = tiles[i]; F.S.partials[i] = partials[i]; F.S.cols[i] = cols[i]; F.S.db[i] = out[i];
+    F.FB.off[i + 1] = F.FB.off[i] + (int)((cols[i] + 63) / 64);
+  }
+  F.S.n = nseg;
+  NEED(covered <= n_g - tail_lo && n_g - tail_lo - covered < 4, "the finalised segments must tile g[tail_lo, n)");
+  HIP_TRY(hipSetDevice(device));
+  int cus = 0;
+  HIP_TRY(hipDeviceGetAttribute(&cus, hipDeviceAttributeMultiprocessorCount, device));
+  const int ntiles = GA.first[count];
+  int nx = cus - ntiles;
+  nx = nx < 8 ? 8 : (nx > 64 ? 64 : nx);
+  const int64_t need = 8 * (int64_t)ntiles + 2 * nx;
+  NEED(sq_len >= need, "sq too small: 8 x tiles + 2 x the finalize workgroups");
+  F.sq = sq; F.gscale = gscale; F.nx = nx; F.step = step; F.mb_index = mb_index;
+  *nsq = need;
+  hipStream_t s = (hipStream_t)stream;
+  const unsigned blocks = (unsigned)(ntiles + nx);
+  if (layout == BRL_GEMM_NT) hipLaunchKernelGGL((mgs::k_gemm_x3s_group<true, true, true>), dim3(blocks), dim3(mgs::THREADS), 0, s, GA);
+  else if (layout == BRL_GEMM_NN) hipLaunchKernelGGL((mgs::k_gemm_x3s_group<true, false, true>), dim3(blocks), dim3(mgs::THREADS), 0, s, GA);
+  else hipLaunchKernelGGL((mgs::k_gemm_x3s_group<false, false, true>), dim3(blocks), dim3(mgs::THREADS), 0, s, GA);
   HIP_TRY(hipGetLastError());
   return BRL_OK;
 }
diff --git a/brl_amd/csrc/brl_ppo.hip b/brl_amd/csrc/brl_ppo.hip
--- a/brl_amd/csrc/brl_ppo.hip
+++ b/brl_amd/csrc/brl_ppo.hip
@@ -6,6 +6,7 @@
 #include <string.h>
 
 #include "abi_common.hpp"
+#include "../../include/brl_step_fused.h"
 
 static inline unsigned thread_grid(int64_t n, int bs) { return (unsigned)((n + bs - 1) / bs); }
 
@@ -64,7 +65,8 @@
   return S;
 }
 __device__ __forceinline__ void ppo_loss_sample(const PpoArgs &A, const PpoSampleIn &S, int64_t b, bool valid, int lane, float lg, float v,
-                                                float g, float (&st)[5], float &illp_lane) {
+                                                float g, float (&st)[5], float &illp_lane, bool store = true, float *dz_lane = nullptr,
+                                                float *dv_out = nullptr) {
   const bool in = lane < BRL_NUM_ACTIONS;
   const bool legal = S.legal;
   const float invB = 1.0f / (float)A.B;
@@ -106,11 +108,13 @@
   const bool live = A.masked ? legal : in;
   const float dz = (live ? dlp * (onehot - psel) : 0.0f) - A.ent_coef * invB * dH;
   illp_lane = legal ? 0.0f : p2;
-  if (valid && in) {
+  if (dz_lane) *dz_lane = dz;
+  if (dv_out) *dv_out = A.vf_coef * dv * invB;
+  if (store && valid && in) {
     A.dlogits[b * A.dls + lane] = dz;
     if (A.illp) A.illp[b * BRL_NUM_ACTIONS + lane] = illp_lane;
   }
-  if (lane == 0 && valid) A.dvalue[b * A.dvs] = A.vf_coef * dv * invB;
+  if (store && lane == 0 && valid) A.dvalue[b * A.dvs] = A.vf_coef * dv * invB;
   st[0] = valid ? vl : 0.0f;
   st[1] = valid ? la : 0.0f;
   st[2] = valid ? H : 0.0f;
@@ -415,6 +419,35 @@
   return BRL_OK;
 }
 
+extern "C" int brl_ppo_heads_loss_bwd(int device, const float *h, int64_t ldh, const float *head_w, const float *head_b, int64_t hidden,
+                                      const uint8_t *mask, const int32_t *action, const float *old_value, const float *old_log_prob,
+                                      const float *gae, const float *targets, int64_t batch, float clip_eps, float vf_coef, float ent_coef,
+                                      int masked, int value_clipping, int reward_scaling, float *heads_out, float *dheads, float *partials,
+                                      float *gram_partials, float *head_parts, int ksplit, int act, float *dh, float *tile_sums, void *stream) {
+  NEED(batch > 0 && hidden > 0 && hidden % 256 == 0 && ldh >= hidden && ldh % 4 == 0, "batch / hidden (a multiple of 256) / ldh");
+  NEED(h && head_w && head_b && mask && action && old_value && old_log_prob && gae && targets, "NULL input array");
+  NEED(dheads && partials && head_parts && dh && tile_sums, "NULL output array");
+  NEED(ksplit >= 1 && ksplit <= 8, "ksplit (1..8)");
+  NEED(act == 0 || act == 1, "act (0 ReLU, 1 tanh)");
+  HIP_TRY(hipSetDevice(device));
+  constexpr int64_t HS = BRL_NUM_ACTIONS + 1;
+  HeadsProductArgs G{};
+  G.h = h; G.ldh = ldh; G.Wh = head_w; G.H = (int)hidden; G.B = batch; G.ksplit = ksplit; G.parts = head_parts; G.part_stride = batch * HS;
+  hipLaunchKernelGGL(k_heads_product, dim3((unsigned)((batch + 15) / 16), (unsigned)ksplit), dim3(HD_WAVES * 64), 0, (hipStream_t)stream, G);
+  HeadsLossBwdArgs A{};
+  HeadsLossArgs &L = A.L;
+  L.h = h; L.ldh = ldh; L.Wh = head_w; L.bh = head_b; L.H = (int)hidden;
+  L.P = PpoArgs{nullptr, HS, nullptr, mask, action, old_value, old_log_prob, gae, targets, batch, clip_eps, vf_coef,
+                ent_coef, masked, value_clipping, dheads, dheads + BRL_NUM_ACTIONS, partials, nullptr, HS, HS, HS};
+  L.heads_out = heads_out; L.gram_partials = gram_partials; L.reward_scaling = reward_scaling;
+  L.parts = head_parts; L.nparts = ksplit; L.part_stride = batch * HS;
+  A.act = act; A.dh = dh; A.tile_sums = tile_sums;
+  const unsigned ctiles = (unsigned)((hidden + HLB_COLS - 1) / HLB_COLS);
+  hipLaunchKernelGGL(k_heads_loss_bwd, dim3(ctiles, (unsigned)((batch + HB_ROWS - 1) / HB_ROWS)), dim3(HLB_THREADS), 0, (hipStream_t)stream, A);
+  HIP_TRY(hipGetLastError());
+  return BRL_OK;
+}
+
 extern "C" int brl_ppo_heads_bwd(int device, const float *dheads, const float *h, int64_t ldh, const float *head_w, int64_t batch,
                                  int64_t hidden, int act, int nsplit, float *dw_partials, float *db_partials, float *dh,
                                  float *tile_sums, const float *loss_partials, const float *gram_partials, int64_t ngroups,
@@ -512,6 +545,23 @@
   return BRL_OK;
 }
 
+extern "C" int brl_adam_apply_gather(int device, float *p, const float *g, float *m, float *v, int64_t n, const float *step, float lr,
+                                     const float *lr_dev, float beta1, float beta2, float eps, float max_norm, const float *partials,
+                                     int64_t npartials, float *norm_out, const void *gather_args, int64_t mbs, void *stream) {
+  NEED(p && g && m && v && step && partials && n > 0 && n % 4 == 0, "p / g / m / v / step / partials / n (a multiple of 4)");
+  NEED(npartials > 0 && npartials < (1 << 30), "npartials");
+  NEED(!gather_args || mbs > 0, "gather_args needs the minibatch size");
+  HIP_TRY(hipSetDevice(device));
+  const unsigned extra = gather_args ? (unsigned)((mbs + 1) / 2) : 0u;
+  AdamRange R{};
+  R.p = p; R.g = g; R.m = m; R.v = v; R.lo4 = 0; R.hi4 = n >> 2; R.partials = partials; R.npartials = (int)npartials; R.step = step;
+  R.lr_dev = lr_dev; R.lr = lr; R.b1 = beta1; R.b2 = beta2; R.eps = eps; R.max_norm = max_norm; R.gscale = 1.0f; R.norm_out = norm_out;
+  hipLaunchKernelGGL(k_adam_apply, dim3((unsigned)ADAM_BLOCKS + extra), dim3(ADAM_THREADS), 0, (hipStream_t)stream, R, ADAM_BLOCKS,
+                     (const GatherArgs *)gather_args);
+  HIP_TRY(hipGetLastError());
+  return BRL_OK;
+}
+
 static int shard_geom(const brl_shard_geom *geom, int rank_lo, int rank_hi, ShardGeom *out) {
   NEED(geom && geom->nbuckets >= 1 && geom->nbuckets <= SHARD_MAX_BUCKETS && geom->world >= 1 && geom->nsub >= 1, "geometry");
   NEED(rank_lo >= 0 && rank_lo < rank_hi && rank_hi <= geom->world, "rank range");
diff --git a/brl_amd/csrc/mlp_gemm_x3.hpp b/brl_amd/csrc/mlp_gemm_x3.hpp
--- a/brl_amd/csrc/mlp_gemm_x3.hpp
+++ b/brl_amd/csrc/mlp_gemm_x3.hpp
@@ -1,6 +1,7 @@
 #pragma once
 
 #include "mlp_gemm.hpp"
+#include "norm_fin_role.hpp"
 
 namespace mgs {
 
@@ -38,7 +39,7 @@
 };
 
 template <bool A_KC, bool B_KC, int EPI>
-__device__ __forceinline__ void gemm_tile(const Args &X, unsigned char *lds, int bid, int nblk) {
+__device__ __forceinline__ void gemm_tile(const Args &X, unsigned char *lds, int bid, int nblk, float *sq = nullptr, float gscale = 1.0f) {
   const mg::Args &G = X.g;
   constexpr int NP = 4;
   const int tid = (int)threadIdx.x, lane = tid & 63, w = __builtin_amdgcn_readfirstlane(tid >> 6);
@@ -293,6 +294,7 @@
       }
   }
   const bool relu = G.act == 0;
+  float sqs = 0.0f;
 #pragma unroll
   for (int g = 0; g < 4; g++) {
     const int n = n0 + 32 * wn + 8 * g + 4 * hh, nc = n < G.N ? n : 0;
@@ -326,6 +328,13 @@
         for (int i = 0; i < 4; i++) cs[i] += ok ? o[i] : 0.0f;
       }
       if (ok) *reinterpret_cast<f32x4 *>(G.C + (int64_t)em * G.ldc + n) = o;
+      if (EPI == mg::EPI_NONE && sq != nullptr && ok) {
+#pragma unroll
+        for (int i = 0; i < 4; i++) {
+          const float x = o[i] * gscale;
+          sqs += x * x;
+        }
+      }
     }
     if (EPI == mg::EPI_GATE_COLSUM && G.colsum != nullptr) {
 #pragma unroll
@@ -336,6 +345,11 @@
       }
       if (r32 == 0 && n < G.N && 2 * tm + wm < (G.M + 63) / 64) *reinterpret_cast<f32x4 *>(G.colsum + (int64_t)(2 * tm + wm) * G.N + n) = cs;
     }
+  }
+  if (EPI == mg::EPI_NONE && sq != nullptr) {
+#pragma unroll
+    for (int o = 1; o < 64; o <<= 1) sqs += __shfl_xor(sqs, o, 64);
+    if (lane == 0) sq[w] = sqs;
   }
   MG_STAMP(3);
 }
@@ -347,18 +361,34 @@
 }
 
 constexpr int GROUP_MAX = 8;
+struct NormFin {
+  float *sq;
+  float gscale;
+  int nx;
+  BiasSegs S;
+  FinBlocks FB;
+  float *step;
+  int32_t *mb_index;
+};
 struct GroupArgs {
   int n;
   int first[GROUP_MAX + 1];
   Args x[GROUP_MAX];
+  NormFin nf;
 };
-template <bool A_KC, bool B_KC>
+template <bool A_KC, bool B_KC, bool NORM = false>
 __global__ __launch_bounds__(THREADS) void k_gemm_x3s_group(GroupArgs GA) {
   __shared__ __attribute__((aligned(16))) unsigned char lds[LDS_BYTES];
   const int b = (int)blockIdx.x;
+  if (NORM && b >= GA.first[GA.n]) {
+    norm_fin_block512(GA.nf.S, GA.nf.FB, b - GA.first[GA.n], GA.nf.nx, GA.nf.gscale, GA.nf.sq + 8 * GA.first[GA.n], GA.nf.step,
+                      GA.nf.mb_index, reinterpret_cast<float *>(lds));
+    return;
+  }
   int p = 0;
   while (p + 1 < GA.n && b >= GA.first[p + 1]) p++;
-  gemm_tile<A_KC, B_KC, mg::EPI_NONE>(GA.x[p], lds, b - GA.first[p], GA.first[p + 1] - GA.first[p]);
+  gemm_tile<A_KC, B_KC, mg::EPI_NONE>(GA.x[p], lds, b - GA.first[p], GA.first[p + 1] - GA.first[p], NORM ? GA.nf.sq + 8 * b : nullptr,
+                                      GA.nf.gscale);
 }
 
 static inline int pick_splitk(int64_t m, int64_t n, int64_t k) {
diff --git a/brl_amd/csrc/norm_fin_role.hpp b/brl_amd/csrc/norm_fin_role.hpp
--- /dev/null
+++ b/brl_amd/csrc/norm_fin_role.hpp
@@ -0,0 +1,67 @@
+#pragma once
+#include <stdint.h>
+
+constexpr int BIAS_MAX_SEGS = 16;
+struct BiasSegs {
+  int n;
+  int64_t tiles[BIAS_MAX_SEGS];
+  const float *partials[BIAS_MAX_SEGS];
+  int64_t cols[BIAS_MAX_SEGS];
+  float *db[BIAS_MAX_SEGS];
+  const int32_t *row_index;
+  int first_row_seg;
+};
+struct FinBlocks { int off[BIAS_MAX_SEGS + 1]; };
+
+__device__ __forceinline__ float bias_col_partial(const BiasSegs &S, const int seg, const int64_t col, const int g) {
+  const int64_t cols = S.cols[seg];
+  const float *p = S.partials[seg];
+  float s = 0.0f;
+  if (col < cols) {
+    const int64_t nt = S.tiles[seg];
+    for (int64_t t0 = g; t0 < nt; t0 += 64) {
+      float v[16];
+#pragma unroll
+      for (int u = 0; u < 16; u++) v[u] = p[((t0 + 4 * u < nt) ? t0 + 4 * u : t0) * cols + col];
+#pragma unroll
+      for (int u = 0; u < 16; u++) s += (t0 + 4 * u < nt) ? v[u] : 0.0f;
+    }
+  }
+  return s;
+}
+
+__device__ __forceinline__ float fin_wave_sum(float v) {
+#pragma unroll
+  for (int o = 1; o < 64; o <<= 1) v += __shfl_xor(v, o, 64);
+  return v;
+}
+
+__device__ __forceinline__ void norm_fin_block512(const BiasSegs &S, const FinBlocks &FB, const int x, const int nx, const float gscale,
+                                                  float *sq, float *step, int32_t *mb_index, float *part) {
+  const int tid = (int)threadIdx.x, hf = tid >> 8, g = (tid >> 6) & 3, c = tid & 63;
+  if (x == 0 && tid == 0) {
+    *step += 1.0f;
+    if (mb_index) *mb_index += 1;
+  }
+  const int nchunks = FB.off[S.n];
+  float acc = 0.0f;
+  for (int e0 = x; e0 < nchunks; e0 += 2 * nx) {
+    const int e = e0 + hf * nx;
+    int seg = 0;
+    while (seg + 1 < S.n && e >= FB.off[seg + 1]) seg++;
+    const int64_t col = (int64_t)(e - FB.off[seg]) * 64 + c;
+    const bool live = e < nchunks;
+    part[tid] = live ? bias_col_partial(S, seg, col, g) : 0.0f;
+    __syncthreads();
+    if (g == 0 && live && col < S.cols[seg]) {
+      const float *q = part + 256 * hf;
+      const float v = (q[c] + q[64 + c]) + (q[128 + c] + q[192 + c]);
+      S.db[seg][col] = v;
+      const float vs = v * gscale;
+      acc += vs * vs;
+    }
+    __syncthreads();
+  }
+  acc = fin_wave_sum(acc);
+  if (g == 0 && c == 0) sq[2 * x + hf] = acc;
+}
diff --git a/brl_amd/csrc/ppo_heads.hpp b/brl_amd/csrc/ppo_heads.hpp
--- a/brl_amd/csrc/ppo_heads.hpp
+++ b/brl_amd/csrc/ppo_heads.hpp
@@ -252,6 +252,187 @@
     const float4 a = cs_s[0][c4], b = cs_s[1][c4], c = cs_s[2][c4], e = cs_s[3][c4];
     *reinterpret_cast<float4 *>(A.tile_sums + (int64_t)rt * A.H + col) =
         make_float4((a.x + b.x) + (c.x + e.x), (a.y + b.y) + (c.y + e.y), (a.z + b.z) + (c.z + e.z), (a.w + b.w) + (c.w + e.w));
+  }
+}
+
+constexpr int HLB_THREADS = 512, HLB_COLS = 256;
+struct HeadsLossBwdArgs {
+  HeadsLossArgs L;
+  int act;
+  float *dh;
+  float *tile_sums;
+};
+
+__global__ __launch_bounds__(HLB_THREADS) void k_heads_loss_bwd(HeadsLossBwdArgs A) {
+  static_assert(HLB_THREADS == HD_WAVES * 64 && HB_ROWS == 2 * HD_WAVES && HB_ROWS % HD_ROWS == 0, "two samples per wave");
+  __shared__ __attribute__((aligned(16))) float dh_s[HB_ROWS][HD_NOUT + 1];
+  __shared__ float illp_s[HB_ROWS][BRL_NUM_ACTIONS + 2];
+  __shared__ float part_s[HB_ROWS][8];
+  __shared__ float rs_red[HD_WAVES], rs_stat[2];
+  __shared__ float4 zs[HB_ROWS][HLB_COLS / 4];
+  const HeadsLossArgs &L = A.L;
+  const int tid = (int)threadIdx.x, lane = tid & 63, w = tid >> 6;
+  const int ct = (int)blockIdx.x, rt = (int)blockIdx.y;
+  const int64_t B = L.P.B, r0 = (int64_t)rt * HB_ROWS;
+  const bool lead = ct == 0;
+  const int c4 = lane, rg = w;
+  const int col = ct * HLB_COLS + 4 * c4;
+  float4 hv[2];
+#pragma unroll
+  for (int u = 0; u < 2; u++) {
+    const int64_t rw = r0 + rg + 8 * u;
+    hv[u] = *reinterpret_cast<const float4 *>(L.h + ((rw < B) ? rw : B - 1) * L.ldh + col);
+  }
+  static_assert(HD_NOUT == 39, "three batches of 13 head rows");
+  const float *wp = L.Wh + col;
+  float4 wv[13];
+#pragma unroll
+  for (int k = 0; k < 13; k++) wv[k] = *reinterpret_cast<const float4 *>(wp + (int64_t)k * L.H);
+
+  float adv_mean = 0.0f, adv_inv = 1.0f;
+  if (L.reward_scaling) {
+    float s = 0.0f;
+    for (int64_t i = tid; i < B; i += HD_WAVES * 64) s += L.P.gae[i];
+    s = wave_sum_f(s);
+    if (lane == 0) rs_red[w] = s;
+    __syncthreads();
+    if (tid == 0) {
+      float t = 0.0f;
+      for (int k = 0; k < HD_WAVES; k++) t += rs_red[k];
+      rs_stat[0] = t / (float)B;
+    }
+    __syncthreads();
+    adv_mean = rs_stat[0];
+    float q = 0.0f;
+    for (int64_t i = tid; i < B; i += HD_WAVES * 64) {
+      const float d = L.P.gae[i] - adv_mean;
+      q += d * d;
+    }
+    q = wave_sum_f(q);
+    __syncthreads();
+    if (lane == 0) rs_red[w] = q;
+    __syncthreads();
+    if (tid == 0) {
+      float t = 0.0f;
+      for (int k = 0; k < HD_WAVES; k++) t += rs_red[k];
+      rs_stat[1] = 1.0f / (sqrtf(t / (float)B) + 1e-8f);
+    }
+    __syncthreads();
+    adv_inv = rs_stat[1];
+  }
+
+  PpoSampleIn in[2];
+  float part[2][HD_MAX_PARTS];
+#pragma unroll
+  for (int j = 0; j < 2; j++) {
+    const int64_t b = r0 + 2 * w + j;
+    const bool valid = b < B;
+    in[j] = ppo_sample_load(L.P, b, valid, lane);
+#pragma unroll
+    for (int p = 0; p < HD_MAX_PARTS; p++)
+      part[j][p] = (valid && lane < HD_NOUT && p < L.nparts) ? L.parts[(int64_t)p * L.part_stride + b * HD_NOUT + lane] : 0.0f;
+  }
+  const float bias = (lane < HD_NOUT) ? L.bh[lane] : 0.0f;
+#pragma unroll
+  for (int j = 0; j < 2; j++) {
+    const int sl = 2 * w + j;
+    const int64_t b = r0 + sl;
+    const bool valid = b < B;
+    float hd = 0.0f;
+    if (lane < HD_NOUT) {
+      hd = bias;
+#pragma unroll
+      for (int p = 0; p < HD_MAX_PARTS; p++) hd += part[j][p];
+      if (lead && valid && L.heads_out) L.heads_out[b * HD_NOUT + lane] = hd;
+    }
+    const float v = __shfl(hd, BRL_NUM_ACTIONS, 64);
+    const float g = L.reward_scaling ? (in[j].gae - adv_mean) * adv_inv : in[j].gae;
+    float st[5], ill, dz, dv;
+    ppo_loss_sample(L.P, in[j], b, valid, lane, hd, v, g, st, ill, lead, &dz, &dv);
+    if (lane < BRL_NUM_ACTIONS) {
+      illp_s[sl][lane] = valid ? ill : 0.0f;
+      dh_s[sl][lane] = valid ? dz : 0.0f;
+    } else if (lane == BRL_NUM_ACTIONS) {
+      dh_s[sl][lane] = valid ? dv : 0.0f;
+    }
+    if (lane == 0) {
+#pragma unroll
+      for (int k = 0; k < 8; k++) part_s[sl][k] = (k < 5) ? st[k] : 0.0f;
+    }
+  }
+  __syncthreads();
+  if (lead) {
+    if (tid < 8 * (HB_ROWS / HD_ROWS)) {
+      const int q = tid >> 3, k = tid & 7;
+      if (r0 + HD_ROWS * q < B) {
+        float s = 0.0f;
+        for (int kk = 0; kk < HD_ROWS; kk++) s += part_s[HD_ROWS * q + kk][k];
+        L.P.partials[((int64_t)rt * (HB_ROWS / HD_ROWS) + q) * 8 + k] = s;
+      }
+    }
+    if (L.gram_partials != nullptr) {
+      for (int e = tid; e < (HB_ROWS / HD_ROWS) * HD_GRAM; e += HLB_THREADS) {
+        const int q = e / HD_GRAM, ee = e - q * HD_GRAM;
+        const int i = ee / BRL_NUM_ACTIONS, j = ee - i * BRL_NUM_ACTIONS;
+        if (r0 + HD_ROWS * q < B) {
+          float s = 0.0f;
+#pragma unroll
+          for (int kk = 0; kk < HD_ROWS; kk++) s += illp_s[HD_ROWS * q + kk][i] * illp_s[HD_ROWS * q + kk][j];
+          L.gram_partials[((int64_t)rt * (HB_ROWS / HD_ROWS) + q) * HD_GRAM + ee] = s;
+        }
+      }
+    }
+  }
+
+  float4 acc[2];
+#pragma unroll
+  for (int u = 0; u < 2; u++) acc[u] = make_float4(0.f, 0.f, 0.f, 0.f);
+#pragma unroll 1
+  for (int n0 = 0; n0 < HD_NOUT; n0 += 13) {
+    if (n0 > 0) {
+#pragma unroll
+      for (int k = 0; k < 13; k++) wv[k] = *reinterpret_cast<const float4 *>(wp + (int64_t)(n0 + k) * L.H);
+    }
+#pragma unroll
+    for (int k = 0; k < 13; k++) {
+#pragma unroll
+      for (int u = 0; u < 2; u++) {
+        const float d = dh_s[rg + 8 * u][n0 + k];
+        acc[u].x += d * wv[k].x; acc[u].y += d * wv[k].y; acc[u].z += d * wv[k].z; acc[u].w += d * wv[k].w;
+      }
+    }
+  }
+#pragma unroll
+  for (int u = 0; u < 2; u++) {
+    const int64_t rw = r0 + rg + 8 * u;
+    float4 z;
+    if (A.act == 0) {
+      z = make_float4(hv[u].x > 0.f ? acc[u].x : 0.f, hv[u].y > 0.f ? acc[u].y : 0.f, hv[u].z > 0.f ? acc[u].z : 0.f,
+                      hv[u].w > 0.f ? acc[u].w : 0.f);
+    } else {
+      z = make_float4(acc[u].x * (1.0f - hv[u].x * hv[u].x), acc[u].y * (1.0f - hv[u].y * hv[u].y),
+                      acc[u].z * (1.0f - hv[u].z * hv[u].z), acc[u].w * (1.0f - hv[u].w * hv[u].w));
+    }
+    if (rw < B) *reinterpret_cast<float4 *>(A.dh + rw * (int64_t)L.H + col) = z;
+    zs[rg + 8 * u][c4] = z;
+  }
+  __syncthreads();
+  if (w == 0) {
+    float4 t[4];
+#pragma unroll
+    for (int q = 0; q < 4; q++) {
+      t[q] = make_float4(0.f, 0.f, 0.f, 0.f);
+#pragma unroll
+      for (int u = 0; u < 4; u++) {
+        if (r0 + q + 4 * u < B) {
+          const float4 z = zs[q + 4 * u][c4];
+          t[q].x += z.x; t[q].y += z.y; t[q].z += z.z; t[q].w += z.w;
+        }
+      }
+    }
+    *reinterpret_cast<float4 *>(A.tile_sums + (int64_t)rt * L.H + col) =
+        make_float4((t[0].x + t[1].x) + (t[2].x + t[3].x), (t[0].y + t[1].y) + (t[2].y + t[3].y), (t[0].z + t[1].z) + (t[2].z + t[3].z),
+                    (t[0].w + t[1].w) + (t[2].w + t[3].w));
   }
 }
 
diff --git a/brl_amd/csrc/ppo_update.hpp b/brl_amd/csrc/ppo_update.hpp
--- a/brl_amd/csrc/ppo_update.hpp
+++ b/brl_amd/csrc/ppo_update.hpp
@@ -96,33 +96,12 @@
   relu_bwd_tiles4_block(dh, h, rows, cols, ld, partials, act, (int)blockIdx.x, (int)blockIdx.y);
 }
 
-constexpr int BIAS_MAX_SEGS = 16;
-struct BiasSegs {
-  int n;
-  int64_t tiles[BIAS_MAX_SEGS];
-  const float *partials[BIAS_MAX_SEGS];
-  int64_t cols[BIAS_MAX_SEGS];
-  float *db[BIAS_MAX_SEGS];
-  const int32_t *row_index;
-  int first_row_seg;
-};
+#include "norm_fin_role.hpp"
 
 __device__ __forceinline__ float bias_finalize_block(const BiasSegs &S, const int seg, const int bx, float (*part)[64]) {
   const int c = (int)(threadIdx.x & 63u), g = (int)(threadIdx.x >> 6);
   const int64_t col = (int64_t)bx * 64 + c, cols = S.cols[seg];
-  const float *p = S.partials[seg];
-  float s = 0.0f;
-  if (col < cols) {
-    const int64_t nt = S.tiles[seg];
-    for (int64_t t0 = g; t0 < nt; t0 += 64) {
-      float v[16];
-#pragma unroll
-      for (int u = 0; u < 16; u++) v[u] = p[((t0 + 4 * u < nt) ? t0 + 4 * u : t0) * cols + col];
-#pragma unroll
-      for (int u = 0; u < 16; u++) s += (t0 + 4 * u < nt) ? v[u] : 0.0f;
-    }
-  }
-  part[g][c] = s;
+  part[g][c] = bias_col_partial(S, seg, col, g);
   __syncthreads();
   float v = 0.0f;
   if (g == 0 && col < cols) {
@@ -140,8 +119,6 @@
 }
 
 constexpr int ADAM_BLOCKS = 1024, ADAM_THREADS = 256;
-
-struct FinBlocks { int off[BIAS_MAX_SEGS + 1]; };
 
 __global__ __launch_bounds__(ADAM_THREADS) void k_adam_norm_fin(const float *g, int64_t n, float gscale, float *partials, float *step,
                                                                 int32_t *mb_index, BiasSegs S, int64_t tail_lo, FinBlocks FB) {
diff --git a/brl_amd/fused_update.py b/brl_amd/fused_update.py
--- a/brl_amd/fused_update.py
+++ b/brl_amd/fused_update.py
@@ -461,6 +461,13 @@
         self._seg_tiles = (C.c_int64 * nseg)(*([self.nsplit] + [groups64 if r == 64 else groups for r in self.tile_rows] + [self.nsplit]))
         self._seg_db = (C.c_void_p * nseg)(*([self.GWh.data_ptr()] + [g.data_ptr() for g in self.Gb] + [self.Gbh.data_ptr()]))
         self._nseg = nseg
+        self.fused_heads = bool(config.get("fused_heads", False)) and not self.ill_coef and self.dw_deferred
+        self.norm_in_dw = bool(config.get("norm_in_dw", True)) and self.dw_x3 and self.allreduce_mode == "none"
+        if self.norm_in_dw:
+            tiles = sum(((t_.shape[0] + 127) // 128) * ((t_.shape[1] + 127) // 128) for t_ in self.GW)
+            self.sq_partials = f(8 * tiles + 2 * 64)
+            self._nsq = C.c_int64(0)
+            self._tail_lo = wa.start
 
     def _build_program(self):
         nl = self.nl
@@ -532,6 +539,17 @@
         s = torch.cuda.current_stream().cuda_stream
         di, cfg = self._di(), self.cfg
         x = self.h[self.nl - 1]
+        top = self.nl - 1
+        if self.fused_heads:
+            chk(L.brl_ppo_heads_loss_bwd(di, x.data_ptr(), x.stride(0), self.Wh.data_ptr(), self.bh.data_ptr(), self.H,
+                                         self.mask.data_ptr(), self.action.data_ptr(), self.old_v.data_ptr(), self.old_lp.data_ptr(),
+                                         self.adv.data_ptr(), self.tgt.data_ptr(), B, float(cfg["clip_eps"]), float(cfg["vf_coef"]),
+                                         float(cfg["ent_coef"]), int(bool(cfg.get("actor_illegal_action_mask", True))),
+                                         int(bool(cfg.get("value_clipping", True))), int(bool(cfg.get("reward_scaling", False))),
+                                         None, self.dheads.data_ptr(), self.partials.data_ptr(), self.gram_partials.data_ptr(),
+                                         self.head_parts.data_ptr(), self.head_ksplit, self.act, self.dzs[top].data_ptr(),
+                                         self.tile_sums[top].data_ptr(), s))
+            return
         chk(L.brl_ppo_heads_loss_split(di, x.data_ptr(), x.stride(0), self.Wh.data_ptr(), self.bh.data_ptr(), self.H,
                                        self.mask.data_ptr(), self.action.data_ptr(), self.old_v.data_ptr(), self.old_lp.data_ptr(),
                                        self.adv.data_ptr(), self.tgt.data_ptr(), B, float(cfg["clip_eps"]), float(cfg["vf_coef"]),
@@ -546,7 +564,6 @@
                                      self.vec.data_ptr(), s))
             chk(L.brl_ppo_illegal_grad(di, self.heads.data_ptr(), self.mask.data_ptr(), self.vec.data_ptr(), self.ill_coef, B,
                                        self.dheads.data_ptr(), s))
-        top = self.nl - 1
         chk(L.brl_ppo_heads_bwd(di, self.dheads.data_ptr(), x.data_ptr(), x.stride(0), self.Wh.data_ptr(), B, self.H, self.act,
                                 self.nsplit, None if self.dw_deferred else self.dwh_partials.data_ptr(),
                                 None if self.dw_deferred else self.dbh_partials.data_ptr(),
@@ -592,6 +609,13 @@
         nl = self.nl
         for l in range(nl - 1, 0, -1):
             self._dz(l)
+        if self.dw_x3 and self.norm_in_dw:
+            import ctypes as C
+            self.capi.check(self.lib.brl_mlp_gemm_x3_group_fin(
+                self._di(), 2, nl, *self._gdw, self.G.data_ptr(), self.n, self._tail_lo, self._nseg, self._seg_scratch, self._seg_cols,
+                self._seg_tiles, self._seg_db, 1.0, self.sq_partials.data_ptr(), self.sq_partials.numel(), self.step.data_ptr(),
+                self.mb_index.data_ptr(), C.addressof(self._nsq), torch.cuda.current_stream().cuda_stream))
+            return
         if self.dw_x3:
             self.capi.check(self.lib.brl_mlp_gemm_x3_group(self._di(), 2, nl, *self._gdw, torch.cuda.current_stream().cuda_stream))
             return
@@ -604,6 +628,12 @@
                                                       self._seg_db, torch.cuda.current_stream().cuda_stream))
 
     def _fin_opt(self):
+        if self.norm_in_dw:
+            self.capi.check(self.lib.brl_adam_apply_gather(
+                self._di(), self.P.data_ptr(), self.G.data_ptr(), self.M.data_ptr(), self.V.data_ptr(), self.n, self.step.data_ptr(),
+                self.lr, self.lr_dev.data_ptr(), float(self.b1), float(self.b2), self.eps, self.max_norm, self.sq_partials.data_ptr(),
+                self._nsq.value, self.norm.data_ptr(), self.gargs.data_ptr(), self.mbs, torch.cuda.current_stream().cuda_stream))
+            return
         self.capi.check(self.lib.brl_adam_clip_fin_gather(
             self._di(), self.P.data_ptr(), self.G.data_ptr(), self.M.data_ptr(), self.V.data_ptr(), self.n, self.step.data_ptr(), self.lr,
             self.lr_dev.data_ptr(), float(self.b1), float(self.b2), self.eps, self.max_norm, self.scratch.data_ptr(),
diff --git a/include/brl_step_fused.h b/include/brl_step_fused.h
--- /dev/null
+++ b/include/brl_step_fused.h
@@ -0,0 +1,30 @@
+#ifndef BRL_STEP_FUSED_H
+#define BRL_STEP_FUSED_H
+
+#include <stdint.h>
+
+#ifdef __cplusplus
+extern "C" {
+#endif
+
+int brl_ppo_heads_loss_bwd(int device, const float *h, int64_t ldh, const float *head_w, const float *head_b, int64_t hidden,
+                           const uint8_t *mask, const int32_t *action, const float *old_value, const float *old_log_prob,
+                           const float *gae, const float *targets, int64_t batch, float clip_eps, float vf_coef, float ent_coef,
+                           int masked, int value_clipping, int reward_scaling, float *heads_out, float *dheads, float *partials,
+                           float *gram_partials, float *head_parts, int ksplit, int act, float *dh, float *tile_sums, void *stream);
+
+int brl_mlp_gemm_x3_group_fin(int device, int layout, int count, const float *const *a, const int64_t *lda, const float *const *b,
+                              const int64_t *ldb, float *const *c, const int64_t *ldc, const int64_t *m, const int64_t *n,
+                              const int64_t *k, const float *g, int64_t n_g, int64_t tail_lo, int nseg, const float *const *partials,
+                              const int64_t *cols, const int64_t *tiles, float *const *out, float gscale, float *sq, int64_t sq_len,
+                              float *step, int32_t *mb_index, int64_t *nsq, void *stream);
+
+int brl_adam_apply_gather(int device, float *p, const float *g, float *m, float *v, int64_t n, const float *step, float lr,
+                          const float *lr_dev, float beta1, float beta2, float eps, float max_norm, const float *partials,
+                          int64_t npartials, float *norm_out, const void *gather_args, int64_t mbs, void *stream);
+
+#ifdef __cplusplus
+}
+#endif
+
+#endif
```

Result: no change. 10.66 billion (median of 4 runs) (+0.0%).
